# MSU-dcypherlab/mfgp-coverage

Hardware: NVIDIA B200
Metric: GP posterior mean+var + coverage step, grid-points/s (coverage iterations/s = 1000/ms_per_step) (higher is better)
Workload: dtype f64

## Files before the change

### include/mfgp_b200.h

```cpp
#ifndef MFGP_B200_H
#define MFGP_B200_H

#include <stdint.h>

#ifdef __cplusplus
extern "C" {
#endif

#define MFGP_TILE 64

#define MFGP_OK 0
#define MFGP_ERR_INVALID (-1)
#define MFGP_ERR_NOT_SPD (-2)
#define MFGP_ERR_CUDA (-3)
#define MFGP_ERR_EMPTY_CELL (-4)

typedef struct mfgp_params {
    double s_L, l_L;
    double s_H, l_H;
    double rho;
    double noise_L, noise_H;
    double mean_L, mean_H;
    double jitter;
    int32_t multi;
    int32_t reserved;
} mfgp_params;

const char* mfgp_version(void);
const char* mfgp_last_error(void);
int64_t mfgp_debug_chol_trace(int64_t* out, int64_t max_tasks);
int64_t mfgp_launch_count(void);
int64_t mfgp_npad(int64_t n);
int64_t mfgp_workspace_bytes(int64_t npad);


int mfgp_build_train_cov(const double* Xt, int64_t NL, int64_t NH, const mfgp_params* p_host,
                         double* K, int64_t npad, int64_t ld, double* Tt, void* stream);

int mfgp_cholesky(double* K, int64_t npad, int64_t ld, double* W, int64_t ldw, int32_t* info, void* work,
                  void* stream);

int mfgp_tri_inverse(const double* L, int64_t npad, int64_t ld, double* W, int64_t ldw, void* work, void* stream);

int mfgp_whiten(const double* W, int64_t npad, int64_t ldw, const double* y, int64_t NL, int64_t NH,
                const mfgp_params* p_host, double* z, void* stream);

int mfgp_cholesky_append(const double* Xt, int64_t NL, int64_t NH_old, int64_t NH_new, const mfgp_params* p_host,
                         double* K, int64_t ld, double* W, int64_t ldw, const double* y, double* z, double* Tt,
                         int32_t* info, void* work, int64_t work_bytes, void* stream);
int64_t mfgp_append_workspace_bytes(int64_t npad);


int mfgp_posterior(const double* Xs, int64_t G, const double* Tt, int64_t NL, int64_t NH,
                   const double* W, int64_t npad, int64_t ldw, const double* z, const mfgp_params* p_host,
                   double* mu, double* var, double* qred, double* Vc, int64_t ldv, void* stream);

int mfgp_grid_tables(const double* ux, int64_t nx, const double* uy, int64_t ny, const double* Tt, int64_t NL, int64_t NH,
                     int64_t npad, const mfgp_params* p_host, double* TLx, double* TLy, double* THx, double* THy,
                     int64_t ldt, void* stream);
int mfgp_posterior_grid(int64_t ny, int64_t g_lo, int64_t G, const double* TLx, const double* TLy, const double* THx,
                        const double* THy, int64_t ldt, int64_t NL, int64_t NH, const double* W, int64_t npad,
                        int64_t ldw, const double* z, const mfgp_params* p_host, double* mu, double* var, double* qred,
                        double* Vc, int64_t ldv, void* stream);

int mfgp_posterior_update(const double* Xs, int64_t G, const double* Tt, int64_t NL, int64_t NH,
                          const double* W, int64_t npad, int64_t ldw, const double* z, const mfgp_params* p_host,
                          int64_t row_lo, double* mu, double* var, double* qred, double* Vc, int64_t ldv, void* stream);
int mfgp_posterior_grid_update(int64_t ny, int64_t g_lo, int64_t G, const double* TLx, const double* TLy,
                               const double* THx, const double* THy, int64_t ldt, int64_t NL, int64_t NH, const double* W,
                               int64_t npad, int64_t ldw, const double* z, const mfgp_params* p_host, int64_t row_lo,
                               double* mu, double* var, double* qred, double* Vc, int64_t ldv, void* stream);

int mfgp_posterior_grid_factored(const double* ux, int64_t nx, const double* uy, int64_t ny, int64_t ix0, int64_t ncols,
                                 const double* Xt, int64_t NL, int64_t NH, const double* W, int64_t npad, int64_t ldw,
                                 const double* z, const mfgp_params* p_host, int64_t rxL, int64_t ryL, int64_t rxH, int64_t ryH,
                                 double xlo, double xhi, double ylo, double yhi, int64_t chunk_cols,
                                 double* mu, double* var, double* qred, double* Gstore, double* Hz_store, void* work,
                                 int64_t work_bytes, void* stream);
int mfgp_posterior_grid_factored_update(const double* ux, int64_t nx, const double* uy, int64_t ny, int64_t ix0, int64_t ncols,
                                        const double* Xt, int64_t NL, int64_t NH, int64_t row_lo, const double* W, int64_t npad,
                                        int64_t ldw, const double* z, const mfgp_params* p_host, int64_t rxL, int64_t ryL,
                                        int64_t rxH, int64_t ryH, double xlo, double xhi, double ylo, double yhi,
                                        int64_t chunk_cols, double* mu, double* var, double* qred, double* Gstore,
                                        double* Hz_store, void* work, int64_t work_bytes, void* stream);
int64_t mfgp_factored_workspace_bytes(int64_t npad, int64_t ncols, int64_t ny, int64_t rxL, int64_t ryL, int64_t rxH,
                                      int64_t ryH, int64_t chunk_cols);

int64_t mfgp_factored_rhs_cols(int64_t rxL, int64_t ryL, int64_t rxH, int64_t ryH);
int mfgp_factored_prepare(const double* ux, int64_t nx, const double* uy, int64_t ny, int64_t ix0, int64_t ncols,
                          const double* Xt, const double* y, int64_t NL, int64_t NH, int64_t npad, const mfgp_params* p_host,
                          int64_t rxL, int64_t ryL, int64_t rxH, int64_t ryH, double xlo, double xhi, double ylo, double yhi,
                          int64_t chunk_cols, double* Ball, int64_t ldB, void* work, int64_t work_bytes, void* stream);
int64_t mfgp_cholesky_solve_workspace_bytes(int64_t npad, int64_t R);
int mfgp_cholesky_solve(double* K, int64_t npad, int64_t ld, double* W, int64_t ldw, int32_t* info, double* Bm, int64_t ldb,
                        int64_t R, void* work, int64_t work_bytes, void* stream);
int mfgp_posterior_grid_factored_solved(const double* ux, int64_t nx, const double* uy, int64_t ny, int64_t ix0, int64_t ncols,
                                        const double* Xt, int64_t NL, int64_t NH, int64_t npad, const mfgp_params* p_host,
                                        int64_t rxL, int64_t ryL, int64_t rxH, int64_t ryH, double xlo, double xhi, double ylo,
                                        double yhi, int64_t chunk_cols, const double* Yall, int64_t ldY, double* z_out,
                                        double* mu, double* var, double* qred, double* Gstore, double* Hz_store, void* work,
                                        int64_t work_bytes, void* stream);

int64_t mfgp_factored_rhs_cols_trunc(int64_t ry, const int32_t* kx);
int mfgp_posterior_grid_factored_trunc(const double* ux, int64_t nx, const double* uy, int64_t ny, int64_t ix0, int64_t ncols,
                                       const double* Xt, int64_t NL, int64_t NH, const double* W, int64_t npad, int64_t ldw,
                                       const double* z, const mfgp_params* p_host, int64_t rxL, int64_t ryL, int64_t rxH, int64_t ryH,
                                       double xlo, double xhi, double ylo, double yhi, int64_t chunk_cols, const int32_t* kx,
                                       double* mu, double* var, double* qred, double* Gstore, double* Hz_store, void* work,
                                       int64_t work_bytes, void* stream);
int mfgp_factored_prepare_trunc(const double* ux, int64_t nx, const double* uy, int64_t ny, int64_t ix0, int64_t ncols,
                                const double* Xt, const double* y, int64_t NL, int64_t NH, int64_t npad, const mfgp_params* p_host,
                                int64_t rxL, int64_t ryL, int64_t rxH, int64_t ryH, double xlo, double xhi, double ylo, double yhi,
                                int64_t chunk_cols, const int32_t* kx, double* Ball, int64_t ldB, void* work, int64_t work_bytes,
                                void* stream);
double* mfgp_factored_gram_target(int64_t nx, int64_t ny, int64_t ix0, int64_t ncols, int64_t NL, int64_t NH, int64_t npad,
                                  const mfgp_params* p_host, int64_t rxL, int64_t ryL, int64_t rxH, int64_t ryH,
                                  int64_t chunk_cols, const int32_t* kx, int64_t ldY, void* work, int64_t work_bytes);
int64_t mfgp_cholesky_solve_gram_workspace_bytes(int64_t npad, int64_t R);
int mfgp_cholesky_solve_gram(double* K, int64_t npad, int64_t ld, double* W, int64_t ldw, int32_t* info, double* Bm, int64_t ldb,
                             int64_t R, double* M, int64_t ldm, void* work, int64_t work_bytes, void* stream);
int mfgp_posterior_grid_factored_solved_gram(const double* ux, int64_t nx, const double* uy, int64_t ny, int64_t ix0,
                                             int64_t ncols, const double* Xt, int64_t NL, int64_t NH, int64_t npad,
                                             const mfgp_params* p_host, int64_t rxL, int64_t ryL, int64_t rxH, int64_t ryH,
                                             double xlo, double xhi, double ylo, double yhi, int64_t chunk_cols,
                                             const int32_t* kx, const double* Yall, int64_t ldY, double* z_out, double* mu,
                                             double* var, double* qred, double* Gstore, double* Hz_store, void* work,
                                             int64_t work_bytes, void* stream);


int cov_assign_reduce(const double* xy, const double* w, const double* var, const double* f, int64_t G,
                      int64_t base_index,
                      const double* seeds_c, int64_t Ac, const double* poly_xy_c, const int32_t* poly_off_c, int64_t nvert_c,
                      const double* seeds_p, int64_t Ap, const double* poly_xy_p, const int32_t* poly_off_p, int64_t nvert_p,
                      double tie_tol, double amax_k0, double amax_rel,
                      double* cent, double* amax_val, int64_t* amax_idx, double* lossp,
                      uint64_t* member_c, int32_t* tie_count, void* work, int64_t work_bytes, void* stream);
int64_t cov_workspace_bytes(int64_t G, int64_t Ac, int64_t Ap);

int cov_assign_reduce_grid(const double* xy, const double* w, const double* var, const double* f, int64_t G, int64_t ny,
                           int64_t base_index,
                           const double* seeds_c, int64_t Ac, const double* poly_xy_c, const int32_t* poly_off_c, int64_t nvert_c,
                           const double* seeds_p, int64_t Ap, const double* poly_xy_p, const int32_t* poly_off_p, int64_t nvert_p,
                           double tie_tol, double amax_k0, double amax_rel,
                           double* cent, double* amax_val, int64_t* amax_idx, double* lossp,
                           int32_t* tie_count, void* work, int64_t work_bytes, void* stream);

int64_t cov_voronoi_clip_workspace_bytes(int64_t A);
int cov_voronoi_clip(const double* seeds, int64_t A, double xmin, double xmax, double ymin, double ymax, double eps,
                     double* poly_xy, int32_t* poly_off, int64_t cap_vertices, double* areas, int32_t* flag, void* work,
                     int64_t work_bytes, void* stream);

int cov_finish(const double* cent, const double* areas_c, int64_t Ac, const double* lossp, const double* areas_p, int64_t Ap,
               const double* amax_val, const int64_t* amax_idx, double xmin, double xmax, double ymin, double ymax,
               const int32_t* flag0, const int32_t* flag1, const int32_t* flag2, const int32_t* flag3, double* out,
               void* stream);

int cov_argmax(const double* v, int64_t G, int64_t base_index, double k0, double rel, double* out_val, int64_t* out_idx,
               void* work, int64_t work_bytes, void* stream);


int64_t choi_greedy(const double* Xs, int64_t G, double* Vc, int64_t ldv, int64_t n0, int64_t cap, double* var,
                    double* qred, const mfgp_params* p_host, double threshold, double tie_rel, int64_t max_picks,
                    int64_t* picks_host,
                    void* work, int64_t work_bytes, void* stream);


typedef struct mfgp_batch {
    int64_t runs, G, nx, ny, A, NL, cap, algo , iterations, max_samples;
    double xmin, xmax, ymin, ymax, eps, tie_tol, amax_rel;
    const double* xy; const double* f; const double* ux; const double* uy;
    double* Xt; double* y; double* W; double* z;
    double* TxL; double* TyL; double* TxH; double* TyH;
    double* mu; double* var;
    double* pos; double* prev; double* cen;
    int64_t* pos_idx;
    double* prob; int32_t* explore;
    int32_t* Ncur; int32_t* knew; int32_t* status; int32_t* noise_used; int32_t* nsamples; int32_t* ties;
    const double* noise; const double* unif;
    double* log_loss; double* log_agent; double* log_sample;
    double* q; int64_t* picks; int32_t* nplan; int32_t* plan_state; int32_t* pmask; int32_t* ccount; int32_t* cties;
    int32_t* tour_off; int32_t* tour_cur; int64_t* tour;
} mfgp_batch;

int mfgp_batch_step(const mfgp_batch* b_host, const mfgp_params* p_host, int64_t iteration, void* stream);


int mfgp_batch_choi_begin(const mfgp_batch* b_host, const mfgp_params* p_host, void* stream);

int mfgp_batch_choi_plan(const mfgp_batch* b_host, const mfgp_params* p_host, double threshold, int64_t rounds, void* stream);

int mfgp_batch_choi_cluster(const mfgp_batch* b_host, void* stream);

int mfgp_batch_choi_tours(const mfgp_batch* b_host, int64_t n_total, int64_t n_max, double* pts, int64_t* gidx, int32_t* ord,
                          void* work, int64_t work_bytes, void* stream);


int64_t mfgp_nlml_workspace_bytes(int64_t npad);
int mfgp_nlml_grad(const double* L, int64_t npad, int64_t ld, const double* W, int64_t ldw, const double* z, const double* Tt,
                   int64_t NL, int64_t NH, const mfgp_params* p_host, double* out, void* work, int64_t work_bytes,
                   void* stream);


int64_t choi_tsp_workspace_bytes(int64_t n_total);
int choi_tsp_tours(const double* pts, const int32_t* off, int64_t A, int64_t n_total, int64_t n_max, int32_t* order,
                   int32_t* moves, void* work, int64_t work_bytes, void* stream);

#ifdef __cplusplus
}
#endif
#endif
```

### mfgp-coverage_b200/_engine.py

```python
import ctypes
import os
import itertools

import numpy as np
import torch

from . import _native as nat

FUSED_GRAM = os.environ.get("MFGP_FUSED_GRAM", "1") != "0"


def chebyshev_order(length_scale, lo, hi, centre_lo, centre_hi, tol=5e-15, rmax=64):
    half, mid = 0.5 * (hi - lo), 0.5 * (hi + lo)
    if not (half > 0.0) or not (length_scale > 0.0):
        return None
    centres = np.linspace(min(centre_lo, lo), max(centre_hi, hi), 17)
    for r in range(8, rmax + 1, 4):
        j = np.arange(r)
        nodes = mid + half * np.cos(np.pi * (j + 0.5) / r)
        f = np.exp(-0.5 * ((nodes[:, None] - centres[None, :]) / length_scale) ** 2)
        c = (np.cos(np.pi * np.outer(np.arange(r), j + 0.5) / r) @ f) * (2.0 / r)
        scale = max(float(np.abs(c).max()), 1e-300)
        if float(np.abs(c[-3:]).max()) <= tol * scale:
            return r
# ... 312 lines not shown
                                                         nat.ptr(mu), nat.ptr(var), nat.ptr(q_out), None, 0,
                                                         nat.stream_ptr()), "mfgp_posterior_grid_update")
            else:
                nat.check(lib.mfgp_posterior_update(nat.ptr(xs_dev), G, nat.ptr(self.Tt), self.NL, self.NH, nat.ptr(self.W),
                                                    self.npad, self.cap, nat.ptr(self.z), ctypes.byref(self.pstruct),
                                                    row_lo, nat.ptr(mu), nat.ptr(var), nat.ptr(q_out), None, 0,
                                                    nat.stream_ptr()), "mfgp_posterior_update")
            return mu, var
        if axes is not None and self.N > 0:
            TLx, TLy, THx, THy, ldt, _ = self.grid_tables(axes)
            nat.check(lib.mfgp_posterior_grid(axes.ny, int(g_lo), G, nat.ptr(TLx), nat.ptr(TLy), nat.ptr(THx),
                                              nat.ptr(THy), ldt, self.NL, self.NH, nat.ptr(self.W), self.npad, self.cap,
                                              nat.ptr(self.z), ctypes.byref(self.pstruct), nat.ptr(mu), nat.ptr(var),
                                              nat.ptr(q_out), nat.ptr(vcache), ldv, nat.stream_ptr()),
                      "mfgp_posterior_grid")
            return mu, var
        nat.check(lib.mfgp_posterior(nat.ptr(xs_dev), G, nat.ptr(self.Tt), self.NL, self.NH, nat.ptr(self.W),
                                     self.npad, self.cap, nat.ptr(self.z), ctypes.byref(self.pstruct), nat.ptr(mu),
                                     nat.ptr(var), nat.ptr(q_out), nat.ptr(vcache), ldv, nat.stream_ptr()),
                  "mfgp_posterior")
        return mu, var

    def _training_range(self):
        if self._xrange is None:
            xt = self.Xt[:self.N]
            lo, hi = xt.min(dim=0).values.tolist(), xt.max(dim=0).values.tolist()
            self._xrange = (lo[0], hi[0], lo[1], hi[1])
        return self._xrange

    def _cheb_orders(self, axes, p, xlo, xhi):
        ylo, yhi = axes.ylo, axes.yhi
        t = self._training_range()
        c = self._forders
        if c is not None and c[0] == (axes.uid, xlo, xhi, p["l_L"], p["l_H"], p["multi"]) and c[1][0] <= t[0] and c[1][1] >= t[1] \
                and c[1][2] <= t[2] and c[1][3] >= t[3]:
            return c[2]
        mx, my = 0.05 * (axes.xhi - axes.xlo), 0.05 * (yhi - ylo)
        hull = (min(t[0], axes.xlo) - mx, max(t[1], axes.xhi) + mx, min(t[2], ylo) - my, max(t[3], yhi) + my)
        rxH = chebyshev_order(p["l_H"], xlo, xhi, hull[0], hull[1])
        ryH = chebyshev_order(p["l_H"], ylo, yhi, hull[2], hull[3])
        rxL = ryL = 0
        ok = rxH is not None and ryH is not None
        if ok and p["multi"]:
            rxL = chebyshev_order(p["l_L"], xlo, xhi, hull[0], hull[1])
            ryL = chebyshev_order(p["l_L"], ylo, yhi, hull[2], hull[3])
            ok = rxL is not None and ryL is not None
        orders = (rxL, ryL, rxH, ryH) if ok else None
        self._ftrunc = None
        if ok and TRUNCATE:
            parts = [(chebyshev_envelope(p["l_H"], xlo, xhi, hull[0], hull[1], rxH),
                      chebyshev_envelope(p["l_H"], ylo, yhi, hull[2], hull[3], ryH))]
            if p["multi"]:
                parts.append((chebyshev_envelope(p["l_L"], xlo, xhi, hull[0], hull[1], rxL),
                              chebyshev_envelope(p["l_L"], ylo, yhi, hull[2], hull[3], ryL)))
            kp = -(-max(rxL, rxH) // 4) * 4
            parts = [(np.pad(ax, (0, kp - ax.size)), ay) for ax, ay in parts]
            self._ftrunc = chebyshev_truncation(parts, kp, max(ryL, ryH))
        self._forders = ((axes.uid, xlo, xhi, p["l_L"], p["l_H"], p["multi"]), hull, orders)
        return orders

    def _factored_plan(self, axes, g_lo, G):
        ny = axes.ny
        if ny < 2 or axes.nx < 2 or g_lo % ny or G % ny:
            return None
        p = self.params
        N = self.npad
        dense = 0.5 * G * N * N
        if self.factored_min_gain > 0 and dense < 4e9:
            return None
        ix0, ncols = g_lo // ny, G // ny
        if ncols < 2:
            return None
        xs = axes.ux_host[ix0:ix0 + ncols]
        xlo, xhi = float(xs.min()), float(xs.max())
        if not (xhi > xlo):
            return None
        key = (axes.uid, g_lo, G, self.npad, p["l_L"], p["l_H"], p["multi"], self.factored_min_gain)
        orders = self._cheb_orders(axes, p, xlo, xhi)
        if self._fplan is not None and self._fplan[0] == key and self._fplan[2] == orders and self._fplan[3] is self._ftrunc:
            return self._fplan[1]
        plan = None
        if orders is not None:
            rxL, ryL, rxH, ryH = orders
            ry, kp = max(ryL, ryH), -(-max(rxL, rxH) // 4) * 4
            R = ry * kp
            fact = 0.5 * N * N * R + ncols * N * R + ncols * N * 64 * 64 + G * 64 * 64
            if fact * self.factored_min_gain < dense:
                chunk = max(64, min(-(-ncols // 64) * 64, ((1 << 28) // max(self.cap * max(ryL, ryH), 1)) // 64 * 64))
                plan = dict(rxL=rxL, ryL=ryL, rxH=rxH, ryH=ryH, xlo=xlo, xhi=xhi, ylo=axes.ylo, yhi=axes.yhi,
                            ix0=ix0, ncols=ncols, chunk=chunk, macs=fact, dense_macs=dense, kx=self._ftrunc)
        self._fplan = (key, plan, orders, self._ftrunc)
        return plan


    def _wsalloc(self, n, slack=8):
        if not GUARD:
            return torch.empty(n + slack, dtype=torch.float64, device=self.device)
        big = torch.full((n + 1024,), _CANARY, dtype=torch.float64, device=self.device)
        self._guards = [g for g in getattr(self, "_guards", []) if g[0] is not None]
        self._guards.append((big, n))
        return big[512:512 + n]

    def check_guards(self):
        torch.cuda.synchronize(self.device)
        return all(bool((big[:512] == _CANARY).all().item()) and bool((big[512 + n:] == _CANARY).all().item())
                   for big, n in getattr(self, "_guards", []))

    def _factored_work(self, axes, plan):
        need = int(nat.lib().mfgp_factored_workspace_bytes(self.cap, plan["ncols"], axes.ny, plan["rxL"], plan["ryL"],
                                                           plan["rxH"], plan["ryH"], plan["chunk"]))
        if self._fwork is None or self._fwork.numel() * 8 < need:
            self._fwork = self._wsalloc(need // 8)
        return self._fwork

    def _factored_stores(self, plan):
        if not self.incremental:
            return None, None
        lib = nat.lib()
        nG = plan["ncols"] * 64 * 64
        nH = int(lib.mfgp_factored_rhs_cols(plan["rxL"], plan["ryL"], plan["rxH"], plan["ryH"]))
        if self._fG is None or self._fG.numel() < nG:
            self._fG = self._wsalloc(nG, 0)
        if self._fHz is None or self._fHz.numel() < nH:
            self._fHz = self._wsalloc(nH, 0)
        return self._fG, self._fHz

    def _fit_and_posterior_fused(self, axes, plan, mu, var, q_out):
        lib = nat.lib()
        st = nat.stream_ptr()
        pp = ctypes.byref(self.pstruct)
        npad, ld = self.npad, self.cap
        o = (plan["rxL"], plan["ryL"], plan["rxH"], plan["ryH"])
        work = self._factored_work(axes, plan)
        geom = (ctypes.c_double(plan["xlo"]), ctypes.c_double(plan["xhi"]), ctypes.c_double(plan["ylo"]),
                ctypes.c_double(plan["yhi"]), plan["chunk"])
        kx = plan.get("kx") if (FUSED_GRAM and not self.incremental) else None
        M, R = None, 0
        if FUSED_GRAM:
            if kx is not None:
                kxp = ctypes.c_void_p(kx.ctypes.data)
                R = int(lib.mfgp_factored_rhs_cols_trunc(int(kx.size), kxp))
                M = lib.mfgp_factored_gram_target(axes.nx, axes.ny, plan["ix0"], plan["ncols"], self.NL, self.NH, npad, pp, *o,
                                                  plan["chunk"], kxp, R, nat.ptr(work), work.numel() * 8)
            if not M:
                kx, kxp = None, None
                R = int(lib.mfgp_factored_rhs_cols(*o))
                M = lib.mfgp_factored_gram_target(axes.nx, axes.ny, plan["ix0"], plan["ncols"], self.NL, self.NH, npad, pp, *o,
                                                  plan["chunk"], None, R, nat.ptr(work), work.numel() * 8)
        else:
            kx, kxp = None, None
            R = int(lib.mfgp_factored_rhs_cols(*o))
        if self._fB is None or self._fB.numel() < self.cap * R:
            self._fB = self._wsalloc(self.cap * R, 0)
        nat.check(lib.mfgp_build_train_cov(nat.ptr(self.Xt), self.NL, self.NH, pp, nat.ptr(self.K), npad, ld,
                                           nat.ptr(self.Tt), st), "mfgp_build_train_cov")
        nat.check(lib.mfgp_factored_prepare_trunc(nat.ptr(axes.ux), axes.nx, nat.ptr(axes.uy), axes.ny, plan["ix0"], plan["ncols"],
                                                  nat.ptr(self.Xt), nat.ptr(self.y), self.NL, self.NH, npad, pp, *o, *geom,
                                                  kxp if kx is not None else None, nat.ptr(self._fB), R, nat.ptr(work),
                                                  work.numel() * 8, st), "mfgp_factored_prepare")
        ev = self.profile_events
        if ev is not None:
            ev[0].record()
        cneed = int(lib.mfgp_cholesky_solve_gram_workspace_bytes(self.cap, R))
        if self._cwork is None or self._cwork.numel() * 8 < cneed:
            self._cwork = self._wsalloc(cneed // 8)
        nat.check(lib.mfgp_cholesky_solve_gram(nat.ptr(self.K), npad, ld, nat.ptr(self.W), ld, nat.ptr(self.info),
                                               nat.ptr(self._fB), R, R, ctypes.c_void_p(M), R, nat.ptr(self._cwork),
                                               self._cwork.numel() * 8, st), "mfgp_cholesky_solve_gram")
        if ev is not None:
            ev[1].record()
        Gs, Hs = self._factored_stores(plan)
        if M:
            nat.check(lib.mfgp_posterior_grid_factored_solved_gram(
                nat.ptr(axes.ux), axes.nx, nat.ptr(axes.uy), axes.ny, plan["ix0"], plan["ncols"], nat.ptr(self.Xt), self.NL,
                self.NH, npad, pp, *o, *geom, kxp if kx is not None else None, nat.ptr(self._fB), R, nat.ptr(self.z), nat.ptr(mu),
                nat.ptr(var), nat.ptr(q_out), nat.ptr(Gs), nat.ptr(Hs), nat.ptr(work), work.numel() * 8, st),
                "mfgp_posterior_grid_factored_solved_gram")
        else:
            nat.check(lib.mfgp_posterior_grid_factored_solved(
                nat.ptr(axes.ux), axes.nx, nat.ptr(axes.uy), axes.ny, plan["ix0"], plan["ncols"], nat.ptr(self.Xt), self.NL,
                self.NH, npad, pp, *o, *geom, nat.ptr(self._fB), R, nat.ptr(self.z), nat.ptr(mu), nat.ptr(var), nat.ptr(q_out),
                nat.ptr(Gs), nat.ptr(Hs), nat.ptr(work), work.numel() * 8, st), "mfgp_posterior_grid_factored_solved")
        self.rhs_cols = (int(kx.sum()) if kx is not None else max(plan["ryL"], plan["ryH"]) * (-(-max(plan["rxL"], plan["rxH"]) // 4) * 4), R)
        self.fused_gram = bool(M)
        self._dirty = False
        self._w_partial = True

    def _posterior_factored(self, axes, plan, mu, var, q_out, row_lo=0):
        lib = nat.lib()
        work = self._factored_work(axes, plan)
        Gs, Hs = self._factored_stores(plan)
        geom = (ctypes.c_double(plan["xlo"]), ctypes.c_double(plan["xhi"]), ctypes.c_double(plan["ylo"]),
                ctypes.c_double(plan["yhi"]), plan["chunk"])
        o = (plan["rxL"], plan["ryL"], plan["rxH"], plan["ryH"])
        if row_lo > 0 and Gs is not None:
            nat.check(lib.mfgp_posterior_grid_factored_update(
                nat.ptr(axes.ux), axes.nx, nat.ptr(axes.uy), axes.ny, plan["ix0"], plan["ncols"], nat.ptr(self.Xt), self.NL,
                self.NH, int(row_lo), nat.ptr(self.W), self.npad, self.cap, nat.ptr(self.z), ctypes.byref(self.pstruct), *o, *geom,
                nat.ptr(mu), nat.ptr(var), nat.ptr(q_out), nat.ptr(Gs), nat.ptr(Hs), nat.ptr(work), work.numel() * 8,
                nat.stream_ptr()), "mfgp_posterior_grid_factored_update")
            return
        kx = plan.get("kx") if Gs is None else None
        nat.check(lib.mfgp_posterior_grid_factored_trunc(
            nat.ptr(axes.ux), axes.nx, nat.ptr(axes.uy), axes.ny, plan["ix0"], plan["ncols"], nat.ptr(self.Xt), self.NL, self.NH,
            nat.ptr(self.W), self.npad, self.cap, nat.ptr(self.z), ctypes.byref(self.pstruct), *o, *geom,
            ctypes.c_void_p(kx.ctypes.data) if kx is not None else None, nat.ptr(mu), nat.ptr(var),
            nat.ptr(q_out), nat.ptr(Gs), nat.ptr(Hs), nat.ptr(work), work.numel() * 8, nat.stream_ptr()),
            "mfgp_posterior_grid_factored")

    def nlml_grad(self):
        if self.N == 0:
            raise ValueError("likelihood of an empty model")
        self.ensure_factor(need_inverse=True)
        self.check_factor(force=True)
        lib = nat.lib()
        need = int(lib.mfgp_nlml_workspace_bytes(self.npad))
        if self._twork is None or self._twork.numel() * 8 < need:
            self._twork = torch.empty(need // 8 + 8, dtype=torch.float64, device=self.device)
        out = torch.empty(10, dtype=torch.float64, device=self.device)
        nat.check(lib.mfgp_nlml_grad(nat.ptr(self.K), self.npad, self.cap, nat.ptr(self.W), self.cap, nat.ptr(self.z),
                                     nat.ptr(self.Tt), self.NL, self.NH, ctypes.byref(self.pstruct), nat.ptr(out),
                                     nat.ptr(self._twork), self._twork.numel() * 8, nat.stream_ptr()), "mfgp_nlml_grad")
        h = out.cpu().numpy()
        return float(h[0]), h[1:].copy()

    def clone(self):
        self.ensure_factor()
        other = DeviceGP(self.device)
        other.NL, other.NH, other.npad, other.cap = self.NL, self.NH, self.npad, self.cap
        other.params = None if self.params is None else dict(self.params)
        other.pstruct = None if self.params is None else params_struct(self.params)
        other.fitted = self.fitted
        for name in ("Xt", "y", "K", "W", "Tt", "z", "work"):
            t = getattr(self, name)
            setattr(other, name, None if t is None else t.clone())
        other.info = self.info.clone()
        other.fit_id = self.fit_id
        other.incremental = self.incremental
        other.use_factored = self.use_factored
        other.factored_min_gain = self.factored_min_gain
        other.lazy_check = self.lazy_check
        other.defer_fit = self.defer_fit
        other.epoch = self.epoch
        return other
```

### mfgp-coverage_b200/_native.py

```python
import ctypes
import os
from ctypes import POINTER, Structure, c_char_p, c_double, c_int, c_int32, c_int64, c_void_p

_HERE = os.path.dirname(os.path.abspath(__file__))
LIB_PATH = os.path.join(_HERE, "csrc", "libmfgp_b200.so")

MFGP_OK, MFGP_ERR_INVALID, MFGP_ERR_NOT_SPD, MFGP_ERR_CUDA, MFGP_ERR_EMPTY_CELL = 0, -1, -2, -3, -4
TILE = 64


class NativeLibraryMissing(RuntimeError):
    pass


class MfgpParams(Structure):
    _fields_ = [("s_L", c_double), ("l_L", c_double), ("s_H", c_double), ("l_H", c_double), ("rho", c_double),
                ("noise_L", c_double), ("noise_H", c_double), ("mean_L", c_double), ("mean_H", c_double),
                ("jitter", c_double), ("multi", c_int32), ("reserved", c_int32)]


class MfgpBatch(Structure):
    _fields_ = [(n, c_int64) for n in ("runs", "G", "nx", "ny", "A", "NL", "cap", "algo", "iterations", "max_samples")] + \
               [(n, c_double) for n in ("xmin", "xmax", "ymin", "ymax", "eps", "tie_tol", "amax_rel")] + \
               [(n, c_void_p) for n in ("xy", "f", "ux", "uy", "Xt", "y", "W", "z", "TxL", "TyL", "TxH", "TyH", "mu", "var", "pos",
                                        "prev", "cen", "pos_idx", "prob", "explore", "Ncur", "knew", "status", "noise_used",
                                        "nsamples", "ties", "noise", "unif", "log_loss", "log_agent", "log_sample",
                                        "q", "picks", "nplan", "plan_state", "pmask", "ccount", "cties", "tour_off", "tour_cur",
                                        "tour")]


SIGNATURES = {
    "mfgp_version": (c_char_p, []),
    "mfgp_last_error": (c_char_p, []),
    "mfgp_launch_count": (c_int64, []),
    "mfgp_debug_chol_trace": (c_int64, [c_void_p, c_int64]),
    "mfgp_npad": (c_int64, [c_int64]),
    "mfgp_workspace_bytes": (c_int64, [c_int64]),
    "mfgp_build_train_cov": (c_int, [c_void_p, c_int64, c_int64, POINTER(MfgpParams), c_void_p, c_int64, c_int64,
                                     c_void_p, c_void_p]),
    "mfgp_cholesky": (c_int, [c_void_p, c_int64, c_int64, c_void_p, c_int64, c_void_p, c_void_p, c_void_p]),
    "mfgp_tri_inverse": (c_int, [c_void_p, c_int64, c_int64, c_void_p, c_int64, c_void_p, c_void_p]),
    "mfgp_whiten": (c_int, [c_void_p, c_int64, c_int64, c_void_p, c_int64, c_int64, POINTER(MfgpParams), c_void_p,
                            c_void_p]),
    "mfgp_posterior": (c_int, [c_void_p, c_int64, c_void_p, c_int64, c_int64, c_void_p, c_int64, c_int64, c_void_p,
                               POINTER(MfgpParams), c_void_p, c_void_p, c_void_p, c_void_p, c_int64, c_void_p]),
    "mfgp_grid_tables": (c_int, [c_void_p, c_int64, c_void_p, c_int64, c_void_p, c_int64, c_int64, c_int64,
                                 POINTER(MfgpParams), c_void_p, c_void_p, c_void_p, c_void_p, c_int64, c_void_p]),
    "mfgp_posterior_grid": (c_int, [c_int64, c_int64, c_int64, c_void_p, c_void_p, c_void_p, c_void_p, c_int64, c_int64,
                                    c_int64, c_void_p, c_int64, c_int64, c_void_p, POINTER(MfgpParams), c_void_p,
                                    c_void_p, c_void_p, c_void_p, c_int64, c_void_p]),
    "mfgp_cholesky_append": (c_int, [c_void_p, c_int64, c_int64, c_int64, POINTER(MfgpParams), c_void_p, c_int64,
                                     c_void_p, c_int64, c_void_p, c_void_p, c_void_p, c_void_p, c_void_p, c_int64,
                                     c_void_p]),
    "mfgp_append_workspace_bytes": (c_int64, [c_int64]),
    "mfgp_posterior_update": (c_int, [c_void_p, c_int64, c_void_p, c_int64, c_int64, c_void_p, c_int64, c_int64,
                                      c_void_p, POINTER(MfgpParams), c_int64, c_void_p, c_void_p, c_void_p, c_void_p,
                                      c_int64, c_void_p]),
    "mfgp_posterior_grid_update": (c_int, [c_int64, c_int64, c_int64, c_void_p, c_void_p, c_void_p, c_void_p, c_int64,
                                           c_int64, c_int64, c_void_p, c_int64, c_int64, c_void_p, POINTER(MfgpParams),
                                           c_int64, c_void_p, c_void_p, c_void_p, c_void_p, c_int64, c_void_p]),
    "mfgp_posterior_grid_factored": (c_int, [c_void_p, c_int64, c_void_p, c_int64, c_int64, c_int64, c_void_p, c_int64,
                                             c_int64, c_void_p, c_int64, c_int64, c_void_p, POINTER(MfgpParams), c_int64,
                                             c_int64, c_int64, c_int64, c_double, c_double, c_double, c_double, c_int64,
                                             c_void_p, c_void_p, c_void_p, c_void_p, c_void_p, c_void_p, c_int64, c_void_p]),
    "mfgp_posterior_grid_factored_trunc": (c_int, [c_void_p, c_int64, c_void_p, c_int64, c_int64, c_int64, c_void_p, c_int64,
                                                   c_int64, c_void_p, c_int64, c_int64, c_void_p, POINTER(MfgpParams), c_int64,
                                                   c_int64, c_int64, c_int64, c_double, c_double, c_double, c_double, c_int64,
                                                   c_void_p, c_void_p, c_void_p, c_void_p, c_void_p, c_void_p, c_void_p, c_int64,
                                                   c_void_p]),
    "mfgp_posterior_grid_factored_update": (c_int, [c_void_p, c_int64, c_void_p, c_int64, c_int64, c_int64, c_void_p, c_int64,
                                                    c_int64, c_int64, c_void_p, c_int64, c_int64, c_void_p, POINTER(MfgpParams),
                                                    c_int64, c_int64, c_int64, c_int64, c_double, c_double, c_double, c_double,
                                                    c_int64, c_void_p, c_void_p, c_void_p, c_void_p, c_void_p, c_void_p, c_int64,
                                                    c_void_p]),
    "mfgp_factored_workspace_bytes": (c_int64, [c_int64, c_int64, c_int64, c_int64, c_int64, c_int64, c_int64, c_int64]),
    "mfgp_factored_rhs_cols": (c_int64, [c_int64, c_int64, c_int64, c_int64]),
    "mfgp_factored_prepare": (c_int, [c_void_p, c_int64, c_void_p, c_int64, c_int64, c_int64, c_void_p, c_void_p, c_int64,
                                      c_int64, c_int64, POINTER(MfgpParams), c_int64, c_int64, c_int64, c_int64, c_double,
                                      c_double, c_double, c_double, c_int64, c_void_p, c_int64, c_void_p, c_int64, c_void_p]),
    "mfgp_cholesky_solve_workspace_bytes": (c_int64, [c_int64, c_int64]),
    "mfgp_cholesky_solve": (c_int, [c_void_p, c_int64, c_int64, c_void_p, c_int64, c_void_p, c_void_p, c_int64, c_int64,
                                    c_void_p, c_int64, c_void_p]),
    "mfgp_posterior_grid_factored_solved": (c_int, [c_void_p, c_int64, c_void_p, c_int64, c_int64, c_int64, c_void_p, c_int64,
                                                    c_int64, c_int64, POINTER(MfgpParams), c_int64, c_int64, c_int64,
                                                    c_int64, c_double, c_double, c_double, c_double, c_int64, c_void_p,
                                                    c_int64, c_void_p, c_void_p, c_void_p, c_void_p, c_void_p, c_void_p,
                                                    c_void_p, c_int64, c_void_p]),
    "mfgp_factored_rhs_cols_trunc": (c_int64, [c_int64, c_void_p]),
    "mfgp_factored_prepare_trunc": (c_int, [c_void_p, c_int64, c_void_p, c_int64, c_int64, c_int64, c_void_p, c_void_p, c_int64,
                                            c_int64, c_int64, POINTER(MfgpParams), c_int64, c_int64, c_int64, c_int64, c_double,
                                            c_double, c_double, c_double, c_int64, c_void_p, c_void_p, c_int64, c_void_p, c_int64,
                                            c_void_p]),
    "mfgp_factored_gram_target": (c_void_p, [c_int64, c_int64, c_int64, c_int64, c_int64, c_int64, c_int64, POINTER(MfgpParams),
                                             c_int64, c_int64, c_int64, c_int64, c_int64, c_void_p, c_int64, c_void_p, c_int64]),
    "mfgp_cholesky_solve_gram_workspace_bytes": (c_int64, [c_int64, c_int64]),
    "mfgp_cholesky_solve_gram": (c_int, [c_void_p, c_int64, c_int64, c_void_p, c_int64, c_void_p, c_void_p, c_int64, c_int64,
                                         c_void_p, c_int64, c_void_p, c_int64, c_void_p]),
    "mfgp_posterior_grid_factored_solved_gram": (c_int, [c_void_p, c_int64, c_void_p, c_int64, c_int64, c_int64, c_void_p, c_int64,
                                                         c_int64, c_int64, POINTER(MfgpParams), c_int64, c_int64, c_int64,
                                                         c_int64, c_double, c_double, c_double, c_double, c_int64, c_void_p,
                                                         c_void_p, c_int64, c_void_p, c_void_p, c_void_p, c_void_p, c_void_p,
                                                         c_void_p, c_void_p, c_int64, c_void_p]),
    "cov_assign_reduce": (c_int, [c_void_p, c_void_p, c_void_p, c_void_p, c_int64, c_int64,
                                  c_void_p, c_int64, c_void_p, c_void_p, c_int64,
                                  c_void_p, c_int64, c_void_p, c_void_p, c_int64,
                                  c_double, c_double, c_double, c_void_p, c_void_p, c_void_p, c_void_p, c_void_p, c_void_p,
                                  c_void_p, c_int64, c_void_p]),
    "cov_workspace_bytes": (c_int64, [c_int64, c_int64, c_int64]),
    "cov_assign_reduce_grid": (c_int, [c_void_p, c_void_p, c_void_p, c_void_p, c_int64, c_int64, c_int64,
                                       c_void_p, c_int64, c_void_p, c_void_p, c_int64,
                                       c_void_p, c_int64, c_void_p, c_void_p, c_int64,
                                       c_double, c_double, c_double, c_void_p, c_void_p, c_void_p, c_void_p, c_void_p,
                                       c_void_p, c_int64, c_void_p]),
    "cov_voronoi_clip_workspace_bytes": (c_int64, [c_int64]),
    "cov_voronoi_clip": (c_int, [c_void_p, c_int64, c_double, c_double, c_double, c_double, c_double, c_void_p, c_void_p,
                                 c_int64, c_void_p, c_void_p, c_void_p, c_int64, c_void_p]),
    "cov_finish": (c_int, [c_void_p, c_void_p, c_int64, c_void_p, c_void_p, c_int64, c_void_p, c_void_p, c_double,
                           c_double, c_double, c_double, c_void_p, c_void_p, c_void_p, c_void_p, c_void_p, c_void_p]),
    "cov_argmax": (c_int, [c_void_p, c_int64, c_int64, c_double, c_double, c_void_p, c_void_p, c_void_p, c_int64,
                           c_void_p]),
    "choi_greedy": (c_int64, [c_void_p, c_int64, c_void_p, c_int64, c_int64, c_int64, c_void_p, c_void_p,
                              POINTER(MfgpParams), c_double, c_double, c_int64, POINTER(c_int64), c_void_p, c_int64,
                              c_void_p]),
    "mfgp_batch_step": (c_int, [POINTER(MfgpBatch), POINTER(MfgpParams), c_int64, c_void_p]),
    "mfgp_batch_choi_begin": (c_int, [POINTER(MfgpBatch), POINTER(MfgpParams), c_void_p]),
    "mfgp_batch_choi_plan": (c_int, [POINTER(MfgpBatch), POINTER(MfgpParams), c_double, c_int64, c_void_p]),
    "mfgp_batch_choi_cluster": (c_int, [POINTER(MfgpBatch), c_void_p]),
    "mfgp_batch_choi_tours": (c_int, [POINTER(MfgpBatch), c_int64, c_int64, c_void_p, c_void_p, c_void_p, c_void_p, c_int64,
                                      c_void_p]),
    "mfgp_nlml_workspace_bytes": (c_int64, [c_int64]),
    "mfgp_nlml_grad": (c_int, [c_void_p, c_int64, c_int64, c_void_p, c_int64, c_void_p, c_void_p, c_int64, c_int64,
                               POINTER(MfgpParams), c_void_p, c_void_p, c_int64, c_void_p]),
    "choi_tsp_workspace_bytes": (c_int64, [c_int64]),
    "choi_tsp_tours": (c_int, [c_void_p, c_void_p, c_int64, c_int64, c_int64, c_void_p, c_void_p, c_void_p, c_int64,
                               c_void_p]),
}

_lib = None


def lib():
    global _lib
    if _lib is None:
        if not os.path.isfile(LIB_PATH):
            raise NativeLibraryMissing(
                f"{LIB_PATH} not found: build it with `make -C {os.path.dirname(LIB_PATH)}` "
                "(or `python -c 'import __graft_entry__ as g; g.build()'`). There is no CPU fallback.")
        handle = ctypes.CDLL(LIB_PATH)
        for name, (res, args) in SIGNATURES.items():
            fn = getattr(handle, name)
            fn.restype = res
            fn.argtypes = args
        _lib = handle
    return _lib


def last_error():
    return lib().mfgp_last_error().decode()


def check(rc, what):
    if rc == MFGP_OK:
        return
    if rc == MFGP_ERR_CUDA:
        raise RuntimeError(f"{what}: CUDA error: {last_error()}")
    if rc == MFGP_ERR_INVALID:
        raise ValueError(f"{what}: invalid argument")
    raise RuntimeError(f"{what}: error code {rc}")


def npad(n):
    return max(TILE, (int(n) + TILE - 1) // TILE * TILE)


def ptr(t):
    return None if t is None else c_void_p(t.data_ptr())


_side_streams = {}


def side_stream(device=None):
    import torch
    dev = torch.cuda.current_device() if device is None else torch.device(device).index
    if dev is None:
        dev = torch.cuda.current_device()
    if dev not in _side_streams:
        _side_streams[dev] = torch.cuda.Stream(device=dev)
    return _side_streams[dev]


def stream_ptr(stream=None):
    import torch
    if stream is not None:
        return c_void_p(stream.cuda_stream)
    try:
        return c_void_p(torch._C._cuda_getCurrentRawStream(torch._C._cuda_getDevice()))
    except AttributeError:
        return c_void_p(torch.cuda.current_stream().cuda_stream)


def require_cuda():
    import torch
    if not torch.cuda.is_available():
        raise RuntimeError("mfgp_coverage_b200 needs a CUDA device (B200, sm_100a); there is no CPU fallback")
    lib()
```

### mfgp-coverage_b200/csrc/common.cuh

```cuda
#pragma once
#include <cstdint>
#include <cstdio>
#include <cuda.h>
#include <cuda_runtime.h>

#include "../../include/mfgp_b200.h"

namespace mfgp {

void set_last_error(const char* what, cudaError_t e);

#define MFGP_CUDA_CHECK(expr)                                   \
    do {                                                        \
        cudaError_t _e = (expr);                                \
        if (_e != cudaSuccess) {                                \
            ::mfgp::set_last_error(#expr, _e);                  \
            return MFGP_ERR_CUDA;                               \
        }                                                       \
    } while (0)

void count_launch();
#define MFGP_LAUNCH_CHECK()                  \
    do {                                     \
        ::mfgp::count_launch();              \
        MFGP_CUDA_CHECK(cudaGetLastError()); \
    } while (0)

__device__ __forceinline__ void dmma884(double& c0, double& c1, double a, double b) {
    asm volatile("mma.sync.aligned.m8n8k4.row.col.f64.f64.f64.f64 {%0,%1}, {%2}, {%3}, {%0,%1};\n"
                 : "+d"(c0), "+d"(c1)
                 : "d"(a), "d"(b));
}

__device__ __forceinline__ void cp_async16(void* smem_dst, const void* gmem_src, bool valid) {
    unsigned s = static_cast<unsigned>(__cvta_generic_to_shared(smem_dst));
    int bytes = valid ? 16 : 0;
    asm volatile("cp.async.cg.shared.global [%0], [%1], 16, %2;\n" ::"r"(s), "l"(gmem_src), "r"(bytes));
}
__device__ __forceinline__ void cp_async_commit() { asm volatile("cp.async.commit_group;\n" ::); }
template <int N>
__device__ __forceinline__ void cp_async_wait() {
    asm volatile("cp.async.wait_group %0;\n" ::"n"(N));
}

__device__ __forceinline__ uint32_t smem_u32(const void* p) { return static_cast<uint32_t>(__cvta_generic_to_shared(p)); }
__device__ __forceinline__ void mbar_init(uint32_t bar, uint32_t count) {
    asm volatile("mbarrier.init.shared::cta.b64 [%0], %1;\n" ::"r"(bar), "r"(count));
}
__device__ __forceinline__ void mbar_arrive(uint32_t bar) {
    asm volatile("mbarrier.arrive.shared::cta.b64 _, [%0];\n" ::"r"(bar) : "memory");
}
__device__ __forceinline__ void mbar_arrive_expect_tx(uint32_t bar, uint32_t bytes) {
    asm volatile("mbarrier.arrive.expect_tx.shared::cta.b64 _, [%0], %1;\n" ::"r"(bar), "r"(bytes) : "memory");
}
__device__ __forceinline__ void mbar_wait(uint32_t bar, uint32_t parity) {
    uint32_t done;
    do {
        asm volatile(
            "{\n .reg .pred p;\n mbarrier.try_wait.parity.shared::cta.b64 p, [%1], %2;\n selp.u32 %0, 1, 0, p;\n}\n"
            : "=r"(done)
            : "r"(bar), "r"(parity)
            : "memory");
    } while (!done);
}
__device__ __forceinline__ void tma_load_2d(uint32_t dst, const CUtensorMap* map, int c0, int c1, uint32_t bar) {
    asm volatile(
        "cp.async.bulk.tensor.2d.shared::cluster.global.mbarrier::complete_tx::bytes [%0], [%1, {%2, %3}], [%4];\n" ::"r"(dst),
        "l"(map), "r"(c0), "r"(c1), "r"(bar)
        : "memory");
}

typedef CUresult (*EncodeTiledFn)(CUtensorMap*, CUtensorMapDataType, cuuint32_t, void*, const cuuint64_t*, const cuuint64_t*,
                                  const cuuint32_t*, const cuuint32_t*, CUtensorMapInterleave, CUtensorMapSwizzle,
                                  CUtensorMapL2promotion, CUtensorMapFloatOOBfill);
inline int make_tensor_map_2d(CUtensorMap* map, const double* base, int64_t rows, int64_t cols, int64_t ld, int box_cols,
                              int box_rows, CUtensorMapSwizzle swizzle) {
    static EncodeTiledFn encode = nullptr;
    if (!encode) {
        void* fn = nullptr;
        cudaDriverEntryPointQueryResult qres;
        MFGP_CUDA_CHECK(cudaGetDriverEntryPoint("cuTensorMapEncodeTiled", &fn, cudaEnableDefault, &qres));
        if (qres != cudaDriverEntryPointSuccess || !fn) {
            set_last_error("cuTensorMapEncodeTiled entry point unavailable", cudaErrorUnknown);
            return MFGP_ERR_CUDA;
        }
        encode = reinterpret_cast<EncodeTiledFn>(fn);
    }
    const cuuint64_t gdim[2] = {(cuuint64_t)cols, (cuuint64_t)rows};
    const cuuint64_t gstride[1] = {(cuuint64_t)ld * sizeof(double)};
    const cuuint32_t box[2] = {(cuuint32_t)box_cols, (cuuint32_t)box_rows};
    const cuuint32_t estr[2] = {1, 1};
    const CUresult r = encode(map, CU_TENSOR_MAP_DATA_TYPE_FLOAT64, 2, const_cast<double*>(base), gdim, gstride, box, estr,
                              CU_TENSOR_MAP_INTERLEAVE_NONE, swizzle, CU_TENSOR_MAP_L2_PROMOTION_L2_256B,
                              CU_TENSOR_MAP_FLOAT_OOB_FILL_NONE);
    if (r != CUDA_SUCCESS) {
        set_last_error("cuTensorMapEncodeTiled failed", cudaErrorInvalidValue);
        return MFGP_ERR_CUDA;
    }
    return MFGP_OK;
}

__device__ __forceinline__ double rbf_scaled(double ax, double ay, double bx, double by, double scale) {
    double d0 = ax - bx, d1 = ay - by;
    double q = __dadd_rn(__dmul_rn(d0, d0), __dmul_rn(d1, d1));
    return scale * exp(-0.5 * q);
}

struct DevParams {
    double s_L, inv_unused, s_H, rho, rho2, noise_L, noise_H, mean_L, mean_H, jitter, l_L, l_H, k0;
    int multi;
};

inline DevParams make_dev_params(const mfgp_params& p) {
    DevParams d;
    d.s_L = p.multi ? p.s_L : 0.0;
    d.inv_unused = 0.0;
    d.s_H = p.s_H;
    d.rho = p.multi ? p.rho : 1.0;
    d.rho2 = d.rho * d.rho;
    d.noise_L = p.noise_L;
    d.noise_H = p.noise_H;
    d.mean_L = p.mean_L;
    d.mean_H = p.mean_H;
    d.jitter = p.jitter;
    d.l_L = p.multi ? p.l_L : 1.0;
    d.l_H = p.l_H;
    d.k0 = p.multi ? (d.rho2 * p.s_L + p.s_H) : p.s_H;
    d.multi = p.multi;
    return d;
}

}
```

### mfgp-coverage_b200/csrc/gp_factored.cu

```cuda
#include "common.cuh"
#include "gemm_f64.cuh"
#include <cstdlib>
#include <cstring>

namespace mfgp {

constexpr int F_LW = 64;
constexpr int F_MAXR = 64;

struct FTrunc {
    short off[F_MAXR + 1];
    short kx[F_MAXR];
    int ry, cols;
};

struct FPart {
    int rx, ry, kpad;
    int loff;
    double inv_l;
    double* Cx; double* Cy;
    double* B;  double* Y;
    double* Ux;
    double* Yp;
    double* Hz;
};

struct ChebJob { int axis, r; double lo, hi, inv_l; double* C; };
struct ChebJobs { ChebJob j[4]; };
constexpr int CHEB_PTS = 32;
__global__ void __launch_bounds__(256) cheb_coef_kernel(const double* __restrict__ Xt, int N, int npad, ChebJobs jobs) {
    __shared__ double D[F_MAXR * (F_MAXR + 1)];
    __shared__ double node[F_MAXR];
    __shared__ double fv[8][F_MAXR];
    const ChebJob jb = jobs.j[blockIdx.y];
    const int r = jb.r, lane = threadIdx.x & 31, wib = threadIdx.x >> 5;
    double* __restrict__ C = jb.C;
    const double mid = 0.5 * (jb.lo + jb.hi), half = 0.5 * (jb.hi - jb.lo);
    for (int e = threadIdx.x; e < r * r; e += 256) {
        const int k = e / r, j = e % r;
        D[k * (F_MAXR + 1) + j] = cospi(k * (j + 0.5) / r) * (k == 0 ? 1.0 : 2.0) / r;
    }
    for (int j = threadIdx.x; j < r; j += 256) node[j] = mid + half * cospi((j + 0.5) / r);
    __syncthreads();
    for (int i = wib; i < CHEB_PTS; i += 8) {
        const int n = blockIdx.x * CHEB_PTS + i;
        if (n >= npad) break;
        if (n >= N) {
            for (int k = lane; k < r; k += 32) C[(int64_t)k * npad + n] = 0.0;
            continue;
        }
        const double U = Xt[2 * n + jb.axis];
        __syncwarp();
        for (int j = lane; j < r; j += 32) {
            const double d = (node[j] - U) * jb.inv_l;
            fv[wib][j] = exp(-0.5 * d * d);
        }
        __syncwarp();
        for (int k = lane; k < r; k += 32) {
            double s0 = 0.0;
            for (int j = 0; j < r; j++) s0 = fma(fv[wib][j], D[k * (F_MAXR + 1) + j], s0);
            C[(int64_t)k * npad + n] = s0;
        }
    }
}

__global__ void cheb_basis_kernel(const double* __restrict__ u, int i0, int count, int rows_pad, double lo, double hi, int r, int ld,
                                  int col0, double* __restrict__ T) {
    const int i = blockIdx.x * blockDim.x + threadIdx.x;
    if (i >= rows_pad) return;
    double* row = T + (int64_t)i * ld + col0;
    if (i >= count) {
        for (int k = 0; k < r; k++) row[k] = 0.0;
        return;
    }
    const double t = (2.0 * u[i0 + i] - (lo + hi)) / (hi - lo);
    double t0 = 1.0, t1 = t;
    for (int k = 0; k < r; k++) {
        row[k] = t0;
        const double t2 = 2.0 * t * t1 - t0;
        t0 = t1; t1 = t2;
    }
}

struct BTab { const double* Cx; const double* Cy; int rx, ry; double coef_lo, coef_hi; };
__global__ void build_B_merged_kernel(BTab t0, BTab t1, int ntab, int npad, int N, int NL, FTrunc tr, double* __restrict__ B,
                                      int64_t ldB) {
    const int n = blockIdx.y;
    const int e = blockIdx.x * blockDim.x + threadIdx.x;
    if (e >= tr.cols) return;
    int l = 0;
    while (tr.off[l + 1] <= e) l++;
    const int k = e - tr.off[l];
    double v = 0.0;
    if (n < N) {
        if (l < t0.ry && k < t0.rx) v = (n < NL ? t0.coef_lo : t0.coef_hi) * t0.Cy[(int64_t)l * npad + n] * t0.Cx[(int64_t)k * npad + n];
        if (ntab > 1 && l < t1.ry && k < t1.rx)
            v += (n < NL ? t1.coef_lo : t1.coef_hi) * t1.Cy[(int64_t)l * npad + n] * t1.Cx[(int64_t)k * npad + n];
    }
    B[(int64_t)n * ldB + e] = v;
}

__global__ void build_z_block_kernel(const double* __restrict__ y, int npad, int N, int NL, double mean_L, double mean_H,
                                     double* __restrict__ B, int64_t ldB) {
    const int n = blockIdx.x, c = threadIdx.x;
    double v = 0.0;
    if (c == 0 && n < N) v = y[n] - (n < NL ? mean_L : mean_H);
    B[(int64_t)n * ldB + c] = v;
}

__global__ void unpack_Y_kernel(const double* __restrict__ Yall, int64_t ldY, int off, int cols, double* __restrict__ Yp) {
    const int n = blockIdx.y;
    const int e = blockIdx.x * blockDim.x + threadIdx.x;
    if (e < cols) Yp[(int64_t)n * cols + e] = Yall[(int64_t)n * ldY + off + e];
}
__global__ void put_z_block_kernel(const double* __restrict__ z, int npad, double* __restrict__ Yall, int64_t ldY, int zoff) {
    const int n = blockIdx.x, c = threadIdx.x;
    Yall[(int64_t)n * ldY + zoff + c] = (c == 0) ? z[n] : 0.0;
}
__global__ void unpack_z_kernel(const double* __restrict__ Yall, int64_t ldY, int off, int npad, double* __restrict__ z) {
    const int n = blockIdx.x * blockDim.x + threadIdx.x;
    if (n < npad) z[n] = Yall[(int64_t)n * ldY + off];
}

constexpr int HZ_SPLIT = 16;
__global__ void __launch_bounds__(256) hz_partial_kernel(const double* __restrict__ Y, const double* __restrict__ z, int npad, int cols,
                                                         double* __restrict__ part) {
    __shared__ double red[8][32];
    const int e = blockIdx.x * 32 + (threadIdx.x & 31), w = threadIdx.x >> 5;
    const int rows = (npad + HZ_SPLIT - 1) / HZ_SPLIT;
    const int n0 = blockIdx.y * rows, n1 = min(npad, n0 + rows);
    double s = 0.0;
    if (e < cols) {
#pragma unroll 4
        for (int n = n0 + w; n < n1; n += 8) s = fma(z[n], Y[(int64_t)n * cols + e], s);
    }
    red[w][threadIdx.x & 31] = s;
    __syncthreads();
    if (w == 0 && e < cols) {
        double t = 0.0;
#pragma unroll
        for (int k = 0; k < 8; k++) t += red[k][threadIdx.x & 31];
        part[(int64_t)blockIdx.y * cols + e] = t;
    }
}
__global__ void hz_reduce_kernel(const double* __restrict__ part, int cols, double* __restrict__ Hz, int accumulate) {
    const int e = blockIdx.x * blockDim.x + threadIdx.x;
    if (e >= cols) return;
    double t = 0.0;
#pragma unroll
    for (int k = 0; k < HZ_SPLIT; k++) t += part[(int64_t)k * cols + e];
    Hz[e] = accumulate ? Hz[e] + t : t;
}

__global__ void zero_rows_kernel(double* __restrict__ Y, int64_t cols, int nrows) {
    const int64_t e = (int64_t)blockIdx.x * blockDim.x + threadIdx.x;
    if (e < cols * nrows) Y[e] = 0.0;
}

constexpr int G_ROWS = 64;

struct GramArgs {
    const double* YpL; const double* YpH; int ryL, ryH;
    int npad;
    double* Gstore;
    int skip_eval;
    int accumulate;
    const double* HzL; const double* HzH;
    const double* UxL; const double* UxH; int kL, kH;
    const double* Uy;
    int ny; int col_begin;
    double mean, k0;
    double* mu; double* var; double* qred;
    int pitch, nstage;
    int poison;
};
constexpr int G_MAXSTAGE = 6;

__device__ __forceinline__ uint32_t f_smem_u32(const void* p) { return static_cast<uint32_t>(__cvta_generic_to_shared(p)); }
__device__ __forceinline__ void f_mbar_init(uint32_t bar, uint32_t count) {
    asm volatile("mbarrier.init.shared::cta.b64 [%0], %1;\n" ::"r"(bar), "r"(count));
}
__device__ __forceinline__ void f_mbar_arrive_expect_tx(uint32_t bar, uint32_t bytes) {
    asm volatile("mbarrier.arrive.expect_tx.shared::cta.b64 _, [%0], %1;\n" ::"r"(bar), "r"(bytes) : "memory");
}
__device__ __forceinline__ void f_mbar_wait(uint32_t bar, uint32_t parity) {
    uint32_t done;
    do {
        asm volatile(
            "{\n .reg .pred p;\n mbarrier.try_wait.parity.shared::cta.b64 p, [%1], %2;\n selp.u32 %0, 1, 0, p;\n}\n"
            : "=r"(done) : "r"(bar), "r"(parity) : "memory");
    } while (!done);
}
__device__ __forceinline__ void f_bulk_g2s(uint32_t dst, const void* src, uint32_t bytes, uint32_t bar) {
    asm volatile("cp.async.bulk.shared::cluster.global.mbarrier::complete_tx::bytes [%0], [%1], %2, [%3];\n" ::"r"(dst), "l"(src),
                 "r"(bytes), "r"(bar) : "memory");
}

__host__ __device__ constexpr int g_ring_slack(int wm, int pitch) { return wm - pitch > 8 ? wm - pitch : 8; }
template <int WM>
__global__ void __launch_bounds__(128) gram_eval_kernel(GramArgs a) {
    constexpr int NT = WM / 8, NTILES = NT * (NT + 1) / 2;
    constexpr int GP = WM + 2;
    extern __shared__ __align__(16) double gsm[];
    const int P = a.pitch, NST = a.nstage, ry = a.ryH;
    const int ring = NST * G_ROWS * P + g_ring_slack(WM, P);
    double* Ts = gsm;
    double* Gs = gsm + ring;
    double* hs = Gs + WM * GP;
    uint64_t* bars = reinterpret_cast<uint64_t*>(hs + 2 * F_LW);
    const int tid = threadIdx.x, lane = tid & 31, warp = tid >> 5;
    const int col = blockIdx.x;
    const int gq = lane >> 2, tq = lane & 3;
    const double* src = a.YpH + (int64_t)col * a.npad * ry;
    const uint32_t bar0 = f_smem_u32(bars);
    const int fill = a.poison ? ring + WM * GP + 2 * F_LW : ring;
    for (int e = tid; e < fill; e += 128) Ts[e] = e < ring ? 0.0 : __longlong_as_double(-1ll);
    if (tid == 0) {
        for (int i = 0; i < NST; i++) f_mbar_init(bar0 + 8 * i, 1);
        asm volatile("fence.mbarrier_init.release.cluster;\n" ::: "memory");
    }
    __syncthreads();
    asm volatile("fence.proxy.async.shared::cta;\n" ::: "memory");
    const uint32_t chunk_bytes = (uint32_t)(G_ROWS * ry * 8);
    const bool whole = P == ry;
    auto stage = [&](int buf, int n0) {
        if (tid == 0) f_mbar_arrive_expect_tx(bar0 + 8 * buf, chunk_bytes);
        double* dst = Ts + buf * G_ROWS * P;
        if (whole) {
            if (tid == 0) f_bulk_g2s(f_smem_u32(dst), src + (int64_t)n0 * ry, chunk_bytes, bar0 + 8 * buf);
        } else {
            __syncwarp();
            if (tid < G_ROWS) f_bulk_g2s(f_smem_u32(dst + tid * P), src + (int64_t)(n0 + tid) * ry, (uint32_t)(ry * 8), bar0 + 8 * buf);
        }
    };
    double acc[NTILES][2];
#pragma unroll
    for (int t = 0; t < NTILES; t++) acc[t][0] = acc[t][1] = 0.0;
    const int nchunk = a.npad / G_ROWS;
    for (int i = 0; i < NST - 1 && i < nchunk; i++) stage(i, i * G_ROWS);
    int buf = 0, par = 0;
    for (int ch = 0; ch < nchunk; ch++) {
        const int nx = ch + NST - 1;
        if (nx < nchunk) stage(nx % NST, nx * G_ROWS);
        f_mbar_wait(bar0 + 8 * buf, par);
        const double* T = Ts + buf * G_ROWS * P;
#pragma unroll
        for (int ks = 0; ks < G_ROWS / 16; ks++) {
            const double* row = T + (4 * (warp + 4 * ks) + tq) * P + gq;
            double f[NT];
#pragma unroll
            for (int i = 0; i < NT; i++) f[i] = row[8 * i];
#pragma unroll
            for (int i = 0; i < NT; i++)
#pragma unroll
                for (int j = 0; j <= i; j++) dmma884(acc[i * (i + 1) / 2 + j][0], acc[i * (i + 1) / 2 + j][1], f[i], f[j]);
        }
        __syncthreads();
        if (++buf == NST) { buf = 0; par ^= 1; }
    }
#pragma unroll 1
// ... 332 lines not shown
            for (int j = 0; j < NT; j++)
                if (8 * j <= 4 * ks + 3) dmma884(acc[j][0], acc[j][1], av, bf[ks][j]);
        }
        double q = 0.0, m = 0.0;
#pragma unroll
        for (int j = 0; j < NT; j++) {
            const double2 u = __ldg(reinterpret_cast<const double2*>(up + j * 8 + 2 * tq));
            q = fma(acc[j][0], u.x, q); q = fma(acc[j][1], u.y, q);
            m = fma(h0[j], u.x, m); m = fma(h1[j], u.y, m);
        }
        q += __shfl_xor_sync(0xffffffffu, q, 1); m += __shfl_xor_sync(0xffffffffu, m, 1);
        q += __shfl_xor_sync(0xffffffffu, q, 2); m += __shfl_xor_sync(0xffffffffu, m, 2);
        if (tq == 0 && m0 + gq < ny) {
            const int64_t gidx = (int64_t)col * ny + m0 + gq;
            var[gidx] = k0 - q;
            mu[gidx] = mean + m;
            if (qred) qred[gidx] = q;
        }
    }
}

__global__ void gpad_zero_kernel(double* __restrict__ G, int ry, int wm, int col_begin) {
    double* g = G + (int64_t)(col_begin + blockIdx.x) * F_LW * F_LW;
    for (int e = threadIdx.x; e < wm * wm; e += blockDim.x) {
        const int r = e / wm, c = e % wm;
        if (r >= ry || c >= ry) g[r * F_LW + c] = 0.0;
    }
}

__global__ void hz_from_M_kernel(const double* __restrict__ M, int ldm, int zrow, int cols, double* __restrict__ Hz) {
    const int e = blockIdx.x * blockDim.x + threadIdx.x;
    if (e < cols) Hz[e] = M[(int64_t)zrow * ldm + e];
}

}

using namespace mfgp;

static inline int64_t round_up(int64_t v, int64_t m) { return (v + m - 1) / m * m; }

static inline int64_t imax(int64_t a, int64_t b) { return a > b ? a : b; }
constexpr int MR_MAXSPLIT = 8;

extern "C" int64_t mfgp_factored_workspace_bytes(int64_t npad, int64_t ncols, int64_t ny, int64_t rxL, int64_t ryL, int64_t rxH,
                                                 int64_t ryH, int64_t chunk_cols) {
    const int64_t rx = imax(rxL, rxH), ry = imax(ryL, ryH), kp = round_up(rx, 4);
    const int64_t ncp = round_up(ncols, 64), ch = round_up(chunk_cols, 64);
    int64_t d = 0;
    d += ny * 64 + npad + ry * kp;
    d += (rxL + ryL + rxH + ryH) * npad;
    const int64_t Rp = round_up(ry * kp + 1, 64);
    d += 2 * npad * Rp;
    d += ncp * kp;
    const int64_t direct = ch * npad * ry;
    const int64_t gram = (MR_MAXSPLIT + 1) * Rp * Rp + ncp * F_LW * F_LW;
    d += direct > gram ? direct : gram;
    return d * 8 + 4096;
}

extern "C" int64_t mfgp_factored_rhs_cols(int64_t rxL, int64_t ryL, int64_t rxH, int64_t ryH) {
    return round_up(imax(ryL, ryH) * round_up(imax(rxL, rxH), 4) + 1, 64);
}

extern "C" int64_t mfgp_factored_rhs_cols_trunc(int64_t ry, const int32_t* kx) {
    if (!kx || ry <= 0 || ry > F_MAXR) return 0;
    int64_t c = 0;
    for (int64_t l = 0; l < ry; l++) c += kx[l];
    return round_up(c + 1, 64);
}

namespace {
struct FGeom {
    const double* ux; int64_t nx; const double* uy; int64_t ny; int64_t ix0, ncols;
    const double* Xt; int64_t NL, NH, npad;
    const mfgp_params* p;
    int64_t rxL, ryL, rxH, ryH;
    double xlo, xhi, ylo, yhi;
    int64_t chunk;
};
struct FTab { int rx, ry; double inv_l; double* Cx; double* Cy; bool lofi; };
struct FLayout {
    FTab tabs[2]; int ntabs;
    FPart parts[1]; int nparts;
    double* Uy; double* zbuf; int64_t ncp, chunk; bool multi;
    FTrunc tr; bool truncated;
};

bool f_set_trunc(FLayout& L, const int32_t* kx_host) {
    const FPart& f = L.parts[0];
    FTrunc& t = L.tr;
    t.ry = f.ry;
    L.truncated = kx_host != nullptr;
    int o = 0;
    for (int l = 0; l < f.ry; l++) {
        const int k = kx_host ? kx_host[l] : f.kpad;
        if (k < 4 || k > f.kpad || (k & 3)) return false;
        t.off[l] = (short)o; t.kx[l] = (short)k;
        o += k;
    }
    for (int l = f.ry; l < F_MAXR; l++) { t.off[l] = (short)o; t.kx[l] = 0; }
    t.off[F_MAXR] = (short)o;
    t.cols = o;
    return true;
}

int f_validate(const FGeom& g, void* work, int64_t work_bytes) {
    if (!g.ux || !g.uy || !g.Xt || !g.p || !work) return MFGP_ERR_INVALID;
    const int64_t N = g.NL + g.NH;
    if (N <= 0 || g.npad < N || g.npad % MFGP_TILE || g.ncols <= 0 || g.ix0 < 0 || g.ix0 + g.ncols > g.nx || g.ny <= 0) return MFGP_ERR_INVALID;
    const bool multi = g.p->multi != 0;
    if (!multi && (g.rxL || g.ryL || g.NL)) return MFGP_ERR_INVALID;
    if (g.rxH <= 0 || g.ryH <= 0 || g.rxH > F_MAXR || g.ryH > F_MAXR || g.rxL > F_MAXR || g.ryL > F_MAXR || (g.ryL % 4) || (g.ryH % 4))
        return MFGP_ERR_INVALID;
    if (multi && (g.rxL <= 0 || g.ryL <= 0)) return MFGP_ERR_INVALID;
    if (!(g.xhi > g.xlo) || !(g.yhi > g.ylo) || g.chunk <= 0) return MFGP_ERR_INVALID;
    if (work_bytes < mfgp_factored_workspace_bytes(g.npad, g.ncols, g.ny, g.rxL, g.ryL, g.rxH, g.ryH, g.chunk)) return MFGP_ERR_INVALID;
    return MFGP_OK;
}

void f_carve(const FGeom& g, void* work, FLayout& L) {
    L.multi = g.p->multi != 0;
    L.ncp = round_up(g.ncols, 64); L.chunk = round_up(g.chunk, 64);
    double* wp = static_cast<double*>(work);
    auto carve = [&](int64_t n) { double* r = wp; wp += n; return r; };
    L.Uy = carve(g.ny * 64);
    L.zbuf = carve(g.npad);
    L.ntabs = 0;
    auto add_tab = [&](int rx, int ry, double l, bool lofi) {
        FTab& t = L.tabs[L.ntabs++];
        t.rx = rx; t.ry = ry; t.inv_l = 1.0 / l; t.lofi = lofi;
        t.Cx = carve((int64_t)rx * g.npad); t.Cy = carve((int64_t)ry * g.npad);
    };
    if (L.multi) add_tab((int)g.rxL, (int)g.ryL, g.p->l_L, true);
    add_tab((int)g.rxH, (int)g.ryH, g.p->l_H, false);
    FPart& f = L.parts[0];
    L.nparts = 1;
    f.rx = (int)imax(g.rxL, g.rxH); f.ry = (int)imax(g.ryL, g.ryH); f.kpad = (int)round_up(f.rx, 4); f.loff = 0; f.inv_l = 0.0;
    f.Cx = f.Cy = nullptr;
    {
        const int64_t Rp = round_up((int64_t)f.ry * f.kpad + 1, 64);
        f.B = carve(g.npad * Rp); f.Y = carve(g.npad * Rp);
    }
    f.Ux = carve(L.ncp * f.kpad);
    {
        const int64_t Rp = round_up((int64_t)f.ry * f.kpad + 1, 64);
        const int64_t direct = L.chunk * g.npad * f.ry;
        const int64_t gram = (MR_MAXSPLIT + 1) * Rp * Rp + L.ncp * F_LW * F_LW;
        f.Yp = carve(direct > gram ? direct : gram);
    }
    f.Hz = carve((int64_t)f.ry * f.kpad);
    f_set_trunc(L, nullptr);
}

int f_tables_and_B(const FGeom& g, FLayout& L, double* Ball, int64_t ldB, cudaStream_t st) {
    const DevParams dp = make_dev_params(*g.p);
    const int64_t N = g.NL + g.NH, npad = g.npad;
    FPart& f = L.parts[0];
    MFGP_CUDA_CHECK(cudaMemsetAsync(L.Uy, 0, sizeof(double) * g.ny * 64, st));
    MFGP_CUDA_CHECK(cudaMemsetAsync(f.Ux, 0, sizeof(double) * L.ncp * f.kpad, st));
    cheb_basis_kernel<<<(unsigned)((L.ncp + 127) / 128), 128, 0, st>>>(g.ux, (int)g.ix0, (int)g.ncols, (int)L.ncp, g.xlo, g.xhi, f.rx, f.kpad,
                                                                    0, f.Ux);
    MFGP_LAUNCH_CHECK();
    cheb_basis_kernel<<<(unsigned)((g.ny + 127) / 128), 128, 0, st>>>(g.uy, 0, (int)g.ny, (int)g.ny, g.ylo, g.yhi, f.ry, 64, 0, L.Uy);
    MFGP_LAUNCH_CHECK();
    BTab bt[2] = {};
    ChebJobs jobs = {};
    for (int ti = 0; ti < L.ntabs; ti++) {
        FTab& t = L.tabs[ti];
        jobs.j[2 * ti] = ChebJob{0, t.rx, g.xlo, g.xhi, t.inv_l, t.Cx};
        jobs.j[2 * ti + 1] = ChebJob{1, t.ry, g.ylo, g.yhi, t.inv_l, t.Cy};
        bt[ti] = BTab{t.Cx, t.Cy, t.rx, t.ry, t.lofi ? dp.rho * dp.s_L : 0.0, t.lofi ? dp.rho2 * dp.s_L : dp.s_H};
    }
    {
        dim3 cgrid((unsigned)((npad + CHEB_PTS - 1) / CHEB_PTS), (unsigned)(2 * L.ntabs));
        cheb_coef_kernel<<<cgrid, 256, 0, st>>>(g.Xt, (int)N, (int)npad, jobs);
        MFGP_LAUNCH_CHECK();
    }
    const int cols = L.tr.cols;
    dim3 bgrid((unsigned)((cols + 127) / 128), (unsigned)npad);
    build_B_merged_kernel<<<bgrid, 128, 0, st>>>(bt[0], bt[1], L.ntabs, (int)npad, (int)N, (int)g.NL, L.tr, Ball ? Ball : f.B,
                                                Ball ? ldB : (int64_t)cols);
    MFGP_LAUNCH_CHECK();
    return MFGP_OK;
}

int f_tail(const FGeom& g, FLayout& L, const double* z, int64_t rows, double* Gstore, double* Hz_store, int accumulate,
           double* mu, double* var, double* qred, cudaStream_t st) {
    const DevParams dp = make_dev_params(*g.p);
    const int64_t npad = rows;
    const int ry0 = L.parts[0].ry;
    const bool narrow = ry0 <= 40;
    const int wm = narrow ? 40 : 64;
    const int pitch = (ry0 % 8 == 4) ? ry0 : ry0 + 4;
    int nstage = (int)(73728 / (G_ROWS * pitch * 8));
    nstage = nstage < 2 ? 2 : (nstage > G_MAXSTAGE ? G_MAXSTAGE : nstage);
    const size_t gsmem = sizeof(double) * ((size_t)nstage * G_ROWS * pitch + g_ring_slack(wm, pitch) + wm * (wm + 2) + 2 * F_LW) +
                         8 * G_MAXSTAGE + 64;
    const char* pe = getenv("MFGP_DEBUG_POISON_SMEM");
    const int poison = pe && std::strcmp(pe, "1") == 0;
    MFGP_CUDA_CHECK(cudaFuncSetAttribute(gram_eval_kernel<40>, cudaFuncAttributeMaxDynamicSharedMemorySize, (int)gsmem));
    MFGP_CUDA_CHECK(cudaFuncSetAttribute(gram_eval_kernel<64>, cudaFuncAttributeMaxDynamicSharedMemorySize, (int)gsmem));
    int64_t hoff = 0;
    for (int pi = 0; pi < L.nparts; pi++) {
        FPart& f = L.parts[pi];
        const int cols = f.ry * f.kpad;
        if (Hz_store) f.Hz = Hz_store + hoff;
        hz_partial_kernel<<<dim3((unsigned)((cols + 31) / 32), HZ_SPLIT), 256, 0, st>>>(f.Y, z, (int)npad, cols, f.Yp);
        MFGP_LAUNCH_CHECK();
        hz_reduce_kernel<<<(cols + 127) / 128, 128, 0, st>>>(f.Yp, cols, f.Hz, accumulate);
        MFGP_LAUNCH_CHECK();
        hoff += cols;
    }
    for (int64_t c0 = 0; c0 < g.ncols; c0 += L.chunk) {
        const int64_t cc = (g.ncols - c0 < L.chunk) ? g.ncols - c0 : L.chunk;
        const int64_t ccp = round_up(cc, 64);
        for (int pi = 0; pi < L.nparts; pi++) {
            FPart& f = L.parts[pi];
            GemmArgs gm{};
            gm.A = f.Ux + c0 * f.kpad; gm.lda = f.kpad; gm.B = f.Y; gm.ldb = f.kpad; gm.C = f.Yp; gm.ldc = npad * (int64_t)f.ry;
            gm.M = (int)ccp; gm.N = (int)(npad * f.ry); gm.K = f.kpad; gm.alpha = 1.0; gm.beta = 0.0; gm.mode = GEMM_GENERAL;
            int rc = launch_gemm(gm, true, 1, st);
            if (rc) return rc;
        }
        GramArgs ga;
        ga.YpL = nullptr; ga.YpH = L.parts[0].Yp;
        ga.ryL = 0; ga.ryH = L.parts[0].ry;
        ga.npad = (int)npad; ga.Uy = L.Uy; ga.ny = (int)g.ny; ga.col_begin = (int)c0;
        ga.Gstore = Gstore; ga.accumulate = accumulate;
        ga.skip_eval = Gstore != nullptr;
        ga.HzL = nullptr; ga.HzH = L.parts[0].Hz;
        ga.UxL = nullptr; ga.UxH = L.parts[0].Ux + c0 * L.parts[0].kpad;
        ga.kL = 0; ga.kH = L.parts[0].kpad;
        ga.mean = dp.mean_H; ga.k0 = dp.k0; ga.mu = mu; ga.var = var; ga.qred = qred;
        ga.pitch = pitch; ga.nstage = nstage; ga.poison = poison;
        if (narrow) gram_eval_kernel<40><<<(unsigned)cc, 128, gsmem, st>>>(ga);
        else gram_eval_kernel<64><<<(unsigned)cc, 128, gsmem, st>>>(ga);
        MFGP_LAUNCH_CHECK();
    }
    if (Gstore) {
        FPart& f = L.parts[0];
        if (narrow)
            geval_mma_kernel<40><<<(unsigned)g.ncols, 128, 0, st>>>(Gstore, f.Hz, f.Ux, f.kpad, f.ry, L.tr, L.Uy, (int)g.ny, dp.mean_H, dp.k0, mu, var, qred);
        else
            geval_mma_kernel<64><<<(unsigned)g.ncols, 128, 0, st>>>(Gstore, f.Hz, f.Ux, f.kpad, f.ry, L.tr, L.Uy, (int)g.ny, dp.mean_H, dp.k0, mu, var, qred);
        MFGP_LAUNCH_CHECK();
    }
    return MFGP_OK;
}
int gram_route_override() {
    const char* e = getenv("MFGP_GRAM");
    if (!e) return 0;
    return std::strcmp(e, "direct") == 0 ? 1 : (std::strcmp(e, "m") == 0 ? 2 : 0);
}

bool f_gram_wanted(const FGeom& g, const FLayout& L, int64_t ldY) {
    const FPart& f = L.parts[0];
    const int64_t npad = g.npad, cols = L.tr.cols;
    const int wm = f.ry <= 40 ? 40 : 64;
    const int nt8 = (f.kpad + 7) / 8;
    if (ldY % 64 || ldY < cols + 1 || nt8 > 8) return false;
    const int ov = gram_route_override();
    if (L.truncated) return ov != 1;
    const double direct = (double)g.ncols * npad * cols + 0.6 * g.ncols * npad * wm * wm;
    const double gram = 0.5 * npad * (double)ldY * ldY + (double)round_up(g.ncols, 64) * (f.ry * (f.ry + 1) / 2) * 64.0 * nt8 * nt8;
    return !(ov == 1 || (ov == 0 && gram >= direct));
}

int64_t f_max_ldY(const FLayout& L) { return round_up((int64_t)L.parts[0].ry * L.parts[0].kpad + 1, 64); }

int f_tail_gram(const FGeom& g, FLayout& L, const double* Yall, int64_t ldY, double* Gstore, double* Hz_store, double* mu,
                double* var, double* qred, bool m_ready, cudaStream_t st) {
    FPart& f = L.parts[0];
    const int64_t npad = g.npad, cols = L.tr.cols;
    const int wm = f.ry <= 40 ? 40 : 64;
    const int nt8 = (f.kpad + 7) / 8;
    if (!f_gram_wanted(g, L, ldY)) return (m_ready || L.truncated) ? MFGP_ERR_INVALID : 1;
    if (L.truncated && (Gstore || Hz_store)) return MFGP_ERR_INVALID;
    const DevParams dp = make_dev_params(*g.p);
    double* M = f.Yp;
    double* part = M + ldY * ldY;
    double* Gbuf = Gstore ? Gstore : part + (int64_t)MR_MAXSPLIT * ldY * ldY;
    if (!m_ready) {
        const int ntile = (int)(ldY / 64), tiles = ntile * (ntile + 1) / 2;
        int nsplit = 740 / tiles;
        if (nsplit < 1) nsplit = 1;
        if (nsplit > MR_MAXSPLIT) nsplit = MR_MAXSPLIT;
        if (nsplit > npad / 128) nsplit = (int)imax(1, npad / 128);
        const int kchunk = (int)((npad / 64 + nsplit - 1) / nsplit) * 64;
        nsplit = (int)((npad + kchunk - 1) / kchunk);
        GemmArgs gm{};
        gm.A = Yall; gm.lda = ldY; gm.B = Yall; gm.ldb = ldY; gm.C = nsplit > 1 ? part : M; gm.ldc = ldY; gm.strideC = ldY * ldY;
        gm.M = (int)ldY; gm.N = (int)ldY; gm.K = (int)npad; gm.alpha = 1.0; gm.beta = 0.0; gm.mode = GEMM_SYRK_LOWER;
        gm.kchunk = nsplit > 1 ? kchunk : 0;
        int rc = launch_syrk_ata(gm, nsplit, st);
        if (rc) return rc;
        if (nsplit > 1) {
            syrk_reduce_lower_kernel<<<dim3((unsigned)((ldY + 127) / 128), (unsigned)ldY), 128, 0, st>>>(part, nsplit, ldY * ldY, (int)ldY, M);
            MFGP_LAUNCH_CHECK();
        }
    }
    if (Hz_store) f.Hz = Hz_store;
    hz_from_M_kernel<<<(unsigned)((cols + 127) / 128), 128, 0, st>>>(M, (int)ldY, (int)cols, (int)cols, f.Hz);
    MFGP_LAUNCH_CHECK();
    QformArgs qa;
    qa.M = M; qa.ldm = (int)ldY; qa.Ux = f.Ux; qa.kpad = f.kpad; qa.tr = L.tr; qa.ry = f.ry; qa.ncols = (int)g.ncols; qa.G = Gbuf; qa.col_begin = 0;
    const int npairs = f.ry * (f.ry + 1) / 2;
    const int cblocks = (int)((g.ncols + 63) / 64);
    int groups = (148 * 3) / cblocks;
    if (groups < 1) groups = 1;
    if (groups > npairs) groups = npairs;
    qa.pairs_per_cta = (npairs + groups - 1) / groups;
    groups = (npairs + qa.pairs_per_cta - 1) / qa.pairs_per_cta;
    const dim3 qgrid((unsigned)cblocks, (unsigned)groups);
    switch (nt8) {
        case 1: qform_kernel<1, true><<<qgrid, 128, 0, st>>>(qa); break;
        case 2: qform_kernel<2, true><<<qgrid, 128, 0, st>>>(qa); break;
        case 3: qform_kernel<3, true><<<qgrid, 128, 0, st>>>(qa); break;
        case 4: qform_kernel<4, true><<<qgrid, 128, 0, st>>>(qa); break;
        case 5: qform_kernel<5, true><<<qgrid, 128, 0, st>>>(qa); break;
        case 6: qform_kernel<6, true><<<qgrid, 128, 0, st>>>(qa); break;
        case 7: qform_kernel<7, false><<<qgrid, 128, 0, st>>>(qa); break;
        default: qform_kernel<8, false><<<qgrid, 128, 0, st>>>(qa); break;
    }
    MFGP_LAUNCH_CHECK();
    static const bool eval_fma = [] { const char* e = getenv("MFGP_GEVAL"); return e && std::strcmp(e, "fma") == 0; }();
    if (eval_fma) {
        if (wm == 40)
            geval_kernel<40, 2><<<(unsigned)g.ncols, 256, 0, st>>>(Gbuf, f.Hz, f.Ux, f.kpad, f.ry, L.tr, L.Uy, (int)g.ny, dp.mean_H, dp.k0, mu, var, qred);
        else
            geval_kernel<64, 1><<<(unsigned)g.ncols, 256, 0, st>>>(Gbuf, f.Hz, f.Ux, f.kpad, f.ry, L.tr, L.Uy, (int)g.ny, dp.mean_H, dp.k0, mu, var, qred);
    } else if (wm == 40) {
        geval_mma_kernel<40><<<(unsigned)g.ncols, 128, 0, st>>>(Gbuf, f.Hz, f.Ux, f.kpad, f.ry, L.tr, L.Uy, (int)g.ny, dp.mean_H, dp.k0, mu, var, qred);
    } else {
        geval_mma_kernel<64><<<(unsigned)g.ncols, 128, 0, st>>>(Gbuf, f.Hz, f.Ux, f.kpad, f.ry, L.tr, L.Uy, (int)g.ny, dp.mean_H, dp.k0, mu, var, qred);
    }
    MFGP_LAUNCH_CHECK();
    if (Gstore && f.ry < wm) {
        gpad_zero_kernel<<<(unsigned)g.ncols, 128, 0, st>>>(Gbuf, f.ry, wm, 0);
        MFGP_LAUNCH_CHECK();
    }
    return MFGP_OK;
}
}

extern "C" int mfgp_posterior_grid_factored_trunc(const double* ux, int64_t nx, const double* uy, int64_t ny, int64_t ix0, int64_t ncols,
                                                  const double* Xt, int64_t NL, int64_t NH, const double* W, int64_t npad, int64_t ldw,
                                                  const double* z, const mfgp_params* p_host, int64_t rxL, int64_t ryL, int64_t rxH,
                                                  int64_t ryH, double xlo, double xhi, double ylo, double yhi, int64_t chunk_cols,
                                                  const int32_t* kx, double* mu, double* var, double* qred, double* Gstore,
                                                  double* Hz_store, void* work, int64_t work_bytes, void* stream) {
    if (!W || !z || !mu || !var || ldw < npad) return MFGP_ERR_INVALID;
    FGeom g{ux, nx, uy, ny, ix0, ncols, Xt, NL, NH, npad, p_host, rxL, ryL, rxH, ryH, xlo, xhi, ylo, yhi, chunk_cols};
    int rc = f_validate(g, work, work_bytes);
    if (rc) return rc;
    cudaStream_t st = static_cast<cudaStream_t>(stream);
    FLayout L;
    f_carve(g, work, L);
    FPart& f0 = L.parts[0];
    if (kx && !Gstore && !Hz_store && gram_route_override() != 1) {
        if (!f_set_trunc(L, kx)) return MFGP_ERR_INVALID;
    }
    const int64_t cols0 = L.tr.cols, Rp = round_up(cols0 + 1, 64);
    if (!Gstore && !Hz_store && f_gram_wanted(g, L, Rp)) {
        rc = f_tables_and_B(g, L, f0.B, Rp, st);
        if (rc) return rc;
        put_z_block_kernel<<<(unsigned)npad, (int)(Rp - cols0), 0, st>>>(z, (int)npad, f0.B, Rp, (int)cols0);
        MFGP_LAUNCH_CHECK();
        GemmArgs gm{};
        gm.A = W; gm.lda = ldw; gm.B = f0.B; gm.ldb = Rp; gm.C = f0.Y; gm.ldc = Rp;
        gm.M = (int)npad; gm.N = (int)Rp; gm.K = (int)npad; gm.alpha = 1.0; gm.beta = 0.0; gm.mode = GEMM_A_LOWER;
        rc = launch_gemm(gm, false, 1, st);
        if (rc) return rc;
        put_z_block_kernel<<<(unsigned)npad, (int)(Rp - cols0), 0, st>>>(z, (int)npad, f0.Y, Rp, (int)cols0);
        MFGP_LAUNCH_CHECK();
        return f_tail_gram(g, L, f0.Y, Rp, nullptr, nullptr, mu, var, qred, false, st);
    }
    rc = f_tables_and_B(g, L, nullptr, 0, st);
    if (rc) return rc;
    for (int pi = 0; pi < L.nparts; pi++) {
        FPart& f = L.parts[pi];
        GemmArgs gm{};
        gm.A = W; gm.lda = ldw; gm.B = f.B; gm.ldb = (int64_t)f.ry * f.kpad; gm.C = f.Y; gm.ldc = (int64_t)f.ry * f.kpad;
        gm.M = (int)npad; gm.N = f.ry * f.kpad; gm.K = (int)npad; gm.alpha = 1.0; gm.beta = 0.0; gm.mode = GEMM_A_LOWER;
        rc = launch_gemm(gm, false, 1, st);
        if (rc) return rc;
    }
    return f_tail(g, L, z, npad, Gstore, Hz_store, 0, mu, var, qred, st);
}

extern "C" int mfgp_posterior_grid_factored(const double* ux, int64_t nx, const double* uy, int64_t ny, int64_t ix0, int64_t ncols,
                                            const double* Xt, int64_t NL, int64_t NH, const double* W, int64_t npad, int64_t ldw,
                                            const double* z, const mfgp_params* p_host, int64_t rxL, int64_t ryL, int64_t rxH,
                                            int64_t ryH, double xlo, double xhi, double ylo, double yhi, int64_t chunk_cols,
                                            double* mu, double* var, double* qred, double* Gstore, double* Hz_store, void* work,
                                            int64_t work_bytes, void* stream) {
    return mfgp_posterior_grid_factored_trunc(ux, nx, uy, ny, ix0, ncols, Xt, NL, NH, W, npad, ldw, z, p_host, rxL, ryL, rxH, ryH, xlo, xhi,
                                              ylo, yhi, chunk_cols, nullptr, mu, var, qred, Gstore, Hz_store, work, work_bytes, stream);
}

extern "C" int mfgp_factored_prepare_trunc(const double* ux, int64_t nx, const double* uy, int64_t ny, int64_t ix0, int64_t ncols,
                                           const double* Xt, const double* y, int64_t NL, int64_t NH, int64_t npad,
                                           const mfgp_params* p_host, int64_t rxL, int64_t ryL, int64_t rxH, int64_t ryH, double xlo,
                                           double xhi, double ylo, double yhi, int64_t chunk_cols, const int32_t* kx, double* Ball,
                                           int64_t ldB, void* work, int64_t work_bytes, void* stream) {
    if (!y || !Ball) return MFGP_ERR_INVALID;
    FGeom g{ux, nx, uy, ny, ix0, ncols, Xt, NL, NH, npad, p_host, rxL, ryL, rxH, ryH, xlo, xhi, ylo, yhi, chunk_cols};
    int rc = f_validate(g, work, work_bytes);
    if (rc) return rc;
    cudaStream_t st = static_cast<cudaStream_t>(stream);
    FLayout L;
    f_carve(g, work, L);
    if (!f_set_trunc(L, kx)) return MFGP_ERR_INVALID;
    const int64_t zoff = L.tr.cols;
    const int64_t R = round_up(zoff + 1, 64);
    if (ldB < R) return MFGP_ERR_INVALID;
    rc = f_tables_and_B(g, L, Ball, ldB, st);
    if (rc) return rc;
    build_z_block_kernel<<<(unsigned)npad, (int)(R - zoff), 0, st>>>(y, (int)npad, (int)(NL + NH), (int)NL, p_host->mean_L, p_host->mean_H,
                                                                     Ball + zoff, ldB);
    MFGP_LAUNCH_CHECK();
    return MFGP_OK;
}

extern "C" int mfgp_factored_prepare(const double* ux, int64_t nx, const double* uy, int64_t ny, int64_t ix0, int64_t ncols,
                                     const double* Xt, const double* y, int64_t NL, int64_t NH, int64_t npad,
                                     const mfgp_params* p_host, int64_t rxL, int64_t ryL, int64_t rxH, int64_t ryH, double xlo,
                                     double xhi, double ylo, double yhi, int64_t chunk_cols, double* Ball, int64_t ldB, void* work,
                                     int64_t work_bytes, void* stream) {
    return mfgp_factored_prepare_trunc(ux, nx, uy, ny, ix0, ncols, Xt, y, NL, NH, npad, p_host, rxL, ryL, rxH, ryH, xlo, xhi, ylo, yhi,
                                       chunk_cols, nullptr, Ball, ldB, work, work_bytes, stream);
}

namespace {
int f_solved_impl(const FGeom& g, const int32_t* kx, const double* Yall, int64_t ldY, double* z_out, double* mu, double* var,
                  double* qred, double* Gstore, double* Hz_store, void* work, int64_t work_bytes, bool m_ready, cudaStream_t st) {
    if (!Yall || !mu || !var) return MFGP_ERR_INVALID;
    int rc = f_validate(g, work, work_bytes);
    if (rc) return rc;
    FLayout L;
    f_carve(g, work, L);
    if (!f_set_trunc(L, kx)) return MFGP_ERR_INVALID;
    const int64_t npad = g.npad;
    const int64_t zoff = L.tr.cols;
    if (ldY < round_up(zoff + 1, 64) || ldY > f_max_ldY(L)) return MFGP_ERR_INVALID;
    unpack_z_kernel<<<(unsigned)((npad + 255) / 256), 256, 0, st>>>(Yall, ldY, (int)zoff, (int)npad, L.zbuf);
    MFGP_LAUNCH_CHECK();
    if (z_out) MFGP_CUDA_CHECK(cudaMemcpyAsync(z_out, L.zbuf, sizeof(double) * npad, cudaMemcpyDeviceToDevice, st));
    rc = f_tail_gram(g, L, Yall, ldY, Gstore, Hz_store, mu, var, qred, m_ready, st);
    if (rc <= 0) return rc;
    int64_t off = 0;
    for (int pi = 0; pi < L.nparts; pi++) {
        FPart& f = L.parts[pi];
        const int cols = f.ry * f.kpad;
        dim3 ug((unsigned)((cols + 255) / 256), (unsigned)npad);
        unpack_Y_kernel<<<ug, 256, 0, st>>>(Yall, ldY, (int)off, cols, f.Y);
        MFGP_LAUNCH_CHECK();
        off += cols;
    }
    return f_tail(g, L, L.zbuf, npad, Gstore, Hz_store, 0, mu, var, qred, st);
}
}

extern "C" int mfgp_posterior_grid_factored_solved(const double* ux, int64_t nx, const double* uy, int64_t ny, int64_t ix0,
                                                   int64_t ncols, const double* Xt, int64_t NL, int64_t NH, int64_t npad,
                                                   const mfgp_params* p_host, int64_t rxL, int64_t ryL, int64_t rxH, int64_t ryH,
                                                   double xlo, double xhi, double ylo, double yhi, int64_t chunk_cols,
                                                   const double* Yall, int64_t ldY, double* z_out, double* mu, double* var,
                                                   double* qred, double* Gstore, double* Hz_store, void* work,
                                                   int64_t work_bytes, void* stream) {
    FGeom g{ux, nx, uy, ny, ix0, ncols, Xt, NL, NH, npad, p_host, rxL, ryL, rxH, ryH, xlo, xhi, ylo, yhi, chunk_cols};
    return f_solved_impl(g, nullptr, Yall, ldY, z_out, mu, var, qred, Gstore, Hz_store, work, work_bytes, false,
                         static_cast<cudaStream_t>(stream));
}

extern "C" double* mfgp_factored_gram_target(int64_t nx, int64_t ny, int64_t ix0, int64_t ncols, int64_t NL, int64_t NH, int64_t npad,
                                             const mfgp_params* p_host, int64_t rxL, int64_t ryL, int64_t rxH, int64_t ryH,
                                             int64_t chunk_cols, const int32_t* kx, int64_t ldY, void* work, int64_t work_bytes) {
    if (!p_host || !work) return nullptr;
    if (work_bytes < mfgp_factored_workspace_bytes(npad, ncols, ny, rxL, ryL, rxH, ryH, chunk_cols)) return nullptr;
    FGeom g{nullptr, nx, nullptr, ny, ix0, ncols, nullptr, NL, NH, npad, p_host, rxL, ryL, rxH, ryH, 0.0, 1.0, 0.0, 1.0, chunk_cols};
    FLayout L;
    f_carve(g, work, L);
    if (!f_set_trunc(L, kx) || ldY < round_up((int64_t)L.tr.cols + 1, 64) || ldY > f_max_ldY(L)) return nullptr;
    return f_gram_wanted(g, L, ldY) ? L.parts[0].Yp : nullptr;
}

extern "C" int mfgp_posterior_grid_factored_solved_gram(const double* ux, int64_t nx, const double* uy, int64_t ny, int64_t ix0,
                                                        int64_t ncols, const double* Xt, int64_t NL, int64_t NH, int64_t npad,
                                                        const mfgp_params* p_host, int64_t rxL, int64_t ryL, int64_t rxH,
                                                        int64_t ryH, double xlo, double xhi, double ylo, double yhi,
                                                        int64_t chunk_cols, const int32_t* kx, const double* Yall, int64_t ldY,
                                                        double* z_out, double* mu, double* var, double* qred, double* Gstore,
                                                        double* Hz_store, void* work, int64_t work_bytes, void* stream) {
    FGeom g{ux, nx, uy, ny, ix0, ncols, Xt, NL, NH, npad, p_host, rxL, ryL, rxH, ryH, xlo, xhi, ylo, yhi, chunk_cols};
    return f_solved_impl(g, kx, Yall, ldY, z_out, mu, var, qred, Gstore, Hz_store, work, work_bytes, true,
                         static_cast<cudaStream_t>(stream));
}

extern "C" int mfgp_posterior_grid_factored_update(const double* ux, int64_t nx, const double* uy, int64_t ny, int64_t ix0,
                                                   int64_t ncols, const double* Xt, int64_t NL, int64_t NH, int64_t row_lo,
                                                   const double* W, int64_t npad, int64_t ldw, const double* z,
                                                   const mfgp_params* p_host, int64_t rxL, int64_t ryL, int64_t rxH, int64_t ryH,
                                                   double xlo, double xhi, double ylo, double yhi, int64_t chunk_cols, double* mu,
                                                   double* var, double* qred, double* Gstore, double* Hz_store, void* work,
                                                   int64_t work_bytes, void* stream) {
    if (!W || !z || !mu || !var || !Gstore || !Hz_store || ldw < npad || row_lo <= 0 || row_lo >= NL + NH) return MFGP_ERR_INVALID;
    FGeom g{ux, nx, uy, ny, ix0, ncols, Xt, NL, NH, npad, p_host, rxL, ryL, rxH, ryH, xlo, xhi, ylo, yhi, chunk_cols};
    int rc = f_validate(g, work, work_bytes);
    if (rc) return rc;
    cudaStream_t st = static_cast<cudaStream_t>(stream);
    FLayout L;
    f_carve(g, work, L);
    rc = f_tables_and_B(g, L, nullptr, 0, st);
    if (rc) return rc;
    const int64_t rb = row_lo / 64 * 64;
    const int64_t M = npad - rb;
    for (int pi = 0; pi < L.nparts; pi++) {
        FPart& f = L.parts[pi];
        const int64_t cols = (int64_t)f.ry * f.kpad;
        int nsplit = (int)(npad / 512);
        if (nsplit < 1) nsplit = 1;
        if (nsplit > 16) nsplit = 16;
        while (nsplit > 1 && (int64_t)(nsplit + 1) * M * cols > npad * cols) nsplit--;
        const int kchunk = (int)((npad / 64 + nsplit - 1) / nsplit) * 64;
        nsplit = (int)((npad + kchunk - 1) / kchunk);
        double* Ynew = f.Y;
        double* part = f.Y + M * cols;
        if (nsplit > 1) {
            GemmArgs gm{};
            gm.A = W + rb * ldw; gm.lda = ldw; gm.B = f.B; gm.ldb = cols; gm.C = part; gm.ldc = cols; gm.strideC = M * cols;
            gm.M = (int)M; gm.N = (int)cols; gm.K = (int)npad; gm.alpha = 1.0; gm.beta = 0.0; gm.mode = GEMM_GENERAL; gm.kchunk = kchunk;
            rc = launch_gemm(gm, false, nsplit, st);
            if (rc) return rc;
            dim3 rgrid((unsigned)((cols + 127) / 128), (unsigned)M);
            splitk_reduce_kernel<<<rgrid, 128, 0, st>>>(part, nsplit, M * cols, (int)cols, Ynew, cols, (int)M, (int)cols, 1.0, 0.0);
            MFGP_LAUNCH_CHECK();
        } else {
            GemmArgs gm{};
            gm.A = W + rb * ldw; gm.lda = ldw; gm.B = f.B; gm.ldb = cols; gm.C = Ynew; gm.ldc = cols;
            gm.M = (int)M; gm.N = (int)cols; gm.K = (int)npad; gm.alpha = 1.0; gm.beta = 0.0; gm.mode = GEMM_GENERAL;
            rc = launch_gemm(gm, false, 1, st);
            if (rc) return rc;
        }
        if (row_lo > rb) {
            const int64_t nz = (row_lo - rb) * cols;
            zero_rows_kernel<<<(unsigned)((nz + 255) / 256), 256, 0, st>>>(Ynew, cols, (int)(row_lo - rb));
            MFGP_LAUNCH_CHECK();
        }
    }
    return f_tail(g, L, z + rb, M, Gstore, Hz_store, 1, mu, var, qred, st);
}
```

### mfgp-coverage_b200/csrc/gp_fit.cu

```cuda
#include "common.cuh"
#include "gemm_f64.cuh"
#include <cstdlib>
#include <mutex>

namespace mfgp {

__global__ void scaled_coords_kernel(const double* __restrict__ Xt, int N, int npad, DevParams p, double* __restrict__ Tt) {
    const int i = blockIdx.x * blockDim.x + threadIdx.x;
    if (i >= npad) return;
    double4 t = make_double4(0.0, 0.0, 0.0, 0.0);
    if (i < N) {
        const double xi = Xt[2 * i], yi = Xt[2 * i + 1];
        t = make_double4(xi / p.l_L, yi / p.l_L, xi / p.l_H, yi / p.l_H);
    }
    reinterpret_cast<double4*>(Tt)[i] = t;
}

__global__ void build_train_cov_kernel(const double* __restrict__ Xt, int NL, int NH, DevParams p, double* __restrict__ K,
                                       int npad, int64_t ld, const double* __restrict__ Tt, int row_begin) {
    const int j = blockIdx.x * blockDim.x + threadIdx.x;
    const int i = row_begin + blockIdx.y * blockDim.y + threadIdx.y;
    const int N = NL + NH;
    if (i >= npad || j >= npad) return;
    if (j >= ((i >> 6) + 1) * 64) return;
    double v;
    if (i >= N || j >= N) {
        v = (i == j) ? 1.0 : 0.0;
    } else {
        double4 a, b;
        if (Tt != nullptr) {
            a = reinterpret_cast<const double4*>(Tt)[i];
            b = reinterpret_cast<const double4*>(Tt)[j];
        } else {
            const double xi = Xt[2 * i], yi = Xt[2 * i + 1], xj = Xt[2 * j], yj = Xt[2 * j + 1];
            a = make_double4(xi / p.l_L, yi / p.l_L, xi / p.l_H, yi / p.l_H);
            b = make_double4(xj / p.l_L, yj / p.l_L, xj / p.l_H, yj / p.l_H);
        }
        const bool iL = i < NL, jL = j < NL;
        if (p.multi) {
            const double kL = rbf_scaled(a.x, a.y, b.x, b.y, p.s_L);
            if (iL && jL) {
                v = kL;
                if (i == j) v = v + p.noise_L;
            } else if (iL != jL) {
                v = p.rho * kL;
            } else {
                const double kH = rbf_scaled(a.z, a.w, b.z, b.w, p.s_H);
                v = __dadd_rn(__dmul_rn(p.rho2, kL), kH);
                if (i == j) v = v + p.noise_H;
            }
        } else {
            v = rbf_scaled(a.z, a.w, b.z, b.w, p.s_H);
            if (i == j) v = v + p.noise_H;
        }
        if (i == j) v = v + p.jitter;
    }
    K[(int64_t)i * ld + j] = v;
}

constexpr int PB = 64;
constexpr int PLD = PB + 1;

struct PotrfScratch {
    double2 colAB[2][PB], rowAB[2][PB];
    double piv[3][PB / 2];
    double fin[3][PB / 2];
    int bad;
};

__device__ __forceinline__ void tile_bar() { asm volatile("bar.sync 1, 256;\n" ::: "memory"); }

template <int BS>
__device__ __forceinline__ void potrf_diag_body(const double* src, int64_t lds, double* A, int64_t ld,
                                                double* __restrict__ Winv, int64_t ldw, int32_t* __restrict__ info, int col0,
                                                PotrfScratch* sc, double* Lsm = nullptr, double* Wsm = nullptr, int lds_out = 0) {
    constexpr int NB = BS / 16;
    double2 (*colAB)[PB] = sc->colAB;
    double2 (*rowAB)[PB] = sc->rowAB;
    double (*piv)[PB / 2] = sc->piv;
    double (*fin)[PB / 2] = sc->fin;
    int& bad = sc->bad;
    const int tid = threadIdx.x;
    const int ti = tid >> 4, tc = tid & 15;
    if (tid == 0) bad = 0;
    double s[NB][NB], m[NB][NB];
#pragma unroll
    for (int a = 0; a < NB; a++)
#pragma unroll
        for (int b = 0; b < NB; b++) {
            const int r = ti + 16 * a, c = tc + 16 * b;
            s[a][b] = (c <= r) ? src[(int64_t)r * lds + c] : 0.0;
            m[a][b] = (r == c) ? 1.0 : 0.0;
        }
#pragma unroll
    for (int jb = 0; jb < NB; jb++) {
#pragma unroll 1
        for (int jp = 0; jp < 8; jp++) {
            const int k = jb * 8 + jp, j0 = 2 * k, j1 = j0 + 1, jj0 = 2 * jp, buf = k & 1;
            if ((tc & 14) == jj0) {
                double* dst = reinterpret_cast<double*>(colAB[buf]) + (tc & 1);
#pragma unroll
                for (int a = 0; a < NB; a++) dst[2 * (ti + 16 * a)] = s[a][jb];
            }
            if ((ti & 14) == jj0) {
                double* dst = reinterpret_cast<double*>(rowAB[buf]) + (ti & 1);
#pragma unroll
                for (int b = 0; b < NB; b++) dst[2 * (tc + 16 * b)] = m[jb][b];
            }
            tile_bar();
            const double2* col = colAB[buf];
            const double2* row = rowAB[buf];
            double pa = col[j0].x;
            const double2 p1 = col[j1];
            double pb = p1.x, pc = p1.y;
            double det = fma(pa, pc, -(pb * pb));
            if (!(pa > 0.0) || !(det > 0.0)) {
                if (tid == 0 && !bad) {
                    bad = 1;
                    atomicCAS(info, 0, col0 + ((pa > 0.0) ? j1 : j0) + 1);
                }
                pa = 1.0; pb = 0.0; pc = 1.0; det = 1.0;
            }
            if (tid == 0) { piv[0][k] = pa; piv[1][k] = pb; piv[2][k] = pc; }
            const double idet = 1.0 / det;
            const double qa = pc * idet, qb = -pb * idet, qc = pa * idet;
            double t1[NB], t2[NB];
#pragma unroll
            for (int a = 0; a < NB; a++) {
                if (a < jb) continue;
                const double2 x = col[ti + 16 * a];
                t1[a] = fma(qa, x.x, qb * x.y);
                t2[a] = fma(qb, x.x, qc * x.y);
            }
#pragma unroll
            for (int b = 0; b < NB; b++) {
                if (b < jb) continue;
                const double2 y = col[tc + 16 * b];
                const bool live = tc + 16 * b > j1;
#pragma unroll
                for (int a = 0; a < NB; a++) {
                    if (a < b) continue;
                    if (live) s[a][b] = fma(-t1[a], y.x, fma(-t2[a], y.y, s[a][b]));
                }
            }
#pragma unroll
            for (int b = 0; b < NB; b++) {
                if (b > jb) continue;
                const double2 z = row[tc + 16 * b];
#pragma unroll
                for (int a = 0; a < NB; a++) {
                    if (a < jb) continue;
                    const bool live = ti + 16 * a > j1;
                    if (live) m[a][b] = fma(-t1[a], z.x, fma(-t2[a], z.y, m[a][b]));
                }
            }
        }
    }
    tile_bar();
    if (tid < BS / 2) {
        const double a = piv[0][tid], b = piv[1][tid], c = piv[2][tid];
        const double r1 = rsqrt(a);
        const double g = b * r1 * r1;
        fin[0][tid] = r1;
        fin[1][tid] = rsqrt(fma(-g, b, c));
        fin[2][tid] = g;
    }
    tile_bar();
    const bool failed = bad != 0;
#pragma unroll
    for (int a = 0; a < NB; a++)
#pragma unroll
        for (int b = 0; b < NB; b++) {
            const int r = ti + 16 * a, c = tc + 16 * b;
            const double v = s[a][b], w = m[a][b];
            const double vp = __shfl_up_sync(0xffffffffu, v, 1);
            const double wp = __shfl_up_sync(0xffffffffu, w, 16);
            const int kc = c >> 1, kr = r >> 1;
            const double lv = (c & 1) ? (v - fin[2][kc] * vp) * fin[1][kc] : v * fin[0][kc];
            const double wv = (r & 1) ? (w - fin[2][kr] * wp) * fin[1][kr] : w * fin[0][kr];
            const double lo = failed ? ((r == c) ? 1.0 : 0.0) : ((c <= r) ? lv : 0.0);
            const double wo = failed ? ((r == c) ? 1.0 : 0.0) : ((c <= r) ? wv : 0.0);
            if (c <= r) A[(int64_t)r * ld + c] = lo;
            if (Winv != nullptr) Winv[(int64_t)r * ldw + c] = wo;
            if (Lsm != nullptr) Lsm[r * lds_out + c] = lo;
            if (Wsm != nullptr) Wsm[r * lds_out + c] = wo;
        }
}

__global__ void __launch_bounds__(256, 1) potrf_diag_kernel(double* __restrict__ A, int64_t ld, double* __restrict__ Winv,
                                                         int64_t ldw, int32_t* __restrict__ info, int jblk) {
    __shared__ __align__(16) PotrfScratch scratch;
    potrf_diag_body<PB>(A, ld, A, ld, Winv, ldw, info, jblk * PB, &scratch);
}

constexpr int DF_K = 32;
constexpr int DF_LDA = DF_K + 4;
constexpr int DF_LDT = PB + 4;
constexpr int DF_STAGE = PB * DF_LDA;
constexpr int DF_TILE = PB * DF_LDT;
constexpr int DF_NSTAGE = 3;
constexpr int DF_SMEM_DOUBLES = DF_NSTAGE * 2 * DF_STAGE;
constexpr int DF_SMEM_BYTES = DF_SMEM_DOUBLES * 8 + 128;
constexpr int DF_THREADS = 256;
constexpr int DF_CTA_THREADS = DF_THREADS + 32;
constexpr uint32_t DF_MK_BYTES = PB * DF_LDA * 8;
constexpr uint32_t DF_KN_BYTES = DF_K * DF_LDT * 8;
constexpr uint32_t DF_TILE_BYTES = PB * DF_LDT * 8;
constexpr int DF_TMA_MIN_NB = 33;

struct DfArgs {
    double* K; int64_t ld;
    double* W; int64_t ldw;
    double* Bm; int64_t ldb;
    int nb, nr;
    int32_t* info;
    int* flagsL;
    int* flagsY;
    int* ctrl;
    int* pause;
    int total;
    double* M; int64_t ldm;
    int* flagsM;
    int mg, m_full, m_tiles, m_total, m_lead;
    long long spin_limit;
    long long* trace;
    int chain_la;
};

__host__ __device__ __forceinline__ void df_group_rows(int gi, int nb, int mg, int m_full, int& kb, int& ke) {
    if (gi < m_full) { kb = gi * mg; ke = kb + mg; return; }
    kb = m_full * mg;
    int left = nb - kb;
    for (int j = m_full; ; j++) {
        const int sz = left > 1 ? (left + 1) / 2 : left;
        if (j == gi) { ke = kb + sz; return; }
        kb += sz; left -= sz;
    }
}
__host__ __forceinline__ int df_gram_groups(int nb, int mg, int& m_full) {
    m_full = nb >= 2 * mg ? (nb - mg) / mg : 0;
    int left = nb - m_full * mg, n = m_full;
    while (left > 0) { left -= left > 1 ? (left + 1) / 2 : left; n++; }
    return n;
}

__device__ __forceinline__ void df_stamp(long long* trace, int task, int k) {
    if (trace != nullptr && threadIdx.x == 0) {
        unsigned long long t;
        asm volatile("mov.u64 %0, %%globaltimer;\n" : "=l"(t));
        trace[task * 16 + k] = (long long)t;
        trace[task * 16 + 8 + k] = clock64();
    }
}

__device__ __forceinline__ int df_ld_acquire(const int* p) {
    int v;
    asm volatile("ld.acquire.gpu.global.s32 %0, [%1];\n" : "=r"(v) : "l"(p) : "memory");
    return v;
}
__device__ __forceinline__ int df_ld_relaxed(const int* p) {
    int v;
    asm volatile("ld.relaxed.gpu.global.s32 %0, [%1];\n" : "=r"(v) : "l"(p) : "memory");
    return v;
}
__device__ __forceinline__ void df_st_release(int* p, int v) {
    asm volatile("st.release.gpu.global.s32 [%0], %1;\n" ::"l"(p), "r"(v) : "memory");
}
template <bool kTma>
__device__ __forceinline__ void df_publish(int* flag) {
    if constexpr (kTma) asm volatile("fence.proxy.async.global;\n" ::: "memory");
    df_st_release(flag, 1);
}
__device__ __forceinline__ void df_st_relaxed(int* p, int v) {
    asm volatile("st.relaxed.gpu.global.s32 [%0], %1;\n" ::"l"(p), "r"(v) : "memory");
}
__device__ __forceinline__ bool df_wait(const int* f, int* ctrl, int32_t* info, long long limit) {
    int ok = 1;
    if ((threadIdx.x & 31) == 0) {
        if (!df_ld_relaxed(f)) {
            const long long t0 = clock64();
            while (!df_ld_relaxed(f)) {
                __nanosleep(32);
                if (clock64() - t0 > limit) { atomicExch(ctrl + 1, 1); atomicExch(info, -1); }
                if (*reinterpret_cast<volatile int*>(ctrl + 1)) { ok = 0; break; }
            }
        }
        (void)df_ld_acquire(f);
    }
    ok = __shfl_sync(0xffffffffu, ok, 0);
    __syncwarp();
    return ok != 0;
}

__device__ __forceinline__ int df_poll_tiles(const int* fa, int fas, const int* fb, int fbs, int kt0, int nk, int* ctrl, int32_t* info,
                                          long long limit) {
    const int lane = threadIdx.x & 31, j = lane & 15, kt = kt0 + j;
    const int* f = lane < 16 ? fa + (int64_t)kt * fas : fb + (int64_t)kt * fbs;
    long long t0 = 0;
    for (int spin = 0;; spin++) {
        const int v = (kt < nk && (spin == 0 || j == 0)) ? df_ld_relaxed(f) : 0;
        const unsigned m = __ballot_sync(0xffffffffu, v != 0);
        const unsigned both = m & (m >> 16) & 0xffffu;
        const int n = __ffs(~both) - 1;
        if (n > 0) {
            if (j < n) (void)df_ld_acquire(f);
            __syncwarp();
            return kt0 + n - 1;
        }
        int stop = 0;
        if (lane == 0) {
            if (spin == 0) t0 = clock64();
            else if (clock64() - t0 > limit) { atomicExch(ctrl + 1, 1); atomicExch(info, -1); }
            stop = *reinterpret_cast<volatile int*>(ctrl + 1);
        }
        if (__shfl_sync(0xffffffffu, stop, 0)) return -1;
        __nanosleep(32);
    }
}


__device__ __forceinline__ void df_next_task(const DfArgs& g, int& held_m, int& dec_c, int& dec_dnext, int& dec_base, int* task) {
    int c = 0, kind = -1, idx = 0, aux = 0;
    int t = -1;
    if (g.M == nullptr) {
        t = atomicAdd(g.ctrl, 1);
    } else {
        for (;;) {
            const int front = df_ld_relaxed(g.ctrl + 3), drawn = df_ld_relaxed(g.ctrl + 4);
            const bool crit_left = df_ld_relaxed(g.ctrl) < g.total;
            auto runnable = [&](int tm) {
                int kb_, ke_;
                df_group_rows(tm / g.m_tiles, g.nb, g.mg, g.m_full, kb_, ke_);
                const int last_row = ke_ - 1;
                return !crit_left || (drawn > last_row && last_row + 2 <= front);
            };
            if (held_m < 0) {
                const int tm = df_ld_relaxed(g.ctrl + 2);
                if (tm < g.m_total && runnable(tm) && (!crit_left || drawn - front >= g.m_lead)) {
                    const int got = atomicAdd(g.ctrl + 2, 1);
                    if (got < g.m_total) held_m = got;
                }
            }
            if (held_m >= 0 && runnable(held_m)) {
                kind = 3; c = held_m / g.m_tiles; idx = held_m % g.m_tiles;
                int ti = 0;
                while ((ti + 1) * (ti + 2) / 2 <= idx) ti++;
                aux = idx - ti * (ti + 1) / 2;
                idx = ti;
                held_m = -1;
                break;
            }
            if (crit_left) {
                t = atomicAdd(g.ctrl, 1);
                if (t < g.total) break;
                t = -1;
                continue;
            }
            if (held_m < 0 && df_ld_relaxed(g.ctrl + 2) >= g.m_total) break;
        }
    }
    if (t == 0) {
        kind = 2; idx = 0;
    } else if (t > 0 && t < g.total) {
        for (;;) {
            int nchain = 0;
            while (dec_dnext + nchain < g.nb) {
                const int d = dec_dnext + nchain;
                const int place = max(0, d - 1 - (g.chain_la > 0 ? d / g.chain_la : 0));
                if (place != dec_c) break;
                nchain++;
            }
            const int ntile = g.nb - dec_c - 2 > 0 ? g.nb - dec_c - 2 : 0;
            const int n = nchain + ntile + g.nr;
            if (t < dec_base + n) {
                const int tl = t - dec_base;
                c = dec_c;
                if (tl < nchain) { kind = 2; idx = dec_dnext + tl; }
                else if (tl < nchain + ntile) { kind = 0; idx = c + 2 + (tl - nchain); }
                else { kind = 1; idx = tl - nchain - ntile; }
                break;
            }
            dec_base += n; dec_c++; dec_dnext += nchain;
        }
        if (g.M != nullptr) atomicMax(g.ctrl + 4, c);
    }
    task[3] = aux;
    task[0] = kind; task[1] = c; task[2] = idx;
}

__device__ __forceinline__ unsigned df_smid() {
    unsigned smid;
    asm volatile("mov.u32 %0, %%smid;\n" : "=r"(smid));
    return smid;
}
__device__ __forceinline__ int* df_pause_flag(const DfArgs& g) { return g.pause + df_smid(); }

__device__ __forceinline__ void df_exit_record(const DfArgs& g, long long t_wait, long long t_loop, long long t_begin, int n_tasks) {
    unsigned long long tg;
    asm volatile("mov.u64 %0, %%globaltimer;\n" : "=l"(tg));
    long long* o = g.trace + 1024 * 16 + (int64_t)blockIdx.x * 8;
    o[0] = t_wait; o[1] = t_loop; o[2] = clock64() - t_begin; o[3] = n_tasks; o[4] = (long long)tg; o[5] = df_smid();
}

struct DfTask {
    int kind, idx, c, i, gi, tj, kb, nk, nslab, fas, fbs;
    bool rhs, chain, gram, bkn;
    const int* fa;
    const int* fb;
};
__device__ __forceinline__ DfTask df_task(const DfArgs& g, const int* task) {
    DfTask t;
    t.kind = task[0]; t.idx = task[2]; t.tj = task[3];
    t.rhs = t.kind == 1; t.chain = t.kind == 2; t.gram = t.kind == 3; t.bkn = t.rhs || t.gram;
    t.c = t.chain ? t.idx - 1 : (t.gram ? 0 : task[1]);
    t.i = t.rhs ? t.c : t.idx;
    t.gi = t.gram ? task[1] : 0;
    int ke = 0;
    t.kb = 0;
    if (t.gram) df_group_rows(t.gi, g.nb, g.mg, g.m_full, t.kb, ke);
    t.nk = t.gram ? ke - t.kb : (t.chain ? (t.idx > 0 ? t.idx - 1 : 0) : t.c);
    t.nslab = t.nk * (PB / DF_K);
    t.fa = t.gram ? g.flagsY + (int64_t)t.kb * g.nr + t.idx : g.flagsL + (int64_t)t.i * g.nb;
    t.fb = t.gram ? g.flagsY + (int64_t)t.kb * g.nr + t.tj
                  : (t.rhs ? g.flagsY + t.idx : g.flagsL + (int64_t)(t.c > 0 ? t.c : 0) * g.nb);
    t.fas = t.gram ? g.nr : 1;
    t.fbs = t.bkn ? g.nr : 1;
    return t;
}

struct DfOut {
    double* Ct; int64_t ldc;
    double* Cd;
    int* flag;
};
__device__ __forceinline__ DfOut df_out(const DfArgs& g, const int* task) {
    const int kind = task[0], idx = task[2], tj = task[3];
    const bool rhs = kind == 1, chain = kind == 2, gram = kind == 3;
    const int c = chain ? idx - 1 : (gram ? 0 : task[1]), cc = c > 0 ? c : 0;
    const int i = rhs ? c : idx;
    DfOut o;
    o.Ct = gram ? g.M + (int64_t)idx * PB * g.ldm + (int64_t)tj * PB
                : (rhs ? g.Bm + (int64_t)c * PB * g.ldb + (int64_t)idx * PB : g.K + (int64_t)i * PB * g.ld + (int64_t)cc * PB);
    o.ldc = gram ? g.ldm : (rhs ? g.ldb : g.ld);
    o.Cd = g.K + (int64_t)(chain ? idx : 0) * PB * (g.ld + 1);
    o.flag = gram ? g.flagsM + (int64_t)task[1] * g.m_tiles + idx * (idx + 1) / 2 + tj
                  : (rhs ? g.flagsY + (int64_t)c * g.nr + idx : g.flagsL + (int64_t)i * g.nb + cc);
    return o;
}

struct DfTile {
    int wm, wn, gq, tq;
    double acc[2][4][2], acc2[2][4][2];

    __device__ __forceinline__ explicit DfTile(int tid) {
        const int lane = tid & 31, warp = tid >> 5;
        wm = (warp >> 1) * 8; wn = (warp & 1) * 8;
        gq = lane >> 2; tq = lane & 3;
    }

    __device__ __forceinline__ void start(const DfArgs& g, const int* task, const DfTask& tk) {
        const bool has_tile = tk.gram ? tk.gi > 0 : !(tk.chain && tk.idx == 0);
        const DfOut in = df_out(g, task);
#pragma unroll
        for (int x = 0; x < 2; x++)
#pragma unroll
            for (int y = 0; y < 4; y++) {
                const int r = wm + x * 32 + gq, cc = wn + y * 16 + tq * 2;
                double2 v = make_double2(0.0, 0.0), d = make_double2(0.0, 0.0);
                if (has_tile) v = *reinterpret_cast<const double2*>(in.Ct + (int64_t)r * in.ldc + cc);
                if (tk.chain) d = *reinterpret_cast<const double2*>(in.Cd + (int64_t)r * g.ld + cc);
                acc[x][y][0] = tk.gram ? v.x : -v.x; acc[x][y][1] = tk.gram ? v.y : -v.y;
                acc2[x][y][0] = -d.x; acc2[x][y][1] = -d.y;
            }
    }

    __device__ __forceinline__ void slab(const double* As, const double* Bs, const DfTask& tk) {
#pragma unroll
        for (int kk = 0; kk < DF_K; kk += 4) {
            double a[2], b[4];
#pragma unroll
            for (int x = 0; x < 2; x++)
                a[x] = tk.gram ? As[(kk + tq) * DF_LDT + wm + x * 32 + gq] : As[(wm + x * 32 + gq) * DF_LDA + kk + tq];
#pragma unroll
            for (int y = 0; y < 4; y++)
                b[y] = tk.bkn ? Bs[(kk + tq) * DF_LDT + wn + y * 16 + gq] : Bs[(wn + y * 16 + gq) * DF_LDA + kk + tq];
#pragma unroll
            for (int x = 0; x < 2; x++)
#pragma unroll
                for (int y = 0; y < 4; y++) dmma884(acc[x][y][0], acc[x][y][1], a[x], b[y]);
            if (tk.chain) {
#pragma unroll
                for (int y = 0; y < 4; y++) b[y] = As[(wn + y * 16 + gq) * DF_LDA + kk + tq];
#pragma unroll
                for (int x = 0; x < 2; x++)
#pragma unroll
                    for (int y = 0; y < 4; y++)
                        if (wn + y * 16 < wm + x * 32 + 8) dmma884(acc2[x][y][0], acc2[x][y][1], a[x], b[y]);
            }
        }
    }

    __device__ __forceinline__ void store(double* Ct, int64_t ldc) const {
#pragma unroll
        for (int x = 0; x < 2; x++)
#pragma unroll
            for (int y = 0; y < 4; y++) {
                const int r = wm + x * 32 + gq, cc = wn + y * 16 + tq * 2;
                double2 v;
                v.x = acc[x][y][0]; v.y = acc[x][y][1];
                *reinterpret_cast<double2*>(Ct + (int64_t)r * ldc + cc) = v;
            }
    }

    __device__ __forceinline__ void stage_x(double* smem) {
        double* Xs = smem;
#pragma unroll
        for (int x = 0; x < 2; x++)
#pragma unroll
            for (int y = 0; y < 4; y++) {
                const int r = wm + x * 32 + gq, cc = wn + y * 16 + tq * 2;
                Xs[r * DF_LDT + cc] = -acc[x][y][0];
                Xs[r * DF_LDT + cc + 1] = -acc[x][y][1];
                acc[x][y][0] = acc[x][y][1] = 0.0;
            }
    }

    __device__ __forceinline__ void solve(double* smem, const DfTask& tk, const DfOut& out) {
        const double* Xs = smem;
        const double* Ws = smem + DF_TILE;
        double* Ls = smem + 2 * DF_TILE;
#pragma unroll 4
        for (int kk = 0; kk < PB; kk += 4) {
            double a[2], b[4];
            if (!tk.rhs) {
#pragma unroll
                for (int x = 0; x < 2; x++) a[x] = Xs[(wm + x * 32 + gq) * DF_LDT + kk + tq];
#pragma unroll
                for (int y = 0; y < 4; y++) b[y] = (kk < wn + y * 16 + 8) ? Ws[(wn + y * 16 + gq) * DF_LDT + kk + tq] : 0.0;
#pragma unroll
                for (int x = 0; x < 2; x++)
#pragma unroll
                    for (int y = 0; y < 4; y++)
                        if (kk < wn + y * 16 + 8) dmma884(acc[x][y][0], acc[x][y][1], a[x], b[y]);
                continue;
            } else {
#pragma unroll
                for (int x = 0; x < 2; x++) a[x] = Ws[(wm + x * 32 + gq) * DF_LDT + kk + tq];
#pragma unroll
                for (int y = 0; y < 4; y++) b[y] = Xs[(kk + tq) * DF_LDT + wn + y * 16 + gq];
            }
#pragma unroll
            for (int x = 0; x < 2; x++)
#pragma unroll
                for (int y = 0; y < 4; y++) dmma884(acc[x][y][0], acc[x][y][1], a[x], b[y]);
        }
#pragma unroll
        for (int x = 0; x < 2; x++)
#pragma unroll
            for (int y = 0; y < 4; y++) {
                const int r = wm + x * 32 + gq, cc = wn + y * 16 + tq * 2;
                double2 v;
                v.x = acc[x][y][0]; v.y = acc[x][y][1];
                *reinterpret_cast<double2*>(out.Ct + (int64_t)r * out.ldc + cc) = v;
                if (tk.chain) { Ls[r * DF_LDT + cc] = v.x; Ls[r * DF_LDT + cc + 1] = v.y; }
            }
    }

    __device__ __forceinline__ void mm32(const double* A, const double* B, bool b_nk, double (&c)[2][2]) const {
        constexpr int H = PB / 2, LO = DF_LDT;
        const int m0 = wm, n0 = 2 * wn;
        c[0][0] = c[0][1] = c[1][0] = c[1][1] = 0.0;
#pragma unroll
        for (int kk = 0; kk < H; kk += 4) {
            const double av = A[(m0 + gq) * LO + kk + tq];
#pragma unroll
            for (int j = 0; j < 2; j++) {
                const double bv = b_nk ? B[(n0 + 8 * j + gq) * LO + kk + tq] : B[(kk + tq) * LO + n0 + 8 * j + gq];
                dmma884(c[j][0], c[j][1], av, bv);
            }
        }
    }

    template <bool kTma>
    __device__ __forceinline__ void chain_tail(const DfArgs& g, int idx, double* smem, const DfOut& out) {
        double* Xs = smem;
        double* Ls = smem + 2 * DF_TILE;
        double* const Cd = out.Cd;
        double* Wd = g.W + (int64_t)idx * PB * (g.ldw + 1);
        df_stamp(g.trace, idx, 3);
        if (idx > 0) {
            tile_bar();
#pragma unroll 4
            for (int kk = 0; kk < PB; kk += 4) {
                double a[2], b[4];
#pragma unroll
                for (int x = 0; x < 2; x++) a[x] = Ls[(wm + x * 32 + gq) * DF_LDT + kk + tq];
#pragma unroll
                for (int y = 0; y < 4; y++) b[y] = Ls[(wn + y * 16 + gq) * DF_LDT + kk + tq];
#pragma unroll
                for (int x = 0; x < 2; x++)
#pragma unroll
                    for (int y = 0; y < 4; y++)
                        if (wn + y * 16 < wm + x * 32 + 8) dmma884(acc2[x][y][0], acc2[x][y][1], a[x], b[y]);
            }
        }
#pragma unroll
        for (int x = 0; x < 2; x++)
#pragma unroll
            for (int y = 0; y < 4; y++) {
                const int r = wm + x * 32 + gq, cc = wn + y * 16 + tq * 2;
                Xs[r * DF_LDT + cc] = -acc2[x][y][0];
                Xs[r * DF_LDT + cc + 1] = -acc2[x][y][1];
            }
        tile_bar();
        if (idx > 0 && threadIdx.x == 0) df_publish<kTma>(out.flag);
        df_stamp(g.trace, idx, 4);
        PotrfScratch* sc = reinterpret_cast<PotrfScratch*>(smem + DF_TILE);
        constexpr int H = PB / 2, LO = DF_LDT;
        double* L11s = Ls;
        double* W11s = Ls + H;
        double* L21s = Ls + H * LO;
        double* Tsm = Ls + H * LO + H;
        double* W22s = Xs;
        const int m0 = wm, n0 = 2 * wn;
// ... 78 lines not shown
    const bool tracing = g.trace != nullptr;
#else
    long long t_wait = 0, t_loop = 0, t_begin = 0, t_mark = 0;
    int n_tasks = 0;
    constexpr bool tracing = false;
#endif

    for (;;) {
        if (!producer) asm volatile("fence.proxy.async.shared::cta;\n" ::: "memory");
        __syncthreads();
        if (producer && lane == 0) {
            df_next_task(g, dec_s[0], dec_s[1], dec_s[2], dec_s[3], task);
            task[4] = dec_s[4]; task[5] = dec_s[5];
        }
        __syncthreads();
        const DfTask tk = df_task(g, task);
        if (tk.kind < 0) {
            if (tracing && tid == 0) df_exit_record(g, t_wait, t_loop, t_begin, n_tasks);
            return;
        }
        n_tasks++;
        if (tk.gram && tk.gi > 0) {
            if (tracing) t_mark = clock64();
            if (producer) {
                const bool w = df_wait(df_out(g, task).flag - g.m_tiles, g.ctrl, g.info, g.spin_limit);
                if (lane == 0) ready_s[2] = w ? 1 : 0;
            }
            __syncthreads();
            if (tracing) t_wait += clock64() - t_mark;
            if (ready_s[2] == 0) return;
        }

        if (producer) {
            const CUtensorMap* amap = tk.gram ? &bmap : &kmap;
            const CUtensorMap* bsrc = tk.bkn ? &bmap : &kmap;
            const int a_col = tk.gram ? tk.idx * PB : 0, a_row = tk.gram ? tk.kb * PB : tk.i * PB;
            const int b_col = tk.gram ? tk.tj * PB : (tk.rhs ? tk.idx * PB : 0);
            const int b_row = tk.gram ? tk.kb * PB : (tk.rhs ? 0 : (tk.c > 0 ? tk.c : 0) * PB);
            const uint32_t bytes = (tk.gram ? DF_KN_BYTES : DF_MK_BYTES) + (tk.bkn ? DF_KN_BYTES : DF_MK_BYTES);
            int ready_kt = -1, paused = 0;
            for (int s = 0; s < tk.nslab; s++) {
                const bool fresh = (s >> 1) > ready_kt;
                if (fresh) {
                    const int r = df_poll_tiles(tk.fa, tk.fas, tk.fb, tk.fbs, s >> 1, tk.nk, g.ctrl, g.info, g.spin_limit);
                    if (r < 0) {
                        if (lane == 0) abort_s = 1;
                        ready_kt = tk.nk;
                    } else {
                        ready_kt = r;
                    }
                }
                if (lane == 0) {
                    const unsigned gs = (unsigned)task[4] + s;
                    const int slot = gs % DF_NSTAGE;
                    while (paused && df_ld_relaxed(df_pause_flag(g)) && !*reinterpret_cast<volatile int*>(g.ctrl + 1)) __nanosleep(200);
                    if (gs >= DF_NSTAGE) mbar_wait(bar_empty + 8 * slot, ((gs / DF_NSTAGE) + 1) & 1);
                    if (fresh) asm volatile("fence.proxy.async.global;\n" ::: "memory");
                    const uint32_t fbar = bar_full + 8 * slot;
                    mbar_arrive_expect_tx(fbar, bytes);
                    const int k0 = s * DF_K;
                    tma_load_2d(smem_u32(As0 + slot * DF_STAGE), amap, tk.gram ? a_col : k0, tk.gram ? a_row + k0 : a_row, fbar);
                    tma_load_2d(smem_u32(Bs0 + slot * DF_STAGE), bsrc, tk.bkn ? b_col : k0, tk.bkn ? b_row + k0 : b_row, fbar);
                    paused = df_ld_relaxed(df_pause_flag(g));
                }
            }
            if (lane == 0) dec_s[4] += tk.nslab;
            __syncthreads();
            if (abort_s) return;
            if (tk.gram || (tk.chain && tk.idx == 0)) continue;
            const bool w = df_wait(g.flagsL + (int64_t)tk.c * g.nb + tk.c, g.ctrl, g.info, g.spin_limit);
            if (lane == 0) {
                ready_s[3] = w ? 1 : 0;
                dec_s[5]++;
                if (w) {
                    if (tk.chain) df_st_relaxed(df_pause_flag(g), 1);
                    asm volatile("fence.proxy.async.global;\n" ::: "memory");
                    mbar_arrive_expect_tx(bar_w, DF_TILE_BYTES);
                    tma_load_2d(smem_u32(df_smem + DF_TILE), &wmap, tk.c * PB, tk.c * PB, bar_w);
                } else {
                    mbar_arrive(bar_w);
                }
            }
            if (!w) return;
            continue;
        }

        DfTile f(tid);
        f.start(g, task, tk);
        const long long t_loop0 = tracing ? clock64() : 0;
        const unsigned gs0 = task[4];
        for (int s = 0; s < tk.nslab; s++) {
            const unsigned gs = gs0 + s;
            const int slot = gs % DF_NSTAGE;
            if (tracing) t_mark = clock64();
            mbar_wait(bar_full + 8 * slot, (gs / DF_NSTAGE) & 1);
            if (tracing) t_wait += clock64() - t_mark;
            f.slab(As0 + slot * DF_STAGE, Bs0 + slot * DF_STAGE, tk);
            __syncwarp();
            if (lane == 0) mbar_arrive(bar_empty + 8 * slot);
        }
        __syncthreads();
        if (abort_s) return;

        if (tracing) t_loop += clock64() - t_loop0;
        if (tk.chain) df_stamp(g.trace, tk.idx, 0);
        const DfOut out = df_out(g, task);
        if (tk.gram) {
            f.store(out.Ct, out.ldc);
        } else if (!(tk.chain && tk.idx == 0)) {
            f.stage_x(df_smem);
            if (tracing) t_mark = clock64();
            tile_bar();
            if (tk.chain) df_stamp(g.trace, tk.idx, 1);
            mbar_wait(bar_w, task[5] & 1);
            if (tracing) t_wait += clock64() - t_mark;
            if (ready_s[3] == 0) return;
            if (tk.chain) df_stamp(g.trace, tk.idx, 2);
            f.solve(df_smem, tk, out);
        }
        if (tk.chain) f.chain_tail<true>(g, tk.idx, df_smem, out);
        df_finish<true>(g, tk, out.flag);
    }
}

__global__ void __launch_bounds__(DF_THREADS, 2) chol_dataflow_cpasync_kernel(DfArgs g) {
    extern __shared__ __align__(16) double df_smem[];
    __shared__ int task[4];
    __shared__ int ready_s[4];
    const int tid = threadIdx.x, lane = tid & 31, warp = tid >> 5;
    double* As0 = df_smem;
    double* Bs0 = df_smem + DF_NSTAGE * DF_STAGE;
    int* const my_pause = df_pause_flag(g);
#ifdef MFGP_DF_ACCOUNTING
    long long t_wait = 0, t_loop = 0, t_begin = clock64(), t_mark = 0;
    int n_tasks = 0;
    const bool tracing = g.trace != nullptr;
#else
    long long t_wait = 0, t_loop = 0, t_begin = 0, t_mark = 0;
    int n_tasks = 0;
    constexpr bool tracing = false;
#endif
    int held_m = -1, dec_c = 0, dec_dnext = 1, dec_base = 1;

    for (;;) {
        __syncthreads();
        if (tid == 0) df_next_task(g, held_m, dec_c, dec_dnext, dec_base, task);
        __syncthreads();
        const DfTask tk = df_task(g, task);
        if (tk.kind < 0) {
            if (tracing && tid == 0) df_exit_record(g, t_wait, t_loop, t_begin, n_tasks);
            return;
        }
        n_tasks++;
        const double* Ag = tk.gram ? g.Bm + (int64_t)tk.kb * PB * g.ldb + (int64_t)tk.idx * PB : g.K + (int64_t)tk.i * PB * g.ld;
        const double* Bg = tk.gram ? g.Bm + (int64_t)tk.kb * PB * g.ldb + (int64_t)tk.tj * PB
                                   : (tk.rhs ? g.Bm + (int64_t)tk.idx * PB : g.K + (int64_t)(tk.c > 0 ? tk.c : 0) * PB * g.ld);
        bool ok = true;
        if (tk.gram && tk.gi > 0) {
            if (tracing) t_mark = clock64();
            if (warp == 0) {
                const bool w = df_wait(df_out(g, task).flag - g.m_tiles, g.ctrl, g.info, g.spin_limit);
                if (lane == 0) ready_s[2] = w ? 1 : 0;
            }
            __syncthreads();
            if (tracing) t_wait += clock64() - t_mark;
            if (ready_s[2] == 0) return;
        }
        DfTile f(tid);
        f.start(g, task, tk);

        auto issue = [&](int s) {
            const int k0 = s * DF_K;
            double* As = As0 + (s % DF_NSTAGE) * DF_STAGE;
            double* Bs = Bs0 + (s % DF_NSTAGE) * DF_STAGE;
            if (!tk.gram) {
#pragma unroll
                for (int e = tid; e < PB * (DF_K / 2); e += DF_THREADS) {
                    const int r = e >> 4, q = e & 15;
                    cp_async16(&As[r * DF_LDA + q * 2], Ag + (int64_t)r * g.ld + k0 + q * 2, true);
                }
            } else {
#pragma unroll
                for (int e = tid; e < DF_K * (PB / 2); e += DF_THREADS) {
                    const int r = e >> 5, q = e & 31;
                    cp_async16(&As[r * DF_LDT + q * 2], Ag + (int64_t)(k0 + r) * g.ldb + q * 2, true);
                }
            }
            if (!tk.bkn) {
#pragma unroll
                for (int e = tid; e < PB * (DF_K / 2); e += DF_THREADS) {
                    const int r = e >> 4, q = e & 15;
                    cp_async16(&Bs[r * DF_LDA + q * 2], Bg + (int64_t)r * g.ld + k0 + q * 2, true);
                }
            } else {
#pragma unroll
                for (int e = tid; e < DF_K * (PB / 2); e += DF_THREADS) {
                    const int r = e >> 5, q = e & 31;
                    cp_async16(&Bs[r * DF_LDT + q * 2], Bg + (int64_t)(k0 + r) * g.ldb + q * 2, true);
                }
            }
            cp_async_commit();
        };
        auto sample = [&](int kt) -> int {
            if (kt >= tk.nk) return 0;
            if (!(df_ld_relaxed(tk.fa + (int64_t)kt * tk.fas) & df_ld_relaxed(tk.fb + (int64_t)kt * tk.fbs))) return 0;
            return df_ld_acquire(tk.fa + (int64_t)kt * tk.fas) & df_ld_acquire(tk.fb + (int64_t)kt * tk.fbs);
        };
        auto peek = [&](int kt) -> int {
            return kt < tk.nk ? (df_ld_relaxed(tk.fa + (int64_t)kt * tk.fas) & df_ld_relaxed(tk.fb + (int64_t)kt * tk.fbs)) : 0;
        };
        auto confirm = [&](int kt) -> int {
            return df_ld_acquire(tk.fa + (int64_t)kt * tk.fas) & df_ld_acquire(tk.fb + (int64_t)kt * tk.fbs);
        };
        const int nslab = tk.nslab;
        int paused = 0;
        const long long t_loop0 = tracing ? clock64() : 0;
        int staged = 0, ready_kt = -1;
        if (tid == 0) ready_s[0] = sample(0) ? 0 : -1;
        __syncthreads();
        ready_kt = ready_s[0];
        while (staged < nslab && staged < DF_NSTAGE - 1 && (staged >> 1) <= ready_kt) { issue(staged); staged++; }
        for (int s = 0; s < nslab; s++) {
            if (staged <= s) {
                const int kt = s >> 1;
                if (tracing) t_mark = clock64();
                if (warp == 0) {
                    bool w = df_wait(tk.fa + (int64_t)kt * tk.fas, g.ctrl, g.info, g.spin_limit);
                    w = df_wait(tk.fb + (int64_t)kt * tk.fbs, g.ctrl, g.info, g.spin_limit) && w;
                    if (lane == 0) ready_s[2] = w ? 1 : 0;
                }
                __syncthreads();
                if (tracing) t_wait += clock64() - t_mark;
                ok = (ready_s[2] != 0) && ok;
                ready_kt = max(ready_kt, kt);
                issue(s);
                staged = s + 1;
                if (staged < nslab && (staged >> 1) <= ready_kt) { issue(staged); staged++; }
            }
            if (staged - 1 - s >= 1) cp_async_wait<1>(); else cp_async_wait<0>();
            if (lane == 0) {
                while (paused && df_ld_relaxed(my_pause)) __nanosleep(200);
                paused = df_ld_relaxed(my_pause);
            }
            if (__syncthreads_or(!ok)) return;
            ready_kt = max(ready_kt, ready_s[s & 1]);
            while (staged < nslab && staged <= s + DF_NSTAGE - 1 && (staged >> 1) <= ready_kt) { issue(staged); staged++; }
            const int seen = (tid == 0) ? peek(ready_kt + 1) : 0;
            f.slab(As0 + (s % DF_NSTAGE) * DF_STAGE, Bs0 + (s % DF_NSTAGE) * DF_STAGE, tk);
            if (tid == 0) ready_s[(s + 1) & 1] = (seen && confirm(ready_kt + 1)) ? ready_kt + 1 : ready_kt;
        }
        __syncthreads();

        if (tracing) t_loop += clock64() - t_loop0;
        if (tk.chain) df_stamp(g.trace, tk.idx, 0);
        const DfOut out = df_out(g, task);
        if (tk.gram) {
            f.store(out.Ct, out.ldc);
        } else if (!(tk.chain && tk.idx == 0)) {
            f.stage_x(df_smem);
            if (tracing) t_mark = clock64();
            if (warp == 0) {
                const bool w = df_wait(g.flagsL + (int64_t)tk.c * g.nb + tk.c, g.ctrl, g.info, g.spin_limit);
                if (lane == 0) ready_s[2] = w ? 1 : 0;
            }
            __syncthreads();
            if (tracing) t_wait += clock64() - t_mark;
            const bool okd = ready_s[2] != 0;
            if (tk.chain && tid == 0) df_st_relaxed(my_pause, 1);
            if (tk.chain) df_stamp(g.trace, tk.idx, 1);
            const double* Wcc = g.W + (int64_t)tk.c * PB * (g.ldw + 1);
            double* Ws = df_smem + DF_TILE;
#pragma unroll
            for (int e = tid; e < PB * (PB / 2); e += DF_THREADS) {
                const int r = e >> 5, q = e & 31;
                cp_async16(&Ws[r * DF_LDT + q * 2], Wcc + (int64_t)r * g.ldw + q * 2, okd);
            }
            cp_async_commit();
            cp_async_wait<0>();
            __syncthreads();
            if (!okd) {
                if (tk.chain && tid == 0) df_st_relaxed(my_pause, 0);
                return;
            }
            if (tk.chain) df_stamp(g.trace, tk.idx, 2);
            f.solve(df_smem, tk, out);
        }
        if (tk.chain) f.chain_tail<false>(g, tk.idx, df_smem, out);
        df_finish<false>(g, tk, out.flag);
    }
}

__global__ void zero_offdiag_blocks_kernel(double* __restrict__ W, int npad, int64_t ldw) {
    const int j = blockIdx.x * blockDim.x + threadIdx.x;
    const int i = blockIdx.y;
    if (j >= npad) return;
    if ((i >> 6) != (j >> 6)) W[(int64_t)i * ldw + j] = 0.0;
}

__global__ void zero_cols_kernel(double* __restrict__ Wcol, int64_t ldw) { Wcol[(int64_t)blockIdx.y * ldw + threadIdx.x] = 0.0; }

__global__ void whiten_kernel(const double* __restrict__ W, int npad, int64_t ldw, const double* __restrict__ y, int NL,
                              int NH, double mean_L, double mean_H, double* __restrict__ z, int row_begin) {
    const int row = row_begin + blockIdx.x * (blockDim.x >> 5) + (threadIdx.x >> 5);
    const int lane = threadIdx.x & 31;
    if (row >= npad) return;
    const int N = NL + NH;
    const int kmax = min(row + 1, N);
    double s = 0.0;
    for (int k = lane; k < kmax; k += 32) {
        const double yc = y[k] - (k < NL ? mean_L : mean_H);
        s += W[(int64_t)row * ldw + k] * yc;
    }
#pragma unroll
    for (int o = 16; o > 0; o >>= 1) s += __shfl_xor_sync(0xffffffffu, s, o);
    if (lane == 0) z[row] = s;
}

}

using namespace mfgp;

extern "C" int64_t mfgp_npad(int64_t n) {
    if (n <= 0) return MFGP_TILE;
    return (n + MFGP_TILE - 1) / MFGP_TILE * MFGP_TILE;
}

constexpr int DF_CTRL_INTS = 16;
constexpr int DF_MIN_MG = 2;
static int64_t df_scratch_ints(int64_t npad, int64_t R, bool gram = false) {
    const int64_t nb = npad / PB, nr = (R + PB - 1) / PB;
    int64_t n = DF_CTRL_INTS + 1024 + nb * nb + nb * nr;
    if (gram) n += ((nb + DF_MIN_MG - 1) / DF_MIN_MG + 16) * (nr * (nr + 1) / 2);
    return n;
}
static int64_t df_scratch_bytes(int64_t npad, int64_t R, bool gram = false) {
    return (df_scratch_ints(npad, R, gram) * 4 + 255) / 256 * 256;
}

extern "C" int64_t mfgp_workspace_bytes(int64_t npad) {
    return npad * npad * 2 + (int64_t)PB * PB * 8 + 256 + df_scratch_bytes(npad, 0);
}

extern "C" int64_t mfgp_cholesky_solve_workspace_bytes(int64_t npad, int64_t R) { return df_scratch_bytes(npad, R); }
extern "C" int64_t mfgp_cholesky_solve_gram_workspace_bytes(int64_t npad, int64_t R) { return df_scratch_bytes(npad, R, true); }

extern "C" int mfgp_build_train_cov(const double* Xt, int64_t NL, int64_t NH, const mfgp_params* p_host, double* K,
                                    int64_t npad, int64_t ld, double* Tt, void* stream) {
    if (!p_host || !K || NL < 0 || NH < 0 || npad < NL + NH || npad % MFGP_TILE || ld < npad) return MFGP_ERR_INVALID;
    if (NL + NH > 0 && !Xt) return MFGP_ERR_INVALID;
    if (!p_host->multi && NL != 0) return MFGP_ERR_INVALID;
    cudaStream_t st = static_cast<cudaStream_t>(stream);
    dim3 block(32, 8), grid((unsigned)((npad + 31) / 32), (unsigned)((npad + 7) / 8));
    const DevParams dp = make_dev_params(*p_host);
    if (Tt) {
        scaled_coords_kernel<<<(unsigned)((npad + 255) / 256), 256, 0, st>>>(Xt, (int)(NL + NH), (int)npad, dp, Tt);
        MFGP_LAUNCH_CHECK();
    }
    build_train_cov_kernel<<<grid, block, 0, st>>>(Xt, (int)NL, (int)NH, dp, K, (int)npad, ld, Tt, 0);
    MFGP_LAUNCH_CHECK();
    return MFGP_OK;
}

namespace {
struct DfMap {
    const double* base = nullptr;
    int64_t rows = 0, cols = 0, ld = 0;
    CUtensorMap map;
};
int df_cached_map(DfMap& m, const double* base, int64_t rows, int64_t cols, int64_t ld, int box_cols, int box_rows) {
    if (m.base == base && m.rows == rows && m.cols == cols && m.ld == ld) return MFGP_OK;
    m.base = nullptr;
    const int rc = make_tensor_map_2d(&m.map, base, rows, cols, ld, box_cols, box_rows, CU_TENSOR_MAP_SWIZZLE_NONE);
    if (rc) return rc;
    m.base = base; m.rows = rows; m.cols = cols; m.ld = ld;
    return MFGP_OK;
}

struct DfScratch {
    long long* trace = nullptr;
    int trace_nb = 0;
    int trace_grid = 0;
    int sms = 0;
    std::mutex map_mu;
    DfMap kmap, bmap, wmap;
};
DfScratch g_df[16];

int chol_dataflow(double* K, int64_t npad, int64_t ld, double* W, int64_t ldw, int32_t* info, double* Bm, int64_t ldb, int64_t R,
                  double* M, int64_t ldm, int* scratch, cudaStream_t st) {
    int dev = 0;
    MFGP_CUDA_CHECK(cudaGetDevice(&dev));
    if (dev < 0 || dev >= 16 || !scratch) return MFGP_ERR_INVALID;
    auto aligned = [](const void* p, int64_t l) { return (reinterpret_cast<uintptr_t>(p) & 15) == 0 && (l & 1) == 0; };
    if (!aligned(K, ld) || !aligned(W, ldw) || (R > 0 && !aligned(Bm, ldb)) || (M && !aligned(M, ldm))) return MFGP_ERR_INVALID;
    DfScratch& sc = g_df[dev];
    const int nb = (int)(npad / PB), nr = (int)(R / PB);
    const int64_t need = df_scratch_ints(npad, R, M != nullptr);
    if (!sc.sms) MFGP_CUDA_CHECK(cudaDeviceGetAttribute(&sc.sms, cudaDevAttrMultiProcessorCount, dev));
    MFGP_CUDA_CHECK(cudaMemsetAsync(scratch, 0, need * sizeof(int), st));
    MFGP_CUDA_CHECK(cudaMemsetAsync(info, 0, sizeof(int32_t), st));
    DfArgs a{};
    a.K = K; a.ld = ld; a.W = W; a.ldw = ldw; a.Bm = Bm; a.ldb = ldb; a.nb = nb; a.nr = nr; a.info = info;
    a.ctrl = scratch; a.pause = scratch + DF_CTRL_INTS; a.flagsL = a.pause + 1024; a.flagsY = a.flagsL + (int64_t)nb * nb;
    a.total = nb + (nb - 1) * (nb - 2) / 2 + nb * nr;
    if (M != nullptr && nr > 0) {
        static const int mg_env = [] { const char* e = getenv("MFGP_DF_MG"); return e ? atoi(e) : 8; }();
        static const int lead_env = [] { const char* e = getenv("MFGP_DF_MLEAD"); return e ? atoi(e) : 32; }();
        a.M = M; a.ldm = ldm; a.flagsM = a.flagsY + (int64_t)nb * nr;
        a.mg = mg_env < DF_MIN_MG ? DF_MIN_MG : mg_env;
        a.m_tiles = nr * (nr + 1) / 2;
        a.m_total = df_gram_groups(nb, a.mg, a.m_full) * a.m_tiles;
        a.m_lead = lead_env;
    }
    static const bool want_trace = [] { const char* e = getenv("MFGP_DF_TRACE"); return e && atoi(e) != 0; }();
    if (want_trace) {
        if (!sc.trace) MFGP_CUDA_CHECK(cudaMalloc(&sc.trace, 1024 * 24 * sizeof(long long)));
        MFGP_CUDA_CHECK(cudaMemsetAsync(sc.trace, 0, 1024 * 24 * sizeof(long long), st));
        a.trace = nb <= 1024 ? sc.trace : nullptr;
        sc.trace_nb = nb;
    }
    static const int chain_la = [] { const char* e = getenv("MFGP_DF_CHAIN_LA"); return e ? atoi(e) : 5; }();
    a.chain_la = chain_la;
    a.spin_limit = 4000000000LL;
    static const int occ = [] { const char* e = getenv("MFGP_DF_OCC"); return e ? atoi(e) : 2; }();
    int grid = (occ < 1 ? 1 : occ) * sc.sms;
    if (grid > a.total + a.m_total) grid = a.total + a.m_total;
    sc.trace_grid = grid < 1024 ? grid : 1024;
    if (nb < DF_TMA_MIN_NB) {
        constexpr int smem_c = DF_SMEM_DOUBLES * sizeof(double);
        MFGP_CUDA_CHECK(cudaFuncSetAttribute(chol_dataflow_cpasync_kernel, cudaFuncAttributeMaxDynamicSharedMemorySize, smem_c));
        chol_dataflow_cpasync_kernel<<<grid, DF_THREADS, smem_c, st>>>(a);
        MFGP_LAUNCH_CHECK();
        return MFGP_OK;
    }
    std::lock_guard<std::mutex> lock(sc.map_mu);
    int rc = df_cached_map(sc.kmap, K, npad, npad, ld, DF_LDA, PB);
    if (!rc) rc = df_cached_map(sc.wmap, W, npad, npad, ldw, DF_LDT, PB);
    if (!rc && nr > 0) rc = df_cached_map(sc.bmap, Bm, npad, R, ldb, DF_LDT, DF_K);
    if (rc) return rc;
    constexpr int smem = DF_SMEM_BYTES;
    MFGP_CUDA_CHECK(cudaFuncSetAttribute(chol_dataflow_kernel, cudaFuncAttributeMaxDynamicSharedMemorySize, smem));
    chol_dataflow_kernel<<<grid, DF_CTA_THREADS, smem, st>>>(sc.kmap.map, nr > 0 ? sc.bmap.map : sc.kmap.map, sc.wmap.map, a);
    MFGP_LAUNCH_CHECK();
    return MFGP_OK;
}
}

extern "C" int64_t mfgp_debug_chol_trace(int64_t* out, int64_t max_tasks) {
    int dev = 0;
    if (cudaGetDevice(&dev) != cudaSuccess || dev < 0 || dev >= 16) return 0;
    DfScratch& sc = g_df[dev];
    if (!sc.trace || !out) return 0;
    if (max_tasks < 0) {
        if (cudaMemcpy(out, sc.trace + 1024 * 16, 1024 * 8 * sizeof(long long), cudaMemcpyDeviceToHost) != cudaSuccess) return 0;
        return sc.trace_grid;
    }
    int64_t n = sc.trace_nb < max_tasks ? sc.trace_nb : max_tasks;
    if (cudaMemcpy(out, sc.trace, n * 16 * sizeof(long long), cudaMemcpyDeviceToHost) != cudaSuccess) return 0;
    return n;
}

extern "C" int mfgp_cholesky(double* K, int64_t npad, int64_t ld, double* W, int64_t ldw, int32_t* info, void* work,
                             void* stream) {
    if (!K || !info || npad <= 0 || npad % MFGP_TILE || ld < npad) return MFGP_ERR_INVALID;
    if (!W && !work) return MFGP_ERR_INVALID;
    if (W && ldw < npad) return MFGP_ERR_INVALID;
    cudaStream_t st = static_cast<cudaStream_t>(stream);
    if (W) {
        if (!work) return MFGP_ERR_INVALID;
        int* scratch = reinterpret_cast<int*>(static_cast<char*>(work) + npad * npad * 2 + (int64_t)PB * PB * 8 + 256);
        return chol_dataflow(K, npad, ld, W, ldw, info, nullptr, 0, 0, nullptr, 0, scratch, st);
    }
    MFGP_CUDA_CHECK(cudaMemsetAsync(info, 0, sizeof(int32_t), st));
    const int nb = (int)(npad / PB);
    constexpr int POTRF_SMEM = 0;
    MFGP_CUDA_CHECK(cudaFuncSetAttribute(potrf_diag_kernel, cudaFuncAttributeMaxDynamicSharedMemorySize, POTRF_SMEM));
    for (int j = 0; j < nb; j++) {
        double* Ajj = K + (int64_t)j * PB * (ld + 1);
        double* Wjj = W ? W + (int64_t)j * PB * (ldw + 1) : static_cast<double*>(work);
        const int64_t ldi = W ? ldw : PB;
        potrf_diag_kernel<<<1, 256, POTRF_SMEM, st>>>(Ajj, ld, Wjj, ldi, info, j);
        MFGP_LAUNCH_CHECK();
        const int rem = (int)(npad - (int64_t)(j + 1) * PB);
        if (rem <= 0) break;
        double* A21 = K + (int64_t)(j + 1) * PB * ld + (int64_t)j * PB;
        GemmArgs t{};
        t.A = A21; t.lda = ld; t.B = Wjj; t.ldb = ldi; t.C = A21; t.ldc = ld;
        t.M = rem; t.N = PB; t.K = PB; t.alpha = 1.0; t.beta = 0.0; t.mode = GEMM_GENERAL;
        int rc = launch_gemm(t, true, 1, st);
        if (rc) return rc;
        GemmArgs s{};
        s.A = A21; s.lda = ld; s.B = A21; s.ldb = ld; s.C = K + (int64_t)(j + 1) * PB * (ld + 1); s.ldc = ld;
        s.M = rem; s.N = rem; s.K = PB; s.alpha = -1.0; s.beta = 1.0; s.mode = GEMM_SYRK_LOWER;
        rc = launch_gemm(s, true, 1, st);
        if (rc) return rc;
    }
    return MFGP_OK;
}

extern "C" int mfgp_cholesky_solve(double* K, int64_t npad, int64_t ld, double* W, int64_t ldw, int32_t* info, double* Bm,
                                   int64_t ldb, int64_t R, void* work, int64_t work_bytes, void* stream) {
    if (!K || !W || !info || !Bm || npad <= 0 || npad % MFGP_TILE || ld < npad || ldw < npad || R <= 0 || R % GT || ldb < R)
        return MFGP_ERR_INVALID;
    if (!work || work_bytes < df_scratch_bytes(npad, R)) return MFGP_ERR_INVALID;
    return chol_dataflow(K, npad, ld, W, ldw, info, Bm, ldb, R, nullptr, 0, static_cast<int*>(work), static_cast<cudaStream_t>(stream));
}

extern "C" int mfgp_cholesky_solve_gram(double* K, int64_t npad, int64_t ld, double* W, int64_t ldw, int32_t* info, double* Bm,
                                        int64_t ldb, int64_t R, double* M, int64_t ldm, void* work, int64_t work_bytes,
                                        void* stream) {
    if (!M) return mfgp_cholesky_solve(K, npad, ld, W, ldw, info, Bm, ldb, R, work, work_bytes, stream);
    if (!K || !W || !info || !Bm || npad <= 0 || npad % MFGP_TILE || ld < npad || ldw < npad || R <= 0 || R % GT || ldb < R || ldm < R)
        return MFGP_ERR_INVALID;
    if (!work || work_bytes < df_scratch_bytes(npad, R, true)) return MFGP_ERR_INVALID;
    return chol_dataflow(K, npad, ld, W, ldw, info, Bm, ldb, R, M, ldm, static_cast<int*>(work), static_cast<cudaStream_t>(stream));
}

extern "C" int mfgp_tri_inverse(const double* L, int64_t npad, int64_t ld, double* W, int64_t ldw, void* work,
                                void* stream) {
    if (!L || !W || !work || npad <= 0 || npad % MFGP_TILE || ld < npad || ldw < npad) return MFGP_ERR_INVALID;
    cudaStream_t st = static_cast<cudaStream_t>(stream);
    double* T = static_cast<double*>(work);
    {
        dim3 grid((unsigned)((npad + 255) / 256), (unsigned)npad);
        zero_offdiag_blocks_kernel<<<grid, 256, 0, st>>>(W, (int)npad, ldw);
        MFGP_LAUNCH_CHECK();
    }
    for (int64_t b = PB; b < npad; b *= 2) {
        const int nfull = (int)(npad / (2 * b));
        const int64_t rem = npad - 2 * b * nfull;
        for (int pass = 0; pass < 2; pass++) {
            int batch;
            int64_t top, h;
            if (pass == 0) { batch = nfull; top = 0; h = b; }
            else { batch = (rem > b) ? 1 : 0; top = 2 * b * nfull; h = rem - b; }
            if (batch == 0) continue;
            GemmArgs g1{};
            g1.A = L + (top + b) * ld + top; g1.lda = ld; g1.strideA = 2 * b * (ld + 1);
            g1.B = W + top * (ldw + 1); g1.ldb = ldw; g1.strideB = 2 * b * (ldw + 1);
            g1.C = T; g1.ldc = b; g1.strideC = b * b;
            g1.M = (int)h; g1.N = (int)b; g1.K = (int)b; g1.alpha = 1.0; g1.beta = 0.0; g1.mode = GEMM_B_LOWER;
            int rc = launch_gemm(g1, false, batch, st);
            if (rc) return rc;
            GemmArgs g2{};
            g2.A = W + (top + b) * (ldw + 1); g2.lda = ldw; g2.strideA = 2 * b * (ldw + 1);
            g2.B = T; g2.ldb = b; g2.strideB = b * b;
            g2.C = W + (top + b) * ldw + top; g2.ldc = ldw; g2.strideC = 2 * b * (ldw + 1);
            g2.M = (int)h; g2.N = (int)b; g2.K = (int)h; g2.alpha = -1.0; g2.beta = 0.0; g2.mode = GEMM_A_LOWER;
            rc = launch_gemm(g2, false, batch, st);
            if (rc) return rc;
        }
    }
    return MFGP_OK;
}

extern "C" int mfgp_whiten(const double* W, int64_t npad, int64_t ldw, const double* y, int64_t NL, int64_t NH,
                           const mfgp_params* p_host, double* z, void* stream) {
    if (!W || !z || !p_host || npad <= 0 || npad % MFGP_TILE || ldw < npad || NL + NH > npad) return MFGP_ERR_INVALID;
    if (NL + NH > 0 && !y) return MFGP_ERR_INVALID;
    cudaStream_t st = static_cast<cudaStream_t>(stream);
    const int wpb = 8;
    whiten_kernel<<<(unsigned)((npad + wpb - 1) / wpb), wpb * 32, 0, st>>>(W, (int)npad, ldw, y, (int)NL, (int)NH,
                                                                          p_host->mean_L, p_host->mean_H, z, 0);
    MFGP_LAUNCH_CHECK();
    return MFGP_OK;
}

extern "C" int mfgp_cholesky_append(const double* Xt, int64_t NL, int64_t NH_old, int64_t NH_new, const mfgp_params* p_host,
                                    double* K, int64_t ld, double* W, int64_t ldw, const double* y, double* z, double* Tt,
                                    int32_t* info, void* work, int64_t work_bytes, void* stream) {
    if (!Xt || !p_host || !K || !W || !y || !z || !info || !work || NL < 0 || NH_old < 0 || NH_new < NH_old) return MFGP_ERR_INVALID;
    const int64_t N_old = NL + NH_old, N_new = NL + NH_new;
    if (N_new == N_old) return MFGP_OK;
    const int64_t npad = mfgp_npad(N_new);
    if (ld < npad || ldw < npad) return MFGP_ERR_INVALID;
    if (!p_host->multi && NL != 0) return MFGP_ERR_INVALID;
    cudaStream_t st = static_cast<cudaStream_t>(stream);
    const DevParams dp = make_dev_params(*p_host);
    MFGP_CUDA_CHECK(cudaMemsetAsync(info, 0, sizeof(int32_t), st));
    constexpr int POTRF_SMEM = 0;
    MFGP_CUDA_CHECK(cudaFuncSetAttribute(potrf_diag_kernel, cudaFuncAttributeMaxDynamicSharedMemorySize, POTRF_SMEM));
    double* part = static_cast<double*>(work);
    if (Tt) {
        scaled_coords_kernel<<<(unsigned)((npad + 255) / 256), 256, 0, st>>>(Xt, (int)N_new, (int)npad, dp, Tt);
        MFGP_LAUNCH_CHECK();
    }
    for (int64_t rb = N_old / PB * PB; rb < npad; rb += PB) {
        {
            dim3 block(32, 8), grid((unsigned)((rb + PB + 31) / 32), PB / 8);
            build_train_cov_kernel<<<grid, block, 0, st>>>(Xt, (int)NL, (int)NH_new, dp, K, (int)(rb + PB), ld, Tt, (int)rb);
            MFGP_LAUNCH_CHECK();
        }
        if (rb > 0) {
            dim3 zgrid(1, (unsigned)rb);
            zero_cols_kernel<<<zgrid, PB, 0, st>>>(W + rb, ldw);
            MFGP_LAUNCH_CHECK();
        }
        double* Kb = K + rb * ld;
        double* Wb = W + rb * ldw;
        double* Kbb = Kb + rb;
        double* Wbb = Wb + rb;
        if (rb > 0) {
            int nsplit = (int)(rb / 256);
            if (nsplit < 1) nsplit = 1;
            if (nsplit > 16) nsplit = 16;
            int kchunk = (int)((rb / PB + nsplit - 1) / nsplit) * PB;
            nsplit = (int)((rb + kchunk - 1) / kchunk);
            const int64_t pstride = (int64_t)PB * rb;
            if (work_bytes < (int64_t)nsplit * pstride * 8) return MFGP_ERR_INVALID;
            dim3 rgrid((unsigned)((rb + 127) / 128), PB);
            GemmArgs g1{};
            g1.A = Kb; g1.lda = ld; g1.B = W; g1.ldb = ldw; g1.C = part; g1.ldc = rb; g1.strideC = pstride;
            g1.M = PB; g1.N = (int)rb; g1.K = (int)rb; g1.alpha = 1.0; g1.beta = 0.0; g1.mode = GEMM_BT_LOWER; g1.kchunk = kchunk;
            int rc = launch_gemm(g1, true, nsplit, st);
            if (rc) return rc;
            splitk_reduce_kernel<<<rgrid, 128, 0, st>>>(part, nsplit, pstride, (int)rb, Kb, ld, PB, (int)rb, 1.0, 0.0);
            MFGP_LAUNCH_CHECK();
            GemmArgs g2{};
            g2.A = Kb; g2.lda = ld; g2.B = Kb; g2.ldb = ld; g2.C = part; g2.ldc = PB; g2.strideC = PB * PB;
            g2.M = PB; g2.N = PB; g2.K = (int)rb; g2.alpha = 1.0; g2.beta = 0.0; g2.mode = GEMM_GENERAL; g2.kchunk = kchunk;
            rc = launch_gemm(g2, true, nsplit, st);
            if (rc) return rc;
            splitk_reduce_kernel<<<dim3(1, PB), 64, 0, st>>>(part, nsplit, PB * PB, PB, Kbb, ld, PB, PB, -1.0, 1.0);
            MFGP_LAUNCH_CHECK();
        }
        potrf_diag_kernel<<<1, 256, POTRF_SMEM, st>>>(Kbb, ld, Wbb, ldw, info, (int)(rb / PB));
        MFGP_LAUNCH_CHECK();
        if (rb > 0) {
            int nsplit = (int)(rb / 256);
            if (nsplit < 1) nsplit = 1;
            if (nsplit > 16) nsplit = 16;
            int kchunk = (int)((rb / PB + nsplit - 1) / nsplit) * PB;
            nsplit = (int)((rb + kchunk - 1) / kchunk);
            const int64_t pstride = (int64_t)PB * rb;
            double* T2 = part + (int64_t)nsplit * pstride;
            if (work_bytes < ((int64_t)nsplit + 1) * pstride * 8) return MFGP_ERR_INVALID;
            GemmArgs g3{};
            g3.A = Kb; g3.lda = ld; g3.B = W; g3.ldb = ldw; g3.C = part; g3.ldc = rb; g3.strideC = pstride;
            g3.M = PB; g3.N = (int)rb; g3.K = (int)rb; g3.alpha = 1.0; g3.beta = 0.0; g3.mode = GEMM_B_LOWER; g3.kchunk = kchunk;
            int rc = launch_gemm(g3, false, nsplit, st);
            if (rc) return rc;
            dim3 rgrid((unsigned)((rb + 127) / 128), PB);
            splitk_reduce_kernel<<<rgrid, 128, 0, st>>>(part, nsplit, pstride, (int)rb, T2, rb, PB, (int)rb, 1.0, 0.0);
            MFGP_LAUNCH_CHECK();
            GemmArgs g4{};
            g4.A = Wbb; g4.lda = ldw; g4.B = T2; g4.ldb = rb; g4.C = Wb; g4.ldc = ldw;
            g4.M = PB; g4.N = (int)rb; g4.K = PB; g4.alpha = -1.0; g4.beta = 0.0; g4.mode = GEMM_GENERAL;
            rc = launch_gemm(g4, false, 1, st);
            if (rc) return rc;
        }
        whiten_kernel<<<PB / 8, 256, 0, st>>>(W, (int)(rb + PB), ldw, y, (int)NL, (int)NH_new, p_host->mean_L, p_host->mean_H, z, (int)rb);
        MFGP_LAUNCH_CHECK();
    }
    return MFGP_OK;
}

extern "C" int64_t mfgp_append_workspace_bytes(int64_t npad) { return (int64_t)17 * PB * npad * 8 + 256; }
```

Measured before the change: 484.5 million.

## Generate covariance and RHS entries inside the dataflow Cholesky instead of materializing

Replaces the separate train-covariance build and the RHS/z build kernels with on-the-fly generation of those entries inside the persistent dataflow Cholesky/solve/gram kernel, driven by scaled coordinates and Chebyshev tables. This removes several launches and a full write and reread of K and B through global memory. It also adds L1 prefetches of the table and coordinate data ahead of use. In exchange the tile tasks do extra arithmetic and gathers, which may lengthen the critical path of the factorization.

```diff
diff --git a/include/mfgp_b200.h b/include/mfgp_b200.h
--- a/include/mfgp_b200.h
+++ b/include/mfgp_b200.h
@@ -119,6 +119,11 @@
 int64_t mfgp_cholesky_solve_gram_workspace_bytes(int64_t npad, int64_t R);
 int mfgp_cholesky_solve_gram(double* K, int64_t npad, int64_t ld, double* W, int64_t ldw, int32_t* info, double* Bm, int64_t ldb,
                              int64_t R, double* M, int64_t ldm, void* work, int64_t work_bytes, void* stream);
+int mfgp_factored_fit(const double* ux, int64_t nx, const double* uy, int64_t ny, int64_t ix0, int64_t ncols, const double* Xt,
+                      const double* y, int64_t NL, int64_t NH, int64_t npad, const mfgp_params* p_host, int64_t rxL, int64_t ryL,
+                      int64_t rxH, int64_t ryH, double xlo, double xhi, double ylo, double yhi, int64_t chunk_cols,
+                      const int32_t* kx, double* Tt, double* K, int64_t ld, double* W, int64_t ldw, int32_t* info, double* Yall,
+                      int64_t ldY, double* M, void* work, int64_t work_bytes, void* cwork, int64_t cwork_bytes, void* stream);
 int mfgp_posterior_grid_factored_solved_gram(const double* ux, int64_t nx, const double* uy, int64_t ny, int64_t ix0,
                                              int64_t ncols, const double* Xt, int64_t NL, int64_t NH, int64_t npad,
                                              const mfgp_params* p_host, int64_t rxL, int64_t ryL, int64_t rxH, int64_t ryH,
diff --git a/mfgp-coverage_b200/_engine.py b/mfgp-coverage_b200/_engine.py
--- a/mfgp-coverage_b200/_engine.py
+++ b/mfgp-coverage_b200/_engine.py
@@ -488,21 +488,18 @@
             R = int(lib.mfgp_factored_rhs_cols(*o))
         if self._fB is None or self._fB.numel() < self.cap * R:
             self._fB = self._wsalloc(self.cap * R, 0)
-        nat.check(lib.mfgp_build_train_cov(nat.ptr(self.Xt), self.NL, self.NH, pp, nat.ptr(self.K), npad, ld,
-                                           nat.ptr(self.Tt), st), "mfgp_build_train_cov")
-        nat.check(lib.mfgp_factored_prepare_trunc(nat.ptr(axes.ux), axes.nx, nat.ptr(axes.uy), axes.ny, plan["ix0"], plan["ncols"],
-                                                  nat.ptr(self.Xt), nat.ptr(self.y), self.NL, self.NH, npad, pp, *o, *geom,
-                                                  kxp if kx is not None else None, nat.ptr(self._fB), R, nat.ptr(work),
-                                                  work.numel() * 8, st), "mfgp_factored_prepare")
+        cneed = int(lib.mfgp_cholesky_solve_gram_workspace_bytes(self.cap, R))
+        if self._cwork is None or self._cwork.numel() * 8 < cneed:
+            self._cwork = self._wsalloc(cneed // 8)
         ev = self.profile_events
         if ev is not None:
             ev[0].record()
-        cneed = int(lib.mfgp_cholesky_solve_gram_workspace_bytes(self.cap, R))
-        if self._cwork is None or self._cwork.numel() * 8 < cneed:
-            self._cwork = self._wsalloc(cneed // 8)
-        nat.check(lib.mfgp_cholesky_solve_gram(nat.ptr(self.K), npad, ld, nat.ptr(self.W), ld, nat.ptr(self.info),
-                                               nat.ptr(self._fB), R, R, ctypes.c_void_p(M), R, nat.ptr(self._cwork),
-                                               self._cwork.numel() * 8, st), "mfgp_cholesky_solve_gram")
+        nat.check(lib.mfgp_factored_fit(nat.ptr(axes.ux), axes.nx, nat.ptr(axes.uy), axes.ny, plan["ix0"], plan["ncols"],
+                                        nat.ptr(self.Xt), nat.ptr(self.y), self.NL, self.NH, npad, pp, *o, *geom,
+                                        kxp if kx is not None else None, nat.ptr(self.Tt), nat.ptr(self.K), ld, nat.ptr(self.W),
+                                        ld, nat.ptr(self.info), nat.ptr(self._fB), R, ctypes.c_void_p(M), nat.ptr(work),
+                                        work.numel() * 8, nat.ptr(self._cwork), self._cwork.numel() * 8, st),
+                  "mfgp_factored_fit")
         if ev is not None:
             ev[1].record()
         Gs, Hs = self._factored_stores(plan)
diff --git a/mfgp-coverage_b200/_native.py b/mfgp-coverage_b200/_native.py
--- a/mfgp-coverage_b200/_native.py
+++ b/mfgp-coverage_b200/_native.py
@@ -94,6 +94,10 @@
     "mfgp_factored_gram_target": (c_void_p, [c_int64, c_int64, c_int64, c_int64, c_int64, c_int64, c_int64, POINTER(MfgpParams),
                                              c_int64, c_int64, c_int64, c_int64, c_int64, c_void_p, c_int64, c_void_p, c_int64]),
     "mfgp_cholesky_solve_gram_workspace_bytes": (c_int64, [c_int64, c_int64]),
+    "mfgp_factored_fit": (c_int, [c_void_p, c_int64, c_void_p, c_int64, c_int64, c_int64, c_void_p, c_void_p, c_int64, c_int64,
+                                  c_int64, POINTER(MfgpParams), c_int64, c_int64, c_int64, c_int64, c_double, c_double, c_double,
+                                  c_double, c_int64, c_void_p, c_void_p, c_void_p, c_int64, c_void_p, c_int64, c_void_p, c_void_p,
+                                  c_int64, c_void_p, c_void_p, c_int64, c_void_p, c_int64, c_void_p]),
     "mfgp_cholesky_solve_gram": (c_int, [c_void_p, c_int64, c_int64, c_void_p, c_int64, c_void_p, c_void_p, c_int64, c_int64,
                                          c_void_p, c_int64, c_void_p, c_int64, c_void_p]),
     "mfgp_posterior_grid_factored_solved_gram": (c_int, [c_void_p, c_int64, c_void_p, c_int64, c_int64, c_int64, c_void_p, c_int64,
diff --git a/mfgp-coverage_b200/csrc/common.cuh b/mfgp-coverage_b200/csrc/common.cuh
--- a/mfgp-coverage_b200/csrc/common.cuh
+++ b/mfgp-coverage_b200/csrc/common.cuh
@@ -42,6 +42,8 @@
 __device__ __forceinline__ void cp_async_wait() {
     asm volatile("cp.async.wait_group %0;\n" ::"n"(N));
 }
+
+__device__ __forceinline__ void prefetch_l1(const void* p) { asm volatile("prefetch.global.L1 [%0];\n" ::"l"(p)); }
 
 __device__ __forceinline__ uint32_t smem_u32(const void* p) { return static_cast<uint32_t>(__cvta_generic_to_shared(p)); }
 __device__ __forceinline__ void mbar_init(uint32_t bar, uint32_t count) {
diff --git a/mfgp-coverage_b200/csrc/fit_inputs.cuh b/mfgp-coverage_b200/csrc/fit_inputs.cuh
--- /dev/null
+++ b/mfgp-coverage_b200/csrc/fit_inputs.cuh
@@ -0,0 +1,74 @@
+#pragma once
+#include "common.cuh"
+
+namespace mfgp {
+
+__device__ __forceinline__ double train_cov_entry(const double4* a, const double4* b, const DevParams& p, int NL, int N, int i, int j) {
+    if (i >= N || j >= N) return (i == j) ? 1.0 : 0.0;
+    const bool iL = i < NL, jL = j < NL;
+    double v;
+    if (p.multi) {
+        const double kL = rbf_scaled(a->x, a->y, b->x, b->y, p.s_L);
+        if (iL && jL) {
+            v = kL;
+            if (i == j) v = __dadd_rn(v, p.noise_L);
+        } else if (iL != jL) {
+            v = __dmul_rn(p.rho, kL);
+        } else {
+            const double kH = rbf_scaled(a->z, a->w, b->z, b->w, p.s_H);
+            v = __dadd_rn(__dmul_rn(p.rho2, kL), kH);
+            if (i == j) v = __dadd_rn(v, p.noise_H);
+        }
+    } else {
+        v = rbf_scaled(a->z, a->w, b->z, b->w, p.s_H);
+        if (i == j) v = __dadd_rn(v, p.noise_H);
+    }
+    if (i == j) v = __dadd_rn(v, p.jitter);
+    return v;
+}
+
+constexpr int F_MAXR = 64;
+
+struct FTrunc {
+    short off[F_MAXR + 1];
+    short kx[F_MAXR];
+    int ry, cols;
+};
+
+struct BTab { const double* Cx; const double* Cy; int rx, ry; double coef_lo, coef_hi; };
+
+struct RhsGen {
+    BTab t0, t1; int ntab;
+    int64_t ldt;
+    FTrunc tr;
+    const double* y; double mean_L, mean_H;
+    int NL, N;
+};
+
+__device__ __forceinline__ int rhs_term(const FTrunc& tr, int e, int l) {
+    while (tr.off[l + 1] <= e) l++;
+    return l;
+}
+
+__device__ __forceinline__ double rhs_b_entry(const RhsGen& g, int n, int l, int k) {
+    double v = 0.0;
+    if (n < g.N) {
+        const BTab& t0 = g.t0;
+        const BTab& t1 = g.t1;
+        if (l < t0.ry && k < t0.rx)
+            v = __dmul_rn(__dmul_rn(n < g.NL ? t0.coef_lo : t0.coef_hi, t0.Cy[(int64_t)l * g.ldt + n]), t0.Cx[(int64_t)k * g.ldt + n]);
+        if (g.ntab > 1 && l < t1.ry && k < t1.rx)
+            v = __fma_rn(__dmul_rn(n < g.NL ? t1.coef_lo : t1.coef_hi, t1.Cy[(int64_t)l * g.ldt + n]), t1.Cx[(int64_t)k * g.ldt + n], v);
+    }
+    return v;
+}
+
+__device__ __forceinline__ double rhs_z_entry(const RhsGen& g, int n, int c) {
+    return (c == g.tr.cols && n < g.N) ? __dsub_rn(g.y[n], n < g.NL ? g.mean_L : g.mean_H) : 0.0;
+}
+
+int chol_solve_generated(const double* Xt, int64_t NL, int64_t NH, const mfgp_params& p, double* Tt, const RhsGen& rhs, double* K,
+                         int64_t npad, int64_t ld, double* W, int64_t ldw, int32_t* info, double* Bm, int64_t ldb, int64_t R, double* M,
+                         int64_t ldm, void* work, int64_t work_bytes, cudaStream_t st, bool check_only);
+
+}
diff --git a/mfgp-coverage_b200/csrc/gp_factored.cu b/mfgp-coverage_b200/csrc/gp_factored.cu
--- a/mfgp-coverage_b200/csrc/gp_factored.cu
+++ b/mfgp-coverage_b200/csrc/gp_factored.cu
@@ -1,4 +1,5 @@
 #include "common.cuh"
+#include "fit_inputs.cuh"
 #include "gemm_f64.cuh"
 #include <cstdlib>
 #include <cstring>
@@ -6,13 +7,6 @@
 namespace mfgp {
 
 constexpr int F_LW = 64;
-constexpr int F_MAXR = 64;
-
-struct FTrunc {
-    short off[F_MAXR + 1];
-    short kx[F_MAXR];
-    int ry, cols;
-};
 
 struct FPart {
     int rx, ry, kpad;
@@ -82,30 +76,17 @@
     }
 }
 
-struct BTab { const double* Cx; const double* Cy; int rx, ry; double coef_lo, coef_hi; };
-__global__ void build_B_merged_kernel(BTab t0, BTab t1, int ntab, int npad, int N, int NL, FTrunc tr, double* __restrict__ B,
-                                      int64_t ldB) {
+__global__ void build_B_merged_kernel(RhsGen g, double* __restrict__ B, int64_t ldB) {
     const int n = blockIdx.y;
     const int e = blockIdx.x * blockDim.x + threadIdx.x;
-    if (e >= tr.cols) return;
-    int l = 0;
-    while (tr.off[l + 1] <= e) l++;
-    const int k = e - tr.off[l];
-    double v = 0.0;
-    if (n < N) {
-        if (l < t0.ry && k < t0.rx) v = (n < NL ? t0.coef_lo : t0.coef_hi) * t0.Cy[(int64_t)l * npad + n] * t0.Cx[(int64_t)k * npad + n];
-        if (ntab > 1 && l < t1.ry && k < t1.rx)
-            v += (n < NL ? t1.coef_lo : t1.coef_hi) * t1.Cy[(int64_t)l * npad + n] * t1.Cx[(int64_t)k * npad + n];
-    }
-    B[(int64_t)n * ldB + e] = v;
-}
-
-__global__ void build_z_block_kernel(const double* __restrict__ y, int npad, int N, int NL, double mean_L, double mean_H,
-                                     double* __restrict__ B, int64_t ldB) {
-    const int n = blockIdx.x, c = threadIdx.x;
-    double v = 0.0;
-    if (c == 0 && n < N) v = y[n] - (n < NL ? mean_L : mean_H);
-    B[(int64_t)n * ldB + c] = v;
+    if (e >= g.tr.cols) return;
+    const int l = rhs_term(g.tr, e, 0);
+    B[(int64_t)n * ldB + e] = rhs_b_entry(g, n, l, e - g.tr.off[l]);
+}
+
+__global__ void build_z_block_kernel(RhsGen g, double* __restrict__ B, int64_t ldB) {
+    const int n = blockIdx.x, c = g.tr.cols + threadIdx.x;
+    B[(int64_t)n * ldB + c] = rhs_z_entry(g, n, c);
 }
 
 __global__ void unpack_Y_kernel(const double* __restrict__ Yall, int64_t ldY, int off, int cols, double* __restrict__ Yp) {
@@ -744,7 +725,7 @@
     f_set_trunc(L, nullptr);
 }
 
-int f_tables_and_B(const FGeom& g, FLayout& L, double* Ball, int64_t ldB, cudaStream_t st) {
+int f_tables(const FGeom& g, FLayout& L, RhsGen& rhs, cudaStream_t st) {
     const DevParams dp = make_dev_params(*g.p);
     const int64_t N = g.NL + g.NH, npad = g.npad;
     FPart& f = L.parts[0];
@@ -768,11 +749,22 @@
         cheb_coef_kernel<<<cgrid, 256, 0, st>>>(g.Xt, (int)N, (int)npad, jobs);
         MFGP_LAUNCH_CHECK();
     }
+    rhs = RhsGen{};
+    rhs.t0 = bt[0]; rhs.t1 = bt[1]; rhs.ntab = L.ntabs; rhs.ldt = npad; rhs.tr = L.tr;
+    rhs.y = nullptr; rhs.mean_L = dp.mean_L; rhs.mean_H = dp.mean_H;
+    rhs.NL = (int)g.NL; rhs.N = (int)N;
+    return MFGP_OK;
+}
+
+int f_tables_and_B(const FGeom& g, FLayout& L, double* Ball, int64_t ldB, cudaStream_t st, RhsGen* rhs_out = nullptr) {
+    RhsGen rhs;
+    const int rc = f_tables(g, L, rhs, st);
+    if (rc) return rc;
     const int cols = L.tr.cols;
-    dim3 bgrid((unsigned)((cols + 127) / 128), (unsigned)npad);
-    build_B_merged_kernel<<<bgrid, 128, 0, st>>>(bt[0], bt[1], L.ntabs, (int)npad, (int)N, (int)g.NL, L.tr, Ball ? Ball : f.B,
-                                                Ball ? ldB : (int64_t)cols);
+    dim3 bgrid((unsigned)((cols + 127) / 128), (unsigned)g.npad);
+    build_B_merged_kernel<<<bgrid, 128, 0, st>>>(rhs, Ball ? Ball : L.parts[0].B, Ball ? ldB : (int64_t)cols);
     MFGP_LAUNCH_CHECK();
+    if (rhs_out) *rhs_out = rhs;
     return MFGP_OK;
 }
 
@@ -1006,12 +998,40 @@
     const int64_t zoff = L.tr.cols;
     const int64_t R = round_up(zoff + 1, 64);
     if (ldB < R) return MFGP_ERR_INVALID;
-    rc = f_tables_and_B(g, L, Ball, ldB, st);
+    RhsGen rhs;
+    rc = f_tables_and_B(g, L, Ball, ldB, st, &rhs);
     if (rc) return rc;
-    build_z_block_kernel<<<(unsigned)npad, (int)(R - zoff), 0, st>>>(y, (int)npad, (int)(NL + NH), (int)NL, p_host->mean_L, p_host->mean_H,
-                                                                     Ball + zoff, ldB);
+    rhs.y = y;
+    build_z_block_kernel<<<(unsigned)npad, (int)(R - zoff), 0, st>>>(rhs, Ball, ldB);
     MFGP_LAUNCH_CHECK();
     return MFGP_OK;
+}
+
+extern "C" int mfgp_factored_fit(const double* ux, int64_t nx, const double* uy, int64_t ny, int64_t ix0, int64_t ncols,
+                                 const double* Xt, const double* y, int64_t NL, int64_t NH, int64_t npad, const mfgp_params* p_host,
+                                 int64_t rxL, int64_t ryL, int64_t rxH, int64_t ryH, double xlo, double xhi, double ylo, double yhi,
+                                 int64_t chunk_cols, const int32_t* kx, double* Tt, double* K, int64_t ld, double* W, int64_t ldw,
+                                 int32_t* info, double* Yall, int64_t ldY, double* M, void* work, int64_t work_bytes, void* cwork,
+                                 int64_t cwork_bytes, void* stream) {
+    if (!y || !Yall) return MFGP_ERR_INVALID;
+    FGeom g{ux, nx, uy, ny, ix0, ncols, Xt, NL, NH, npad, p_host, rxL, ryL, rxH, ryH, xlo, xhi, ylo, yhi, chunk_cols};
+    int rc = f_validate(g, work, work_bytes);
+    if (rc) return rc;
+    FLayout L;
+    f_carve(g, work, L);
+    if (!f_set_trunc(L, kx)) return MFGP_ERR_INVALID;
+    if (ldY % 64 || ldY < round_up(L.tr.cols + 1, 64) || ldY > f_max_ldY(L)) return MFGP_ERR_INVALID;
+    RhsGen rhs{};
+    rhs.NL = (int)NL; rhs.N = (int)(NL + NH);
+    rc = chol_solve_generated(Xt, NL, NH, *p_host, Tt, rhs, K, npad, ld, W, ldw, info, Yall, ldY, ldY, M, ldY, cwork, cwork_bytes,
+                              nullptr, true);
+    if (rc) return rc;
+    cudaStream_t st = static_cast<cudaStream_t>(stream);
+    rc = f_tables(g, L, rhs, st);
+    if (rc) return rc;
+    rhs.y = y;
+    return chol_solve_generated(Xt, NL, NH, *p_host, Tt, rhs, K, npad, ld, W, ldw, info, Yall, ldY, ldY, M, ldY, cwork, cwork_bytes, st,
+                                false);
 }
 
 extern "C" int mfgp_factored_prepare(const double* ux, int64_t nx, const double* uy, int64_t ny, int64_t ix0, int64_t ncols,
diff --git a/mfgp-coverage_b200/csrc/gp_fit.cu b/mfgp-coverage_b200/csrc/gp_fit.cu
--- a/mfgp-coverage_b200/csrc/gp_fit.cu
+++ b/mfgp-coverage_b200/csrc/gp_fit.cu
@@ -1,4 +1,5 @@
 #include "common.cuh"
+#include "fit_inputs.cuh"
 #include "gemm_f64.cuh"
 #include <cstdlib>
 #include <mutex>
@@ -23,11 +24,8 @@
     const int N = NL + NH;
     if (i >= npad || j >= npad) return;
     if (j >= ((i >> 6) + 1) * 64) return;
-    double v;
-    if (i >= N || j >= N) {
-        v = (i == j) ? 1.0 : 0.0;
-    } else {
-        double4 a, b;
+    double4 a = make_double4(0.0, 0.0, 0.0, 0.0), b = a;
+    if (i < N && j < N) {
         if (Tt != nullptr) {
             a = reinterpret_cast<const double4*>(Tt)[i];
             b = reinterpret_cast<const double4*>(Tt)[j];
@@ -36,26 +34,8 @@
             a = make_double4(xi / p.l_L, yi / p.l_L, xi / p.l_H, yi / p.l_H);
             b = make_double4(xj / p.l_L, yj / p.l_L, xj / p.l_H, yj / p.l_H);
         }
-        const bool iL = i < NL, jL = j < NL;
-        if (p.multi) {
-            const double kL = rbf_scaled(a.x, a.y, b.x, b.y, p.s_L);
-            if (iL && jL) {
-                v = kL;
-                if (i == j) v = v + p.noise_L;
-            } else if (iL != jL) {
-                v = p.rho * kL;
-            } else {
-                const double kH = rbf_scaled(a.z, a.w, b.z, b.w, p.s_H);
-                v = __dadd_rn(__dmul_rn(p.rho2, kL), kH);
-                if (i == j) v = v + p.noise_H;
-            }
-        } else {
-            v = rbf_scaled(a.z, a.w, b.z, b.w, p.s_H);
-            if (i == j) v = v + p.noise_H;
-        }
-        if (i == j) v = v + p.jitter;
-    }
-    K[(int64_t)i * ld + j] = v;
+    }
+    K[(int64_t)i * ld + j] = train_cov_entry(&a, &b, p, NL, N, i, j);
 }
 
 constexpr int PB = 64;
@@ -207,6 +187,12 @@
 constexpr uint32_t DF_KN_BYTES = DF_K * DF_LDT * 8;
 constexpr uint32_t DF_TILE_BYTES = PB * DF_LDT * 8;
 constexpr int DF_TMA_MIN_NB = 33;
+
+struct DfGen {
+    const double4* Tt;
+    DevParams p;
+    RhsGen rhs;
+};
 
 struct DfArgs {
     double* K; int64_t ld;
@@ -225,6 +211,7 @@
     long long spin_limit;
     long long* trace;
     int chain_la;
+    DfGen gen;
 };
 
 __host__ __device__ __forceinline__ void df_group_rows(int gi, int nb, int mg, int m_full, int& kb, int& ke) {
@@ -459,6 +446,10 @@
     }
 
     __device__ __forceinline__ void start(const DfArgs& g, const int* task, const DfTask& tk) {
+        if (g.gen.Tt != nullptr && !tk.gram) {
+            generate(g, task, tk);
+            return;
+        }
         const bool has_tile = tk.gram ? tk.gi > 0 : !(tk.chain && tk.idx == 0);
         const DfOut in = df_out(g, task);
 #pragma unroll
@@ -470,6 +461,100 @@
                 if (has_tile) v = *reinterpret_cast<const double2*>(in.Ct + (int64_t)r * in.ldc + cc);
                 if (tk.chain) d = *reinterpret_cast<const double2*>(in.Cd + (int64_t)r * g.ld + cc);
                 acc[x][y][0] = tk.gram ? v.x : -v.x; acc[x][y][1] = tk.gram ? v.y : -v.y;
+                acc2[x][y][0] = -d.x; acc2[x][y][1] = -d.y;
+            }
+    }
+
+    __device__ __forceinline__ void generate(const DfArgs& g, const int* task, const DfTask& tk) {
+        const DfGen& gen = g.gen;
+        const RhsGen& b = gen.rhs;
+        const int r0 = tk.i * PB;
+        if (tk.rhs) {
+            int l = 0;
+#pragma unroll
+            for (int y = 0; y < 4; y++) {
+                const int e = tk.idx * PB + wn + y * 16 + tq * 2;
+                if (e >= b.tr.cols) break;
+                l = rhs_term(b.tr, e, l);
+                const int k = e - b.tr.off[l];
+#pragma unroll
+                for (int x = 0; x < 2; x++) {
+                    const int n = r0 + wm + x * 32 + gq;
+                    const BTab* ts[2] = {&b.t0, &b.t1};
+#pragma unroll
+                    for (int t = 0; t < 2; t++) {
+                        if (t >= b.ntab || l >= ts[t]->ry || k >= ts[t]->rx) continue;
+                        prefetch_l1(ts[t]->Cy + (int64_t)l * b.ldt + n);
+                        prefetch_l1(ts[t]->Cx + (int64_t)k * b.ldt + n);
+                        if (k + 1 < ts[t]->rx) prefetch_l1(ts[t]->Cx + (int64_t)(k + 1) * b.ldt + n);
+                    }
+                }
+            }
+        } else {
+#pragma unroll
+            for (int x = 0; x < 2; x++) prefetch_l1(gen.Tt + r0 + wm + x * 32 + gq);
+#pragma unroll
+            for (int y = 0; y < 4; y++) {
+                const int j = wn + y * 16 + tq * 2;
+                if (!(tk.chain && tk.idx == 0)) prefetch_l1(gen.Tt + tk.c * PB + j);
+                if (tk.chain) prefetch_l1(gen.Tt + r0 + j);
+            }
+        }
+        if (tk.chain) {
+            double* Cd = df_out(g, task).Cd;
+#pragma unroll 2
+            for (int q = 0; q < 16; q++) {
+                const int r = wm + (q >> 3) * 32 + gq, c = wn + ((q >> 1) & 3) * 16 + tq * 2 + (q & 1);
+                Cd[(int64_t)r * g.ld + c] = train_cov_entry(gen.Tt + r0 + r, gen.Tt + r0 + c, gen.p, b.NL, b.N, r0 + r, r0 + c);
+            }
+        }
+#pragma unroll
+        for (int x = 0; x < 2; x++)
+#pragma unroll
+            for (int y = 0; y < 4; y++) acc[x][y][0] = acc[x][y][1] = 0.0;
+        if (tk.rhs) {
+            int l = 0;
+#pragma unroll 2
+            for (int q = 0; q < 8; q++) {
+                const int x = q & 1, y = q >> 1;
+                const int n = r0 + wm + x * 32 + gq, e = tk.idx * PB + wn + y * 16 + tq * 2;
+                double v0, v1;
+                if (e < b.tr.cols) {
+                    l = rhs_term(b.tr, e, l);
+                    const int k = e - b.tr.off[l];
+                    v0 = -rhs_b_entry(b, n, l, k);
+                    v1 = -rhs_b_entry(b, n, l, k + 1);
+                } else {
+                    v0 = -rhs_z_entry(b, n, e);
+                    v1 = -rhs_z_entry(b, n, e + 1);
+                }
+#pragma unroll
+                for (int xx = 0; xx < 2; xx++)
+#pragma unroll
+                    for (int yy = 0; yy < 4; yy++)
+                        if (q == yy * 2 + xx) { acc[xx][yy][0] = v0; acc[xx][yy][1] = v1; }
+            }
+        } else if (!(tk.chain && tk.idx == 0)) {
+            const int c0 = tk.c * PB;
+#pragma unroll 2
+            for (int q = 0; q < 16; q++) {
+                const int i = r0 + wm + (q >> 3) * 32 + gq, j = c0 + wn + ((q >> 1) & 3) * 16 + tq * 2 + (q & 1);
+                const double v = -train_cov_entry(gen.Tt + i, gen.Tt + j, gen.p, b.NL, b.N, i, j);
+#pragma unroll
+                for (int xx = 0; xx < 2; xx++)
+#pragma unroll
+                    for (int yy = 0; yy < 4; yy++)
+#pragma unroll
+                        for (int hh = 0; hh < 2; hh++)
+                            if (q == xx * 8 + yy * 2 + hh) acc[xx][yy][hh] = v;
+            }
+        }
+#pragma unroll
+        for (int x = 0; x < 2; x++)
+#pragma unroll
+            for (int y = 0; y < 4; y++) {
+                double2 d = make_double2(0.0, 0.0);
+                if (tk.chain) d = *reinterpret_cast<const double2*>(df_out(g, task).Cd + (int64_t)(wm + x * 32 + gq) * g.ld + wn + y * 16 + tq * 2);
                 acc2[x][y][0] = -d.x; acc2[x][y][1] = -d.y;
             }
     }
@@ -854,9 +939,6 @@
             return;
         }
         n_tasks++;
-        const double* Ag = tk.gram ? g.Bm + (int64_t)tk.kb * PB * g.ldb + (int64_t)tk.idx * PB : g.K + (int64_t)tk.i * PB * g.ld;
-        const double* Bg = tk.gram ? g.Bm + (int64_t)tk.kb * PB * g.ldb + (int64_t)tk.tj * PB
-                                   : (tk.rhs ? g.Bm + (int64_t)tk.idx * PB : g.K + (int64_t)(tk.c > 0 ? tk.c : 0) * PB * g.ld);
         bool ok = true;
         if (tk.gram && tk.gi > 0) {
             if (tracing) t_mark = clock64();
@@ -870,6 +952,9 @@
         }
         DfTile f(tid);
         f.start(g, task, tk);
+        const double* Ag = tk.gram ? g.Bm + (int64_t)tk.kb * PB * g.ldb + (int64_t)tk.idx * PB : g.K + (int64_t)tk.i * PB * g.ld;
+        const double* Bg = tk.gram ? g.Bm + (int64_t)tk.kb * PB * g.ldb + (int64_t)tk.tj * PB
+                                   : (tk.rhs ? g.Bm + (int64_t)tk.idx * PB : g.K + (int64_t)(tk.c > 0 ? tk.c : 0) * PB * g.ld);
 
         auto issue = [&](int s) {
             const int k0 = s * DF_K;
@@ -1088,13 +1173,18 @@
 };
 DfScratch g_df[16];
 
+bool df_aligned(const double* K, int64_t ld, const double* W, int64_t ldw, const double* Bm, int64_t ldb, int64_t R, const double* M,
+                int64_t ldm) {
+    auto aligned = [](const void* p, int64_t l) { return (reinterpret_cast<uintptr_t>(p) & 15) == 0 && (l & 1) == 0; };
+    return aligned(K, ld) && aligned(W, ldw) && (R == 0 || aligned(Bm, ldb)) && (!M || aligned(M, ldm));
+}
+
 int chol_dataflow(double* K, int64_t npad, int64_t ld, double* W, int64_t ldw, int32_t* info, double* Bm, int64_t ldb, int64_t R,
-                  double* M, int64_t ldm, int* scratch, cudaStream_t st) {
+                  double* M, int64_t ldm, int* scratch, cudaStream_t st, const DfGen* gen = nullptr) {
     int dev = 0;
     MFGP_CUDA_CHECK(cudaGetDevice(&dev));
     if (dev < 0 || dev >= 16 || !scratch) return MFGP_ERR_INVALID;
-    auto aligned = [](const void* p, int64_t l) { return (reinterpret_cast<uintptr_t>(p) & 15) == 0 && (l & 1) == 0; };
-    if (!aligned(K, ld) || !aligned(W, ldw) || (R > 0 && !aligned(Bm, ldb)) || (M && !aligned(M, ldm))) return MFGP_ERR_INVALID;
+    if (!df_aligned(K, ld, W, ldw, Bm, ldb, R, M, ldm)) return MFGP_ERR_INVALID;
     DfScratch& sc = g_df[dev];
     const int nb = (int)(npad / PB), nr = (int)(R / PB);
     const int64_t need = df_scratch_ints(npad, R, M != nullptr);
@@ -1102,6 +1192,7 @@
     MFGP_CUDA_CHECK(cudaMemsetAsync(scratch, 0, need * sizeof(int), st));
     MFGP_CUDA_CHECK(cudaMemsetAsync(info, 0, sizeof(int32_t), st));
     DfArgs a{};
+    if (gen) a.gen = *gen;
     a.K = K; a.ld = ld; a.W = W; a.ldw = ldw; a.Bm = Bm; a.ldb = ldb; a.nb = nb; a.nr = nr; a.info = info;
     a.ctrl = scratch; a.pause = scratch + DF_CTRL_INTS; a.flagsL = a.pause + 1024; a.flagsY = a.flagsL + (int64_t)nb * nb;
     a.total = nb + (nb - 1) * (nb - 2) / 2 + nb * nr;
@@ -1216,6 +1307,28 @@
         return MFGP_ERR_INVALID;
     if (!work || work_bytes < df_scratch_bytes(npad, R, true)) return MFGP_ERR_INVALID;
     return chol_dataflow(K, npad, ld, W, ldw, info, Bm, ldb, R, M, ldm, static_cast<int*>(work), static_cast<cudaStream_t>(stream));
+}
+
+namespace mfgp {
+int chol_solve_generated(const double* Xt, int64_t NL, int64_t NH, const mfgp_params& p, double* Tt, const RhsGen& rhs, double* K,
+                         int64_t npad, int64_t ld, double* W, int64_t ldw, int32_t* info, double* Bm, int64_t ldb, int64_t R, double* M,
+                         int64_t ldm, void* work, int64_t work_bytes, cudaStream_t st, bool check_only) {
+    const int64_t N = NL + NH;
+    if (!Xt || !Tt || !K || !W || !info || !Bm || NL < 0 || NH < 0 || N <= 0 || npad < N || npad % MFGP_TILE || ld < npad ||
+        ldw < npad || R <= 0 || R % GT || ldb < R || (M && ldm < R))
+        return MFGP_ERR_INVALID;
+    if ((!p.multi && NL != 0) || rhs.NL != NL || rhs.N != N || (reinterpret_cast<uintptr_t>(Tt) & 31)) return MFGP_ERR_INVALID;
+    if (!work || work_bytes < df_scratch_bytes(npad, R, M != nullptr) || !df_aligned(K, ld, W, ldw, Bm, ldb, R, M, ldm))
+        return MFGP_ERR_INVALID;
+    if (check_only) return MFGP_OK;
+    DfGen gen;
+    gen.Tt = reinterpret_cast<const double4*>(Tt);
+    gen.p = make_dev_params(p);
+    gen.rhs = rhs;
+    scaled_coords_kernel<<<(unsigned)((npad + 255) / 256), 256, 0, st>>>(Xt, (int)N, (int)npad, gen.p, Tt);
+    MFGP_LAUNCH_CHECK();
+    return chol_dataflow(K, npad, ld, W, ldw, info, Bm, ldb, R, M, ldm, static_cast<int*>(work), st, &gen);
+}
 }
 
 extern "C" int mfgp_tri_inverse(const double* L, int64_t npad, int64_t ld, double* W, int64_t ldw, void* work,
```

Measured after the change: 481.2 million, median of 6. No clear change (-0.7%).
